# ZhuoyangLiu2005/MLA

Measured on AMD Instinct MI355X. Metric: training samples/sec + step-time, MLA-Llama2-7B bf16, higher is better.
Workload: dtype bf16; 1 GPU; BASELINE.json configs[1]: MLA-Llama2-7B SFT, use_pointcloud+use_contrastive, 672x672(+mask) image + 1024 points + 32 text tokens, per-GPU batch 8 x 4 diffusion repeats = 32 x 548 tokens; model=mla-llama2-7b, global_batch=8, seq_len=548, parallelism=single-gpu, activation_save_level=1, optimizer=fused AdamW + grad clip inside the timed region

## Files before the change

### include/mla_hip.h

```cpp
#ifndef MLA_HIP_H
#define MLA_HIP_H

#include <stddef.h>
#include <stdint.h>

#ifdef __cplusplus
extern "C" {
#endif

typedef struct ihipStream_t* mla_stream_t;

const char* mla_last_error(void);
int mla_query(int what);
const char* mla_gemm_source_id(void);
int mla_selftest(const void* src_1k, int* out_tr_256, void* out_glds_1k, mla_stream_t stream);
int mla_calib_mfma(const void* operands, float* out, int blocks, int iters, double* flops_per_launch, mla_stream_t stream);
int mla_dispatch_probe(int* out, int blocks, int hold_us, mla_stream_t stream);

int mla_gemm_bf16(const void* A, const void* B, void* C, const void* R, const void* bias, int M, int N, int K, int lda, int ldb,
                  int ldc, int ldr, int a_mode, int b_mode, int out_fp32, int accumulate, float alpha, int force_generic,
                  mla_stream_t stream);
int mla_gemm_bf16_ws(const void* A, const void* B, void* C, const void* R, const void* bias, int M, int N, int K, int lda, int ldb,
                     int ldc, int ldr, int a_mode, int b_mode, int out_fp32, int accumulate, float alpha, int force_generic,
                     float* workspace, size_t workspace_bytes, mla_stream_t stream);
int mla_gemm_sq_slots(int M, int N, int K, size_t workspace_bytes);
int mla_gemm_kloop(int mode);
int mla_gemm_cus(int n);
int mla_gemm_bf16_ws_sq(const void* A, const void* B, void* C, int M, int N, int K, int lda, int ldb, int ldc, int accumulate,
                        float alpha, float* workspace, size_t workspace_bytes, float* sq_out, int sq_capacity, int* sq_slots,
                        mla_stream_t stream);
int mla_gemm_bf16_ws_sq_rm(const void* A, const void* B, void* C, int M, int N, int K, int lda, int ldb, int ldc, int a_mode, int b_mode,
                           int accumulate, float alpha, float* workspace, size_t workspace_bytes, float* sq_out, int sq_capacity,
                           int* sq_slots, mla_stream_t stream);

int mla_gemm_qkv_rope(const void* A, const void* B, void* C, int M, int N, int K, int lda, int ldb, int ldc, const float* rope_cos,
                      const float* rope_sin, int S, int rope_cols, mla_stream_t stream);

int mla_gemm_gateup_swiglu(const void* x, const void* wgu, void* gu, void* act, void* actT, int M, int I, int K, int lda, int ldb,
                           long long ldt, mla_stream_t stream);
int mla_gemm_dact_swiglu_bwd(const void* dy, const void* wT, const void* gu, void* dgu, void* dguT, int M, int I, int K, int lda,
                             int ldb, long long ldt, mla_stream_t stream);
int mla_gemm_dact_swiglu_bwd_rm(const void* dy, const void* w, const void* gu, void* dgu, void* dguT, int M, int I, int K, int lda,
                                int ldb, long long ldt, mla_stream_t stream);

int mla_gemm_res_norm(const void* A, const void* B, void* C, const void* R, const void* g, void* xg, float* ss, int M, int N, int K,
                      int lda, int ldb, int ldc, int ldr, float* workspace, size_t workspace_bytes, mla_stream_t stream);
int mla_gemm_qkv_rope_rs(const void* A, const void* B, void* C, int M, int N, int K, int lda, int ldb, int ldc, const float* rope_cos,
                         const float* rope_sin, int S, int rope_cols, const float* ss, int parts, float eps, float* rstd,
                         mla_stream_t stream);
int mla_gemm_gateup_swiglu_rs(const void* x, const void* wgu, void* gu, void* act, void* actT, int M, int I, int K, int lda, int ldb,
                              long long ldt, const float* ss, int parts, float eps, float* rstd, mla_stream_t stream);
int mla_rmsnorm_prep(const void* x, const void* w, void* xg, float* rstd, int rows, int H, float eps, mla_stream_t stream);

int mla_rmsnorm_fwd(const void* x, const void* w, void* y, float* rstd, int rows, int H, float eps, mla_stream_t stream);
int mla_rmsnorm_apply(const void* x, const void* w, const float* rstd, void* y, long long rows, int H, mla_stream_t stream);
int mla_rmsnorm_bwd_blocks(int rows);
int mla_rmsnorm_bwd(const void* dy, const void* x, const void* w, const float* rstd, const void* dres, void* dx, float* dw,
                    int dw_accumulate, int rows, int H, float* workspace, size_t workspace_bytes, mla_stream_t stream);
int mla_timm_rmsnorm_fwd(const void* x, const void* w, void* y, float* mean, float* rstd, int rows, int H, float eps,
                         mla_stream_t stream);
int mla_timm_rmsnorm_bwd(const void* dy, const void* x, const void* w, const float* mean, const float* rstd, void* dx, float* dw,
                         int dw_accumulate, int rows, int H, float* workspace, size_t workspace_bytes, mla_stream_t stream);
int mla_colsum_blocks(int rows);
int mla_colsum_bf16(const void* dy, float* out, int accumulate, int rows, int N, int ld, float* workspace, size_t workspace_bytes,
                    mla_stream_t stream);
int mla_layernorm_fwd(const void* x, const void* w, const void* b, void* y, int rows, int H, float eps, mla_stream_t stream);

int mla_rope_inplace(void* buf, const float* cos_t, const float* sin_t, long long tokens, int S, int nheads, int D, int ld,
                     int q_off, int k_off, int backward, mla_stream_t stream);

int mla_swiglu_fwd(const void* gu, void* act, long long rows, int I, mla_stream_t stream);
int mla_swiglu_bwd(const void* dact, const void* gu, void* dgu, void* act_out, long long rows, int I, mla_stream_t stream);
int mla_act_fwd(const void* x, void* y, long long n, int kind, mla_stream_t stream);
int mla_act_bwd(const void* dy, const void* x, void* dx, long long n, int kind, mla_stream_t stream);

int mla_cast_f32_to_bf16(const float* x, void* y, long long n, mla_stream_t stream);
int mla_cast_bf16_to_f32(const void* x, float* y, long long n, mla_stream_t stream);
int mla_add_bf16(const void* a, const void* b, void* y, long long n, mla_stream_t stream);
int mla_gather_rows_bf16(const void* src, const long long* idx, void* out, long long rows, int H, int scatter, mla_stream_t stream);

int mla_transpose_bf16(const void* src, void* dst, long long R, int C, long long ld, long long ldt, mla_stream_t stream);
int mla_rmsnorm_apply_t(const void* x, const void* w, const float* rstd, void* dst, long long rows, int H, long long ldt,
                        mla_stream_t stream);
int mla_swiglu_fwd_t(const void* gu, void* dst, long long rows, int I, long long ldt, mla_stream_t stream);
int mla_swiglu_fwd_dual(const void* gu, void* act, void* actT, long long rows, int I, long long ldt, mla_stream_t stream);
int mla_swiglu_bwd_t(const void* dact, const void* gu, void* dgu, void* dguT, long long rows, int I, long long ldt, mla_stream_t stream);

int mla_embedding_fwd(const long long* ids, const void* table, void* out, long long tokens, int H, int vocab, mla_stream_t stream);
int mla_embedding_bwd(const long long* ids, const void* dy, float* grad, float* workspace, long long tokens, int H, int vocab,
                      mla_stream_t stream);

int mla_adamw_step(float* p, const float* g, float* m, float* v, void* p16, long long n, float lr, float beta1, float beta2,
                   float eps, float weight_decay, int step, const float* grad_scale, mla_stream_t stream);
int mla_adamw_step_groups(float* p, const float* g, float* m, float* v, void* p16, long long n, long long n_decay, float lr, float beta1,
                          float beta2, float eps, float weight_decay, int step, const float* grad_scale, mla_stream_t stream);
int mla_sumsq_f32(const float* x, long long n, float* out, int accumulate, float* workspace, size_t workspace_bytes,
                  mla_stream_t stream);
int mla_sum_partials(const float* partial, int n, float* out, int accumulate, mla_stream_t stream);
int mla_clip_coef(const float* sumsq, float max_norm, float* coef, float* norm_out, mla_stream_t stream);

int mla_q_sample(const float* x0, const float* noise, const long long* t, const float* sqrt_ac, const float* sqrt_1mac, float* out,
                 int batch, int per, int nsteps, mla_stream_t stream);

int mla_attn_fwd(const void* q, const void* k, const void* v, void* o, float* lse, const int* seqlens, int B, int S, int H,
                 int head_dim, long long ld_qkv, long long ld_o, float scale, mla_stream_t stream);
int mla_attn_fwd_g(const void* q, const void* k, const void* v, void* o, float* lse, const int* seqlens, int B, int S, int H,
                   int head_dim, long long ld_qkv, long long ld_o, float scale, int grp_start, int grp_len, const int* grp_starts,
                   mla_stream_t stream);
int mla_attn_bwd_g(const void* q, const void* k, const void* v, const void* o, const void* dout, const float* lse, const int* seqlens,
                   void* dq, void* dk, void* dv, float* delta, int B, int S, int H, int head_dim, long long ld_qkv, long long ld_o,
                   float scale, const float* rope_cos, const float* rope_sin, void* dqT, void* dkT, void* dvT, void* oT,
                   long long ldt, int* head_sync, long long head_sync_ints, int grp_start, int grp_len, const int* grp_starts,
                   int rope_per_sample, mla_stream_t stream);
long long mla_attn_bwd_sync_ints(int B, int H);
int mla_attn_bwd(const void* q, const void* k, const void* v, const void* o, const void* dout, const float* lse, const int* seqlens,
                 void* dq, void* dk, void* dv, float* delta, int B, int S, int H, int head_dim, long long ld_qkv, long long ld_o,
                 float scale, const float* rope_cos, const float* rope_sin, int* head_sync, long long head_sync_ints,
                 mla_stream_t stream);
int mla_attn_bwd_t(const void* q, const void* k, const void* v, const void* o, const void* dout, const float* lse, const int* seqlens,
                   void* dq, void* dk, void* dv, float* delta, int B, int S, int H, int head_dim, long long ld_qkv, long long ld_o,
                   float scale, const float* rope_cos, const float* rope_sin, void* dqT, void* dkT, void* dvT, void* oT,
                   long long ldt, int* head_sync, long long head_sync_ints, mla_stream_t stream);
long long mla_attn_bwd_ws_bytes(int B, int S, int H);
int mla_attn_bwd_ws(const void* q, const void* k, const void* v, const void* o, const void* dout, const float* lse, const int* seqlens,
                    void* dq, void* dk, void* dv, float* delta, int B, int S, int H, int head_dim, long long ld_qkv, long long ld_o,
                    float scale, const float* rope_cos, const float* rope_sin, void* dqT, void* dkT, void* dvT, void* oT, long long ldt,
                    void* ws, long long ws_bytes, mla_stream_t stream);

int mla_gemv_bf16(const void* x, long long ldx, const void* W, long long ldw, void* out, long long ldo, long long out_batch_stride,
                  int rows_per_batch, const void* residual, long long ld_res, int M, int N, int K, int pre, const void* pre_w, float eps,
                  const float* rope_cos, const float* rope_sin, int rope_cols, mla_stream_t stream);
int mla_attn_decode(const void* q, const void* k, const void* v, void* o, int B, int H, int head_dim, int S_kv, int R, long long ld,
                    long long batch_stride, long long ld_o, float scale, mla_stream_t stream);
int mla_gemm_skinny_bf16(const void* x, long long ldx, const void* W, long long ldw, void* out, long long ldo, long long out_batch_stride,
                         int rows_per_batch, const void* residual, long long ld_res, int M, int N, int K, int pre, const void* pre_w, float eps,
                         const float* rope_cos, const float* rope_sin, int rope_cols, mla_stream_t stream);
int mla_quant_fp8_rows(const void* W, long long ldw, void* q, long long ldq, float* scale, int N, int K, mla_stream_t stream);
int mla_gemv_w8(const void* x, long long ldx, const void* W, long long ldw, const float* w_scale, void* out, long long ldo,
                long long out_batch_stride, int rows_per_batch, const void* residual, long long ld_res, int M, int N, int K, int pre,
                const void* pre_w, float eps, const float* rope_cos, const float* rope_sin, int rope_cols, mla_stream_t stream);
int mla_gemm_skinny_w8(const void* x, long long ldx, const void* W, long long ldw, const float* w_scale, void* out, long long ldo,
                       long long out_batch_stride, int rows_per_batch, const void* residual, long long ld_res, int M, int N, int K, int pre,
                       const void* pre_w, float eps, const float* rope_cos, const float* rope_sin, int rope_cols, mla_stream_t stream);
int mla_attn_chunk(const void* q, const void* k, const void* v, void* o, int B, int H, int head_dim, int S_kv, int R, long long ld,
                   long long batch_stride, long long ld_o, float scale, mla_stream_t stream);
int mla_attn_chunk_ragged(const void* q, const void* k, const void* v, void* o, int B, int H, int head_dim, const int* kv_len, int S_cap,
                          int R, long long ld, long long batch_stride, long long ld_o, float scale, mla_stream_t stream);
int mla_gemm_suffix_bf16(const void* x, long long ldx, const void* W, long long ldw, void* out, long long ldo, long long out_batch_stride,
                         int rows_per_batch, const int* slot, int cap_rows, const void* residual, long long ld_res, int M, int N, int K,
                         const float* rope_cos, const float* rope_sin, int rope_cols, mla_stream_t stream);
int mla_gemm_suffix_w8(const void* x, long long ldx, const void* W, long long ldw, const float* w_scale, void* out, long long ldo,
                       long long out_batch_stride, int rows_per_batch, const int* slot, int cap_rows, const void* residual, long long ld_res,
                       int M, int N, int K, const float* rope_cos, const float* rope_sin, int rope_cols, mla_stream_t stream);
int mla_attn_chunk_groups(const void* q, const void* k, const void* v, void* o, int G, int H, int head_dim, int S_p, int R, long long ld,
                          long long ld_o, float scale, mla_stream_t stream);
int mla_attn_chunk_groups_gw(const void* q, const void* k, const void* v, void* o, int G, int H, int head_dim, int S_p, int R, long long ld,
                             long long ld_o, float scale, int gw, int order, mla_stream_t stream);
int mla_attn_chunk_ragged_groups(const void* q, const void* k, const void* v, void* o, int B, int G, int H, int head_dim,
                                 const int* prefix_len, int S_cap, int R, long long ld, long long batch_stride, long long ld_o, float scale,
                                 mla_stream_t stream);
int mla_attn_chunk_ragged_groups_gw(const void* q, const void* k, const void* v, void* o, int B, int G, int H, int head_dim,
                                    const int* prefix_len, int S_cap, int R, long long ld, long long batch_stride, long long ld_o, float scale,
                                    int gw, int order, mla_stream_t stream);
int mla_gemm_suffix_bf16_pos(const void* x, long long ldx, const void* W, long long ldw, void* out, long long ldo, long long out_batch_stride,
                             int rows_per_batch, const int* slot, int cap_rows, const void* residual, long long ld_res, int M, int N, int K,
                             const float* rope_cos, const float* rope_sin, int rope_cols, const int* rope_pos, int rope_rows,
                             mla_stream_t stream);
int mla_gemm_suffix_w8_pos(const void* x, long long ldx, const void* W, long long ldw, const float* w_scale, void* out, long long ldo,
                           long long out_batch_stride, int rows_per_batch, const int* slot, int cap_rows, const void* residual,
                           long long ld_res, int M, int N, int K, const float* rope_cos, const float* rope_sin, int rope_cols,
                           const int* rope_pos, int rope_rows, mla_stream_t stream);
int mla_gemm_prefill_plan(int M, int N, int K, int cus, int* out4);
long long mla_gemm_prefill_ws_bytes(int M, int N, int K);
int mla_gemm_prefill_bf16(const void* x, long long ldx, const void* W, long long ldw, void* out, long long ldo, long long out_batch_stride,
                          int rows_per_batch, const void* residual, long long ld_res, int M, int N, int K, void* workspace,
                          size_t workspace_bytes, mla_stream_t stream);
int mla_gemm_prefill_qkv_rope(const void* x, long long ldx, const void* W, long long ldw, void* out, long long ldo,
                              long long out_batch_stride, int rows_per_batch, int M, int N, int K, const float* rope_cos,
                              const float* rope_sin, int rope_cols, int head_dim, void* workspace, size_t workspace_bytes,
                              mla_stream_t stream);
int mla_gemm_prefill_gateup_swiglu(const void* x, long long ldx, const void* wgu, long long ldw, void* act, long long ldo,
                                   long long out_batch_stride, int rows_per_batch, int M, int I, int K, void* workspace,
                                   size_t workspace_bytes, mla_stream_t stream);
int mla_gemm_prefill_f8_plan(int M, int N, int K, int cus, int* out4);
long long mla_gemm_prefill_f8_ws_bytes(int M, int N, int K);
int mla_gemm_prefill_f8(const void* xq, long long ldx, const float* x_scale, const void* Wq, long long ldw, const float* w_scale, void* out,
                        long long ldo, long long out_batch_stride, int rows_per_batch, const void* residual, long long ld_res, int M, int N,
                        int K, void* workspace, size_t workspace_bytes, mla_stream_t stream);
int mla_gemm_prefill_f8_qkv_rope(const void* xq, long long ldx, const float* x_scale, const void* Wq, long long ldw, const float* w_scale,
                                 void* out, long long ldo, long long out_batch_stride, int rows_per_batch, int M, int N, int K,
                                 const float* rope_cos, const float* rope_sin, int rope_cols, int head_dim, void* workspace,
                                 size_t workspace_bytes, mla_stream_t stream);
int mla_gemm_prefill_f8_gateup_swiglu(const void* xq, long long ldx, const float* x_scale, const void* wgu_q, long long ldw,
                                      const float* w_scale, void* act, long long ldo, long long out_batch_stride, int rows_per_batch, int M,
                                      int I, int K, void* workspace, size_t workspace_bytes, mla_stream_t stream);
int mla_gemm_prefill_f8_wide_plan(int M, int N, int K, int cus, int* out4);
long long mla_gemm_prefill_f8_wide_ws_bytes(int M, int N, int K);
int mla_gemm_prefill_f8_wide(const void* xq, long long ldx, const float* x_scale, const void* Wq, long long ldw, const float* w_scale,
                             void* out, long long ldo, long long out_batch_stride, int rows_per_batch, const void* residual,
                             long long ld_res, int M, int N, int K, void* workspace, size_t workspace_bytes, mla_stream_t stream);
int mla_gemm_prefill_f8_wide_qkv_rope(const void* xq, long long ldx, const float* x_scale, const void* Wq, long long ldw,
                                      const float* w_scale, void* out, long long ldo, long long out_batch_stride, int rows_per_batch, int M,
                                      int N, int K, const float* rope_cos, const float* rope_sin, int rope_cols, int head_dim,
                                      void* workspace, size_t workspace_bytes, mla_stream_t stream);
int mla_gemm_prefill_f8_wide_gateup_swiglu(const void* xq, long long ldx, const float* x_scale, const void* wgu_q, long long ldw,
                                           const float* w_scale, void* act, long long ldo, long long out_batch_stride, int rows_per_batch,
                                           int M, int I, int K, void* workspace, size_t workspace_bytes, mla_stream_t stream);

int mla_ddim_step(float* x, const void* eps, void* x_bf16, const float* coef, int* step, int n, int steps, int advance,
                  mla_stream_t stream);
int mla_ddpm_step(float* x, const void* eps, void* x_bf16, const float* coef, const float* noise, int* step, int n, int steps,
                  int advance, mla_stream_t stream);
int mla_sampler_rows(void* h_in, const void* t_table, const void* x_e, const int* step, int G, int T, int H, int steps,
                     mla_stream_t stream);

int mla_attn_chunk_split_plan(int B, int H, int R, int S_kv, int cus, int* out4);
long long mla_attn_chunk_split_ws_bytes(int B, int H, int R, int S_kv, int splits);
int mla_attn_chunk_split(const void* q, const void* k, const void* v, void* o, int B, int H, int head_dim, int S_kv, int R, long long ld,
                         long long batch_stride, long long ld_o, float scale, int splits, void* ws, size_t ws_bytes, mla_stream_t stream);
int mla_attn_groups_split(const void* q, const void* k, const void* v, void* o, int B, int G, int H, int head_dim, const int* prefix_len,
                          int S_p_or_cap, int R, long long ld, long long batch_stride, long long ld_o, float scale, int splits, void* ws,
                          size_t ws_bytes, mla_stream_t stream);

int mla_ce_fwd(const void* logits, int logits_fp32, long long ld, const long long* labels, float* loss, float* lse, int rows,
               int ncols, long long ignore_index, mla_stream_t stream);
int mla_ce_bwd(const void* logits, int logits_fp32, long long ld, const long long* labels, const float* lse, const float* gscale,
               float inv_count, void* dlogits, long long ldd, int rows, int ncols, long long ignore_index, mla_stream_t stream);
int mla_infonce_bwd(const float* L, const float* rlse, const float* clse, const float* gscale, void* dL, int M, int Mp,
                    mla_stream_t stream);
int mla_l2norm_fwd(const void* x, void* y, float* norms, int rows, int ncols, float eps, mla_stream_t stream);
int mla_l2norm_bwd(const void* dy, const void* y, const float* norms, void* dx, int rows, int ncols, mla_stream_t stream);

int mla_project_points(const float* xyz, const float* consts21, long long* idx, unsigned char* valid, int n, float W, float Hh,
                       float stride, int ph, int pw, mla_stream_t stream);
int mla_fps(const float* xyz, const long long* start, long long* out, int B, int N, int npoint, mla_stream_t stream);
int mla_knn(const float* xyz, const float* centers, int* out, int B, int N, int G, int k, mla_stream_t stream);
int mla_gather_rows_f32(const float* src, const long long* idx, float* out, int B, int N, int G, int W, mla_stream_t stream);
int mla_lga_prep(const float* xyz, const void* feats, const long long* fps_idx, const int* knn, void* rows, float* lc_xyz, int B,
                 int N, int G, int K, int C, float alpha, float beta, mla_stream_t stream);
int mla_colstats_blocks(long long rows);
int mla_colstats_bf16(const void* x, float* mean, float* var, long long rows, int C, int ld, float* workspace, size_t workspace_bytes,
                      mla_stream_t stream);
int mla_bn_apply(const void* x, const float* mean, const float* var, const void* w, const void* b, const void* res, void* y,
                 long long rows, int C, float eps, int relu, mla_stream_t stream);
int mla_maxpool_k(const void* x, void* out, long long groups, int K, int C, mla_stream_t stream);
int mla_lga_prep_bwd(const void* drows, const long long* fps_idx, const int* knn, float* dfeats, int B, int N, int G, int K, int C,
                     mla_stream_t stream);
int mla_maxpool_k_bwd(const void* x, const void* dy, void* dx, long long groups, int K, int C, mla_stream_t stream);

int mla_im2col_patch(const void* pix, int pix_fp32, void* rows, int B, int CT, int Himg, int Wimg, int P, int Kpad,
                     mla_stream_t stream);
int mla_avgpool_tokens(const void* x, void* y, int B, int gh, int gw, int C, int cs, mla_stream_t stream);
int mla_local_attn(const void* q, const void* kv, void* out, int B, int gh, int gw, int C, int cs, int heads, float scale,
                   mla_stream_t stream);
int mla_local_attn_bwd(const void* q, const void* kv, const void* dout, void* dq, void* dkv, int B, int gh, int gw, int C, int cs,
                       int heads, float scale, mla_stream_t stream);
int mla_clip_preprocess(const unsigned char* img, int B, int Hin, int Win, const int* bounds_h, const int* coef_h, int ks_h,
                        const int* bounds_v, const int* coef_v, int ks_v, void* out, int out_fp32, int OH, int OW, const float* mean3,
                        const float* std3, int mask_channel, mla_stream_t stream);
int mla_avgpool_tokens_bwd(const void* dy, const void* other, void* dx, int B, int gh, int gw, int C, int cs, mla_stream_t stream);

int mla_gemm_batched_bf16(const void* A, const void* B, void* C, int M, int N, int K, int lda, int ldb, int ldc, int a_mode, int b_mode,
                          int out_fp32, float alpha, int n_outer, int n_inner, long long sAo, long long sAi, long long sBo,
                          long long sBi, long long sCo, long long sCi, mla_stream_t stream);

int mla_softmax_rows_fwd(const float* scores, void* P, void* Pd, long long rows, int ncols, int nvalid, float p,
                         unsigned long long seed, mla_stream_t stream);
int mla_softmax_rows_bwd(const void* dPd, int dpd_fp32, const void* P, void* dS, long long rows, int ncols, int nvalid, float p,
                         unsigned long long seed, mla_stream_t stream);
int mla_dropout_fwd(const void* x, const void* residual, void* y, long long n, float p, unsigned long long seed, mla_stream_t stream);
int mla_dropout_bwd(const void* dy, void* dx, long long n, float p, unsigned long long seed, mla_stream_t stream);
int mla_scale_batch(const void* x, const float* scale, void* y, long long batch, long long per, mla_stream_t stream);
int mla_layernorm_stats_fwd(const void* x, const void* w, const void* b, void* y, float* mean, float* rstd, long long rows, int H,
                            float eps, mla_stream_t stream);
int mla_layernorm_bwd_blocks(long long rows);
int mla_layernorm_bwd(const void* dy, const void* x, const void* w, const float* mean, const float* rstd, void* dx, float* dw,
                      float* db, int accumulate, long long rows, int H, float* workspace, size_t workspace_bytes,
                      mla_stream_t stream);
int mla_seqmean_fwd(const void* x, void* y, int B, int S, int C, mla_stream_t stream);
int mla_seqmean_bwd(const void* dy, void* dx, int B, int S, int C, mla_stream_t stream);
int mla_bn_bwd_blocks(long long rows);
int mla_bn_bwd(const void* dy, const void* x, const float* mean, const float* var, const void* w, void* dx, float* dw, float* db,
               int accumulate, long long rows, int C, float eps, float* workspace, size_t workspace_bytes, mla_stream_t stream);
int mla_chamfer_fwd(const float* pred, const float* gt, float* d1, int* i1, float* d2, int* i2, float* loss, int B, int N, int M,
                    float* workspace, size_t workspace_bytes, mla_stream_t stream);
int mla_chamfer_bwd(const float* pred, const float* gt, const float* d1, const int* i1, const float* d2, const int* i2,
                    const float* gscale, float* dpred, int B, int N, int M, mla_stream_t stream);
int mla_imgloss_fwd(const void* delta_raw, int ld, const void* curr, const void* next, int img_fp32, float* sums, int B, int CT_curr,
                    int CT_next, int HW, int ps, float clip, float* workspace, size_t workspace_bytes, mla_stream_t stream);
int mla_imgroi_fwd(const void* delta_raw, int ld, const void* a_raw, int lda, const void* o_raw, int ldo, const unsigned char* roi,
                   const void* curr, const void* next, int img_fp32, float* sums, int B, int CT_curr, int CT_next, int HW, int ps,
                   float clip, float shift, float* workspace, size_t workspace_bytes, mla_stream_t stream);
int mla_imgroi_bwd(const void* delta_raw, int ld, const void* a_raw, int lda, const void* o_raw, int ldo, const unsigned char* roi,
                   const void* curr, const void* next, int img_fp32, const float* coef, void* ddelta_raw, float* dalpha_raw,
                   float* doff_raw, int B, int CT_curr, int CT_next, int HW, int ps, float clip, float shift, mla_stream_t stream);
int mla_imgloss_bwd(const void* delta_raw, int ld, const void* curr, const void* next, int img_fp32, const float* gscale,
                    void* ddelta_raw, int B, int CT_curr, int CT_next, int HW, int ps, float clip, mla_stream_t stream);

int mla_side_traffic(const float* a, const float* b, float* out, long long n, int blocks, int lds_bytes, int sleep_ticks, mla_stream_t stream);

#ifdef __cplusplus
}
#endif
#endif
```

### mla_amd/csrc/gemm256.hip

```cpp
#include "common.h"

#include "gemm_args.h"

#include "gemm256_kloop_clobbers.inc"
#include "gemm256_kloop_rm_clobbers.inc"
#ifndef MLA_GEMM_PLAIN_STORES
#define MLA_ST16(ADDR, VAL) __builtin_nontemporal_store((u32x4_t)(VAL), (u32x4_t*)(ADDR))
#define MLA_LD16(ADDR) __builtin_nontemporal_load((const u32x4_t*)(ADDR))
#else
#define MLA_ST16(ADDR, VAL) (*(u32x4_t*)(ADDR) = (VAL))
#define MLA_LD16(ADDR) (*(const u32x4_t*)(ADDR))
#endif

namespace {

constexpr int SLOT = 16384;
constexpr int SA0 = 0, SB0 = SLOT, SB1 = 2 * SLOT, SA1 = 3 * SLOT, BUF = 4 * SLOT;

__device__ __forceinline__ int hsw(int kr) { return (kr & 3) | (((kr >> 3) & 1) << 2); }
__device__ __forceinline__ int xcd_remap(int bid, int nwg) {
  const int q = nwg >> 3, r = nwg & 7;
  const int xcd = bid & 7, idx = bid >> 3;
  return (xcd < r ? xcd * (q + 1) : r * (q + 1) + (xcd - r) * q) + idx;
}

template <int MODE, bool IS_A>
__device__ __forceinline__ const bf16_t* stage_src(const bf16_t* g, int ld, int base, int lim, int h, int instr, int lane) {
  const int p = instr * 64 + lane;
  if (MODE == 0) {
    const int rp = p >> 3, cp = p & 7;
    const int c = cp ^ (rp & 7);
    int gi = base + h * 128 + rp;
    gi = gi < lim ? gi : lim - 1;
    return g + (size_t)gi * ld + c * 8;
  } else {
    const int kr = p >> 4, cp = p & 15;
    const int c = cp ^ (hsw(kr) << 1);
    const int ip = c * 8;
    int gi = base + h * 128 + ip;
    gi = (gi + 8 <= lim) ? gi : 0;
    return g + (size_t)kr * ld + gi;
  }
}

#ifndef MLA_GROUP_M
#define MLA_GROUP_M 4
#endif
#ifndef MLA_GEMM256_UNTRACKED
#define MLA_GEMM256_UNTRACKED 0
#endif
template <int AMODE, int BMODE, int EPI = 0, bool ASM = false>
__global__ __launch_bounds__(512, 2) void gemm256_kernel(GemmArgs p) {
  const bool LGKM_BEFORE = false;
  const int GROUP_M = MLA_GROUP_M;
#ifdef MLA_GEMM256_ABLATION
  const bool NO_READ = (p.debug & 4) != 0, NO_STAGE = (p.debug & 8) != 0, NO_BAR2 = (p.debug & 16) != 0, NO_BAR1 = (p.debug & 32) != 0;
  const int dbg = p.debug;
#else
  constexpr bool NO_READ = false, NO_STAGE = false, NO_BAR2 = false, NO_BAR1 = false;
  constexpr int dbg = 0;
#endif
  extern __shared__ __attribute__((aligned(16))) char smem[];
  const int tid = threadIdx.x, lane = tid & 63;
  const int wave = __builtin_amdgcn_readfirstlane(tid >> 6);
  const int wr = wave >> 2, wc = wave & 3;
  const int li = lane & 15, lg = lane >> 4;

  const int num_m = (p.M + 255) / 256, num_n = (p.N + 255) / 256;
  int pid, kt0 = 0, nt = p.K / 64;
  float* part = nullptr;
  if (p.sk_split <= 1) {
    pid = xcd_remap(blockIdx.x, gridDim.x);
  } else if ((int)blockIdx.x < p.sk_full) {
    pid = xcd_remap(blockIdx.x, p.sk_full);
  } else {
    const int u = blockIdx.x - p.sk_full;
    const int slice = u % p.sk_split;
    pid = p.sk_full + u / p.sk_split;
    if ((nt & 1) == 0) {
      const int np = nt >> 1;
      kt0 = 2 * (int)((long long)slice * np / p.sk_split);
      nt = 2 * (int)((long long)(slice + 1) * np / p.sk_split) - kt0;
    } else {
    kt0 = (int)((long long)slice * nt / p.sk_split);
    nt = (int)((long long)(slice + 1) * nt / p.sk_split) - kt0;
    }
    part = p.sk_ws + (size_t)u * 65536;
  }
#ifdef MLA_EXPERIMENTAL_KERNELS
  if (EPI != 0 && p.stagger_mode && (int)blockIdx.x < 256) {
    const bool late = p.stagger_mode == 1 ? (blockIdx.x & 1) : ((blockIdx.x >> 3) & 1);
    if (late) {
      const unsigned long long t0 = wall_clock64();
      while ((long long)(wall_clock64() - t0) < (long long)p.stagger_ticks) __builtin_amdgcn_s_sleep(64);
    }
  }
#endif
  const int in_group = GROUP_M * num_n;
  const int group_id = pid / in_group;
  const int first_m = group_id * GROUP_M;
  const int gsz = (num_m - first_m) < GROUP_M ? (num_m - first_m) : GROUP_M;
  const int pid_m = first_m + (pid % in_group) % gsz;
  const int pid_n = (pid % in_group) / gsz;
  const int m0 = pid_m * 256, n0 = pid_n * 256;

  f32x4_t acc[8][4];
  if constexpr (ASM) {
    static_assert(EPI == 0 || (AMODE == 0 && BMODE == 0) || (EPI == 2 && AMODE == 0 && BMODE == 1),
                  "the fused epilogues take k-contiguous operands (SwiGLU backward: or the weight as stored, B reduction-major)");
    const unsigned c0 = ((unsigned)lg ^ ((unsigned)li & 7u)) << 4;
    const unsigned vA0 = (unsigned)((wr * 64 + li) * 128) + c0, vB0 = 32768u + (unsigned)((wc * 32 + li) * 128) + c0;
    const unsigned lchunk = ((unsigned)lane & 7u) ^ (((unsigned)lane >> 3) & 7u);
    const int rt0 = wave * 32 + (lane >> 3);
    const int lastA = (p.M - 1 - m0) < 255 ? (p.M - 1 - m0) : 255;
    int lastB = (p.N - 1 - n0) < 255 ? (p.N - 1 - n0) : 255, bshift = 0;
    const bf16_t* pB = p.B + (size_t)n0 * p.ldb + (size_t)kt0 * 64;
    if (EPI == 1) {
      pB = p.B + (size_t)pid_n * 128 * p.ldb;
      bshift = wave >= 4 ? p.sf_I - 128 : 0;
      lastB = 255;
    }
    const unsigned oA0 = (unsigned)rt0 * (unsigned)p.lda * 2u + lchunk * 16u;
    const unsigned oB0 = (unsigned)(rt0 + bshift) * (unsigned)p.ldb * 2u + lchunk * 16u;
    const unsigned oAmax = (unsigned)lastA * (unsigned)p.lda * 2u + lchunk * 16u;
    const unsigned oBmax = (unsigned)(lastB + bshift) * (unsigned)p.ldb * 2u + lchunk * 16u;
    const int sA8 = p.lda * 16, sB8 = p.ldb * 16;
    const bf16_t* pA = p.A + (size_t)m0 * p.lda + (size_t)kt0 * 64;
    const int kmax = nt * 128 - 128, nit = nt >> 1, ldsw = wave * 4096;
    const bool img_bf16 = !part && !p.out_fp32 && p.R == nullptr && p.bias == nullptr;
    const bool rowscale = img_bf16 && p.rs_rstd != nullptr;
    if (rowscale && tid < 256) {
      const int mr = (m0 + tid) < p.M ? (m0 + tid) : (p.M - 1);
      float r;
      if (p.rs_ss) {
        const float* sp = p.rs_ss + (size_t)mr * p.rs_parts;
        float t = 0.f;
        for (int j = 0; j < p.rs_parts; ++j) t += sp[j];
        r = 1.0f / sqrtf(t / (float)p.K + p.rs_eps);
        if (pid_n == 0 && m0 + tid < p.M) p.rs_rstd[mr] = r;
      } else {
        r = p.rs_rstd[mr];
      }
      *(float*)(smem + 2 * BUF + tid * 4) = r;
    }
    const int emode = img_bf16 ? (rowscale ? 2 : 0) : 1;
    const float alpha = part ? 1.f : p.alpha;
    const unsigned vImg = img_bf16 ? (unsigned)((wr * 64 + li) * 512) + ((((unsigned)(wc * 4 + (lg >> 1))) ^ (unsigned)li) << 4) + (unsigned)(lg & 1) * 8u
                                   : (unsigned)((wr * 64 + li) * 1024) + ((((unsigned)(wc * 8 + lg)) ^ (unsigned)li) << 4);
    if constexpr (AMODE != 0 || BMODE != 0) {
      const int hs = ((li >> 2) & 3) | ((lg & 1) << 2);
      const unsigned rmrow = (unsigned)((lg * 8 + (li >> 2)) * 16), rmsub = (unsigned)((li & 3) >> 1), rmlo = (unsigned)(li & 1) * 8u;
      const unsigned vA = AMODE ? (rmrow + (((unsigned)(wr * 8) + rmsub) ^ ((unsigned)hs << 1))) * 16u + rmlo : vA0;
      const unsigned vB = BMODE ? 32768u + (rmrow + (((unsigned)(wc * 4) + rmsub) ^ ((unsigned)hs << 1))) * 16u + rmlo : vB0;
      const unsigned oAh0 = AMODE ? (unsigned)((const char*)stage_src<1, true>(p.A, p.lda, m0, p.M, 0, wave * 2, lane) - (const char*)p.A) : oA0;
      const unsigned oAh1 = AMODE ? (unsigned)((const char*)stage_src<1, true>(p.A, p.lda, m0, p.M, 1, wave * 2, lane) - (const char*)p.A) : oAmax;
      const unsigned oBh0 = BMODE ? (unsigned)((const char*)stage_src<1, false>(p.B, p.ldb, n0, p.N, 0, wave * 2, lane) - (const char*)p.B) : oB0;
      const unsigned oBh1 = BMODE ? (unsigned)((const char*)stage_src<1, false>(p.B, p.ldb, n0, p.N, 1, wave * 2, lane) - (const char*)p.B) : oBmax;
      const bf16_t* pAr = AMODE ? p.A + (size_t)kt0 * 64 * p.lda : pA;
      const bf16_t* pBr = BMODE ? p.B + (size_t)kt0 * 64 * p.ldb : pB;
      const int ldswA = AMODE ? wave * 2048 : ldsw, ldswB = BMODE ? wave * 2048 : ldsw;
      const int sA4 = p.lda * 8, sB4 = p.ldb * 8;
      const int nit_s = __builtin_amdgcn_readfirstlane(nit), emode_s = __builtin_amdgcn_readfirstlane(emode);
      const int alpha_s = __builtin_amdgcn_readfirstlane(__float_as_int(alpha));
#if defined(__HIP_DEVICE_COMPILE__)
#define MLA_KLOOP_RM_OPERANDS                                                                                                              \
        : : [pA] "s"(pAr), [pB] "s"(pBr), [nit] "s"(nit_s), [ldsw] "s"(ldswA), [ldswB] "s"(ldswB), [kA] "s"(p.lda), [kB] "s"(p.ldb),          \
            [sA8] "s"(sA8), [sB8] "s"(sB8), [sA4] "s"(sA4), [sB4] "s"(sB4), [emode] "s"(emode_s), [alpha] "s"(alpha_s), [vA0] "v"(vA),         \
            [vB0] "v"(vB), [oA0] "v"(oAh0), [oA2] "v"(oAh1), [oAmax] "v"(oAh1), [oB0] "v"(oBh0), [oB2] "v"(oBh1), [oBmax] "v"(oBh1),        \
            [vImg] "v"(vImg)                                                                                                                \
        : "memory", "scc", "vcc", "s40", "s41", "s42", "s43", "s44", "s45", "s46", "s47", "s48", "s49", "s50", "s51", "s52", "s53", "s54",  \
          "s55", "s56", "s57", "s58"
      if constexpr (AMODE != 0 && BMODE != 0) {
        asm volatile(
#include "gemm256_kloop_rm11.inc"
            MLA_KLOOP_RM_OPERANDS, G256K_RM11_CLOBBERS);
      } else if constexpr (AMODE != 0) {
        asm volatile(
#include "gemm256_kloop_rm10.inc"
            MLA_KLOOP_RM_OPERANDS, G256K_RM10_CLOBBERS);
      } else {
        asm volatile(
#include "gemm256_kloop_rm01.inc"
            MLA_KLOOP_RM_OPERANDS, G256K_RM01_CLOBBERS);
      }
#undef MLA_KLOOP_RM_OPERANDS
#endif
    } else {
#if defined(__HIP_DEVICE_COMPILE__)
    asm volatile(
#include "gemm256_kloop.inc"
        : : [pA] "s"(pA), [pB] "s"(pB), [kmax] "v"(kmax), [nit] "v"(nit), [ldsw] "s"(ldsw), [sA8] "s"(sA8), [sB8] "s"(sB8),
            [emode] "v"(emode), [alpha] "v"(alpha), [vA0] "v"(vA0), [vB0] "v"(vB0), [oA0] "v"(oA0), [oB0] "v"(oB0), [oAmax] "v"(oAmax),
            [oBmax] "v"(oBmax), [vImg] "v"(vImg)
        : "memory", "scc", "vcc", "s40", "s41", "s42", "s43", "s44", "s45", "s46", "s47", "s48", "s49", "s50", "s51", "s52", "s53", G256K_CLOBBERS);
#endif
    }
    if constexpr (EPI == 0) if (part) {
#pragma unroll
      for (int hf = 0; hf < 2; ++hf) {
        if (hf) {
          __syncthreads();
#if defined(__HIP_DEVICE_COMPILE__)
          asm volatile(
#include "gemm256_kloop_half1.inc"
              : : [alpha] "v"(alpha), [vImg] "v"(vImg) : "memory", "v0", "v1", "v2", "v3", "v4", "v5", "v6", "v7", "v8", "v9", "v10", "v11",
                "v12", "v13", "v14", "v15", "v16", "v17", "v18", "v19");
#endif
        }
        __syncthreads();
#pragma unroll
        for (int it = 0; it < 16; ++it) {
          const int row = wave * 16 + it;
          *(f32x4_t*)(part + (hf * 128 + row) * 256 + lane * 4) = *(const f32x4_t*)(smem + row * 1024 + ((lane ^ (row & 63)) << 4));
        }
      }
      return;
    }
  } else {
  const size_t stepA = (dbg & 64) ? 0 : (dbg & 2) ? 64 : (AMODE == 0 ? 64 : (size_t)64 * p.lda);
  const size_t stepB = (dbg & 64) ? 0 : (dbg & 2) ? 64 : (BMODE == 0 ? 64 : (size_t)64 * p.ldb);
  const bf16_t* pA0[2]; const bf16_t* pA1[2]; const bf16_t* pB0[2]; const bf16_t* pB1[2];
#pragma unroll
  for (int it = 0; it < 2; ++it) {
    if (dbg & 2) {
      pA0[it] = stage_src<0, true>(p.A, 4096, 0, 4096, 0, wave * 2 + it, lane);
      pA1[it] = stage_src<0, true>(p.A, 4096, 0, 4096, 1, wave * 2 + it, lane);
      pB0[it] = stage_src<0, false>(p.B, 4096, 0, 4096, 0, wave * 2 + it, lane);
      pB1[it] = stage_src<0, false>(p.B, 4096, 0, 4096, 1, wave * 2 + it, lane);
      continue;
    }
    pA0[it] = stage_src<AMODE, true>(p.A, p.lda, m0, p.M, 0, wave * 2 + it, lane);
    pA1[it] = stage_src<AMODE, true>(p.A, p.lda, m0, p.M, 1, wave * 2 + it, lane);
    if (EPI == 1) {
      pB0[it] = stage_src<BMODE, false>(p.B, p.ldb, pid_n * 128, p.sf_I, 0, wave * 2 + it, lane);
      pB1[it] = stage_src<BMODE, false>(p.B, p.ldb, p.sf_I + pid_n * 128 - 128, 2 * p.sf_I, 1, wave * 2 + it, lane);
      continue;
    }
    pB0[it] = stage_src<BMODE, false>(p.B, p.ldb, n0, p.N, 0, wave * 2 + it, lane);
    pB1[it] = stage_src<BMODE, false>(p.B, p.ldb, n0, p.N, 1, wave * 2 + it, lane);
  }
  if (kt0) {
#pragma unroll
    for (int it = 0; it < 2; ++it) {
      pA0[it] += (size_t)kt0 * stepA; pA1[it] += (size_t)kt0 * stepA;
      pB0[it] += (size_t)kt0 * stepB; pB1[it] += (size_t)kt0 * stepB;
    }
  }
  int tA0 = 0, tA1 = 0, tB0 = 0, tB1 = 0;
  constexpr bool UNTRACKED = (AMODE != 0 || BMODE != 0) || MLA_GEMM256_UNTRACKED;

#define STAGE(PTR, TCNT, STEP, SLOTOFF)                                                           \
  do {                                                                                            \
    const size_t back__ = (TCNT < nt) ? 0 : (size_t)TCNT * (STEP);  \
    char* dst__ = smem + (TCNT & 1) * BUF + (SLOTOFF) + wave * 2048;                              \
    if (!NO_STAGE || TCNT < 2) {  \
      if (UNTRACKED) {                                                                            \
        glds16_untracked(PTR[0] - back__, dst__);                                                 \
        glds16_untracked(PTR[1] - back__, dst__ + 1024);                                          \
      } else {                                                                                    \
        glds16(PTR[0] - back__, dst__);                                                           \
        glds16(PTR[1] - back__, dst__ + 1024);                                                    \
      }                                                                                           \
    }                                                                                             \
    PTR[0] += (STEP); PTR[1] += (STEP); ++TCNT;                                                   \
  } while (0)

  int offA[4], offB[2];
  if (AMODE == 0) {
    offA[0] = (wr * 64 + li) * 128 + ((lg ^ (li & 7)) * 16);
    offA[1] = offA[2] = offA[3] = 0;
  } else {
    const int h = ((li >> 2) & 3) | ((lg & 1) << 2);
#pragma unroll
    for (int rb = 0; rb < 4; ++rb)
      offA[rb] = ((lg * 8 + (li >> 2)) * 16 + ((wr * 8 + rb * 2 + ((li & 3) >> 1)) ^ (h << 1))) * 16 + (li & 1) * 8;
  }
  if (BMODE == 0) {
    offB[0] = (wc * 32 + li) * 128 + ((lg ^ (li & 7)) * 16);
    offB[1] = 0;
  } else {
    const int h = ((li >> 2) & 3) | ((lg & 1) << 2);
#pragma unroll
    for (int cb = 0; cb < 2; ++cb)
      offB[cb] = ((lg * 8 + (li >> 2)) * 16 + ((wc * 4 + cb * 2 + ((li & 3) >> 1)) ^ (h << 1))) * 16 + (li & 1) * 8;
  }

  auto ldA = [&](const char* slot, int rb, int ks) -> bf16x8_t {
    if (AMODE == 0) {
      return *(const bf16x8_t*)(slot + ((offA[0] + rb * 2048) ^ (ks * 64)));
    } else {
      if (dbg & 1) return *(const bf16x8_t*)(slot + (((wr * 64 + li) * 128 + ((lg ^ (li & 7)) * 16) + rb * 2048) ^ (ks * 64)));
      union { bf16x8_t v; short4_t h2[2]; } u;
      u.h2[0] = lds_tr16_b64(slot + offA[rb] + ks * 8192);
      u.h2[1] = lds_tr16_b64(slot + offA[rb] + ks * 8192 + 1024);
      return u.v;
    }
  };
  auto ldB = [&](const char* slot, int cb, int ks) -> bf16x8_t {
    if (BMODE == 0) {
      return *(const bf16x8_t*)(slot + ((offB[0] + cb * 2048) ^ (ks * 64)));
    } else {
      if (dbg & 1) return *(const bf16x8_t*)(slot + (((wc * 32 + li) * 128 + ((lg ^ (li & 7)) * 16) + cb * 2048) ^ (ks * 64)));
      union { bf16x8_t v; short4_t h2[2]; } u;
      u.h2[0] = lds_tr16_b64(slot + offB[cb] + ks * 8192);
      u.h2[1] = lds_tr16_b64(slot + offB[cb] + ks * 8192 + 1024);
      return u.v;
    }
  };

#pragma unroll
  for (int a = 0; a < 8; ++a)
#pragma unroll
    for (int b = 0; b < 4; ++b) acc[a][b] = f32x4_t{0.f, 0.f, 0.f, 0.f};

  bf16x8_t fa[4][2], fb0[2][2], fb1[2][2];
  bool rd_on = true;

#define READ_A(SLOTP)                                              \
  if (rd_on) _Pragma("unroll") for (int rb = 0; rb < 4; ++rb) {    \
    fa[rb][0] = ldA(SLOTP, rb, 0); fa[rb][1] = ldA(SLOTP, rb, 1);  \
  }
#define READ_B(DST, SLOTP)                                          \
  if (rd_on) _Pragma("unroll") for (int cb = 0; cb < 2; ++cb) {     \
    DST[cb][0] = ldB(SLOTP, cb, 0); DST[cb][1] = ldB(SLOTP, cb, 1); \
  }
#define SEG_END()                                                  \
  __builtin_amdgcn_sched_barrier(0);                               \
  if (LGKM_BEFORE) asm volatile("s_waitcnt vmcnt(8) lgkmcnt(0)" ::: "memory"); \
  else asm volatile("s_waitcnt vmcnt(10)" ::: "memory");           \
  if (!NO_BAR1) __builtin_amdgcn_s_barrier();                      \
  asm volatile("s_waitcnt lgkmcnt(0)" ::: "memory");               \
  __builtin_amdgcn_sched_barrier(0);
#define MMA(QI, QJ, FB)                                                                                          \
  __builtin_amdgcn_s_setprio(1);                                                                                 \
  _Pragma("unroll") for (int ks = 0; ks < 2; ++ks)                                                               \
  _Pragma("unroll") for (int rb = 0; rb < 4; ++rb)                                                               \
  _Pragma("unroll") for (int cb = 0; cb < 2; ++cb)                                                               \
    acc[QI * 4 + rb][QJ * 2 + cb] =                                                                              \
        __builtin_amdgcn_mfma_f32_16x16x32_bf16(FB[cb][ks], fa[rb][ks], acc[QI * 4 + rb][QJ * 2 + cb], 0, 0, 0); \
  __builtin_amdgcn_s_setprio(0);                                                                                 \
  __builtin_amdgcn_sched_barrier(0);                                                                             \
  asm volatile("" ::: "memory");                                                                                 \
  if (!NO_BAR2) __builtin_amdgcn_s_barrier();                                                                    \
  asm volatile("" ::: "memory");

  STAGE(pB0, tB0, stepB, SB0);
  STAGE(pA0, tA0, stepA, SA0);
  STAGE(pB1, tB1, stepB, SB1);
  STAGE(pA1, tA1, stepA, SA1);
  STAGE(pB0, tB0, stepB, SB0);
  STAGE(pA0, tA0, stepA, SA0);
  STAGE(pB1, tB1, stepB, SB1);
  asm volatile("s_waitcnt vmcnt(10)" ::: "memory");
  __builtin_amdgcn_s_barrier();
  READ_B(fb0, smem + SB0)
  if (wr == 1) __builtin_amdgcn_s_barrier();

#define TILE_BODY(X, Y, T_)                                          \
  {                                                                  \
    const char* buf = smem + ((T_) & 1) * BUF;                       \
    const char* nbuf = smem + (((T_) + 1) & 1) * BUF;                \
    if (NO_READ) rd_on = (T_) < 2;                                   \
    STAGE(pA1, tA1, stepA, SA1);                       \
    READ_A(buf + SA0)                                                \
    SEG_END()                                                        \
    MMA(0, 0, X)                                                     \
    STAGE(pB0, tB0, stepB, SB0);                       \
    READ_B(Y, buf + SB1)                                             \
    SEG_END()                                                        \
    MMA(0, 1, Y)                                                     \
    STAGE(pA0, tA0, stepA, SA0);                       \
    READ_A(buf + SA1)                                                \
    SEG_END()                                                        \
    MMA(1, 1, Y)                                                     \
    STAGE(pB1, tB1, stepB, SB1);                       \
    READ_B(Y, nbuf + SB0)                                            \
    SEG_END()                                                        \
    MMA(1, 0, X)                                                     \
  }
  int t = 0;
  for (; t + 1 < nt; t += 2) {
    TILE_BODY(fb0, fb1, t)
    TILE_BODY(fb1, fb0, t + 1)
  }
  if (t < nt) TILE_BODY(fb0, fb1, t)
#undef TILE_BODY
  if (wr == 0) __builtin_amdgcn_s_barrier();
  asm volatile("s_waitcnt vmcnt(0)" ::: "memory");
  }

  if constexpr (!ASM) if (part) {
#pragma unroll
    for (int ri = 0; ri < 8; ++ri) {
      const int ml = (ri >> 2) * 128 + wr * 64 + (ri & 3) * 16 + li;
#pragma unroll
      for (int ci = 0; ci < 4; ++ci) {
        const int nl = (ci >> 1) * 128 + wc * 32 + (ci & 1) * 16 + lg * 4;
        *(f32x4_t*)(part + ml * 256 + nl) = acc[ri][ci];
      }
    }
    return;
  }
  const bool vec_ok = ((p.ldc & 3) == 0) && (p.R == nullptr || (p.ldr & 3) == 0);
  const bool fast = (p.N & 7) == 0 && (p.ldc & 7) == 0 && (((uintptr_t)p.C) & 15) == 0 &&
                    (p.R == nullptr || ((p.ldr & 7) == 0 && (((uintptr_t)p.R) & 15) == 0)) &&
                    (p.bias == nullptr || (((uintptr_t)p.bias) & 15) == 0);
  if (fast) {
    __syncthreads();
    if (!p.out_fp32 && p.R == nullptr && p.bias == nullptr) {
      if constexpr (!ASM) {
      if (p.rs_rstd) {
        if (tid < 256) {
          const int mr = (m0 + tid) < p.M ? (m0 + tid) : (p.M - 1);
          float r;
          if (p.rs_ss) {
            const float* sp = p.rs_ss + (size_t)mr * p.rs_parts;
            float t = 0.f;
            for (int j = 0; j < p.rs_parts; ++j) t += sp[j];
            r = 1.0f / sqrtf(t / (float)p.K + p.rs_eps);
            if (pid_n == 0 && m0 + tid < p.M) p.rs_rstd[mr] = r;
          } else {
            r = p.rs_rstd[mr];
          }
          *(float*)(smem + 2 * BUF + tid * 4) = r;
        }
        __syncthreads();
      }
#pragma unroll
      for (int ri = 0; ri < 8; ++ri) {
        const int ml = (ri >> 2) * 128 + wr * 64 + (ri & 3) * 16 + li;
        const float rsc = p.rs_rstd ? *(const float*)(smem + 2 * BUF + ml * 4) : p.alpha;
#pragma unroll
        for (int ci = 0; ci < 4; ++ci) {
          const int nl = (ci >> 1) * 128 + wc * 32 + (ci & 1) * 16 + lg * 4;
          u32x2_t o;
          o[0] = pack2bf(acc[ri][ci][0] * rsc, acc[ri][ci][1] * rsc);
          o[1] = pack2bf(acc[ri][ci][2] * rsc, acc[ri][ci][3] * rsc);
          *(u32x2_t*)(smem + ml * 512 + ((((nl >> 3) ^ (ml & 31))) << 4) + ((nl >> 2) & 1) * 8) = o;
        }
      }
      }
      __syncthreads();
      if (EPI == 1) {
        const int I = p.sf_I, cbase = pid_n * 128;
        const size_t ld2 = (size_t)2 * I;
        for (int s4 = 0; s4 < 4; ++s4) {
          char* scrA = smem + s4 * 64 * 512;
          u32x4_t pa[2];
#pragma unroll
          for (int k4 = 0; k4 < 4; ++k4) {
            const int idx = tid + 512 * k4;
            const int rl = idx >> 5, ch = idx & 31;
            const int row = s4 * 64 + rl, m = m0 + row;
            if (p.C && m < p.M)
              MLA_ST16((bf16_t*)p.C + (size_t)m * ld2 + (ch < 16 ? cbase + ch * 8 : I + cbase + (ch - 16) * 8), *(const u32x4_t*)(smem + row * 512 + ((ch ^ (row & 31)) << 4)));
          }
#pragma unroll
          for (int k2 = 0; k2 < 2; ++k2) {
            const int idx = tid + 512 * k2;
            const int rl = idx >> 4, c = idx & 15;
            const int row = s4 * 64 + rl, m = m0 + row;
            float gv[8], uv[8], o[8];
            unpack8(*(const u32x4_t*)(smem + row * 512 + ((c ^ (row & 31)) << 4)), gv);
            unpack8(*(const u32x4_t*)(smem + row * 512 + (((16 + c) ^ (row & 31)) << 4)), uv);
#pragma unroll
            for (int j = 0; j < 8; ++j) o[j] = swiglu_fwd_elem(gv[j], uv[j]);
            pa[k2] = pack8(o);
            if (p.sf_act && m < p.M) MLA_ST16(p.sf_act + (size_t)m * I + cbase + c * 8, pa[k2]);
          }
          if (p.sf_actT == nullptr) continue;
          __syncthreads();
#pragma unroll
          for (int k2 = 0; k2 < 2; ++k2) {
            const int idx = tid + 512 * k2;
            const int rl = idx >> 4, c = idx & 15;
            const int slot2 = (rl ^ (2 * c)) * 2;
#pragma unroll
            for (int j = 0; j < 4; ++j) {
              const int c0 = (c * 8 + 2 * j) * 128 + slot2;
              *(unsigned short*)(scrA + c0) = (unsigned short)(pa[k2][j] & 0xffffu);
              *(unsigned short*)(scrA + c0 + 128) = (unsigned short)(pa[k2][j] >> 16);
            }
          }
          __syncthreads();
#pragma unroll
          for (int k2 = 0; k2 < 2; ++k2) {
            const int idx = tid + 512 * k2;
            const int col = idx >> 3, rc = idx & 7;
            const int chc = col >> 3, b = chc & 3;
            const int m = m0 + s4 * 64 + rc * 8;
            if (m < p.M) {
              u32x4_t w = *(const u32x4_t*)(scrA + col * 128 + ((rc ^ (chc >> 2)) << 4));
              if (b & 1) w = u32x4_t{w[1], w[0], w[3], w[2]};
              if (b & 2) w = u32x4_t{w[2], w[3], w[0], w[1]};
              MLA_ST16(p.sf_actT + (size_t)(cbase + col) * p.sf_ldt + m, w);
            }
          }
        }
        return;
      }
      if (EPI == 2) {
        const int I = p.sw_I;
        char* scrB = smem + 2 * BUF;
        const size_t ld2 = (size_t)2 * I;
        u32x4_t gq[4], uq[4];
        auto fetch_gu = [&](int strip, u32x4_t* g4, u32x4_t* u4) {
#pragma unroll
          for (int k4 = 0; k4 < 4; ++k4) {
            const int idx = tid + 512 * k4;
            const int m = m0 + strip * 64 + (idx >> 5), n = n0 + (idx & 31) * 8;
            g4[k4] = u32x4_t{0u, 0u, 0u, 0u};
            u4[k4] = g4[k4];
            if (m < p.M && n < p.N) {
              g4[k4] = MLA_LD16(p.sw_gu + (size_t)m * ld2 + n);
              u4[k4] = MLA_LD16(p.sw_gu + (size_t)m * ld2 + I + n);
            }
          }
        };
        if constexpr (ASM) fetch_gu(0, gq, uq);
        for (int s4 = 0; s4 < 4; ++s4) {
          char* scrA = smem + s4 * 64 * 512;
          u32x4_t pg[4], pu[4];
          u32x4_t gn[4], un[4];
          if constexpr (ASM) if (s4 < 3) fetch_gu(s4 + 1, gn, un);
#pragma unroll
          for (int k4 = 0; k4 < 4; ++k4) {
            const int idx = tid + 512 * k4;
            const int rl = idx >> 5, ch = idx & 31;
            const int row = s4 * 64 + rl;
            const int m = m0 + row, n = n0 + ch * 8;
            pg[k4] = u32x4_t{0u, 0u, 0u, 0u};
            pu[k4] = pg[k4];
            if (m < p.M && n < p.N) {
              float dv[8], gv[8], uv[8], dg[8], du[8];
              unpack8(*(const u32x4_t*)(smem + row * 512 + ((ch ^ (row & 31)) << 4)), dv);
              if constexpr (ASM) {
                unpack8(gq[k4], gv);
                unpack8(uq[k4], uv);
              } else {
              unpack8(*(const u32x4_t*)(p.sw_gu + (size_t)m * ld2 + n), gv);
              unpack8(*(const u32x4_t*)(p.sw_gu + (size_t)m * ld2 + I + n), uv);
              }
#pragma unroll
              for (int j = 0; j < 8; ++j) swiglu_bwd_elem(dv[j], gv[j], uv[j], dg[j], du[j]);
              pg[k4] = pack8(dg);
              pu[k4] = pack8(du);
              MLA_ST16(p.sw_dgu + (size_t)m * ld2 + n, pg[k4]);
              MLA_ST16(p.sw_dgu + (size_t)m * ld2 + I + n, pu[k4]);
            }
          }
          if (p.sw_dguT == nullptr) {
            if constexpr (ASM) {
#pragma unroll
              for (int k4 = 0; k4 < 4; ++k4) { gq[k4] = gn[k4]; uq[k4] = un[k4]; }
            }
            continue;
          }
          __syncthreads();
#pragma unroll
          for (int k4 = 0; k4 < 4; ++k4) {
            const int idx = tid + 512 * k4;
            const int rl = idx >> 5, ch = idx & 31;
            const int slot2 = (rl ^ (2 * ch)) * 2;
#pragma unroll
            for (int j = 0; j < 4; ++j) {
              const int c0 = (ch * 8 + 2 * j) * 128 + slot2;
              *(unsigned short*)(scrA + c0) = (unsigned short)(pg[k4][j] & 0xffffu);
              *(unsigned short*)(scrA + c0 + 128) = (unsigned short)(pg[k4][j] >> 16);
              *(unsigned short*)(scrB + c0) = (unsigned short)(pu[k4][j] & 0xffffu);
              *(unsigned short*)(scrB + c0 + 128) = (unsigned short)(pu[k4][j] >> 16);
            }
          }
          __syncthreads();
#pragma unroll
          for (int k4 = 0; k4 < 4; ++k4) {
            const int idx = tid + 512 * k4;
            const int col = idx >> 3, rc = idx & 7;
            const int chc = col >> 3;
            const int off = col * 128 + ((rc ^ (chc >> 2)) << 4);
            const int b = chc & 3;
            const int m = m0 + s4 * 64 + rc * 8, n = n0 + col;
            if (m < p.M && n < p.N) {
#pragma unroll
              for (int which = 0; which < 2; ++which) {
                u32x4_t w = *(const u32x4_t*)((which ? scrB : scrA) + off);
                if (b & 1) w = u32x4_t{w[1], w[0], w[3], w[2]};
                if (b & 2) w = u32x4_t{w[2], w[3], w[0], w[1]};
                MLA_ST16(p.sw_dguT + (size_t)(which * I + n) * p.sw_ldt + m, w);
              }
            }
          }
          if constexpr (ASM) {
#pragma unroll
            for (int k4 = 0; k4 < 4; ++k4) { gq[k4] = gn[k4]; uq[k4] = un[k4]; }
          }
        }
        return;
      }
      const int ch = lane & 31;
      const int n = n0 + ch * 8;
      if (p.rope_cos && n0 < p.rope_cols) {
        if (n < p.N) {
          const bool lo = (ch & 8) == 0;
#pragma unroll 4
          for (int it = 0; it < 16; ++it) {
            const int row = wave * 32 + it * 2 + (lane >> 5);
            const int m = m0 + row;
            if (m < p.M) {
              float own[8], par[8], c[8], sn[8], o[8];
              unpack8(*(const u32x4_t*)(smem + row * 512 + ((ch ^ (row & 31)) << 4)), own);
              unpack8(*(const u32x4_t*)(smem + row * 512 + (((ch ^ 8) ^ (row & 31)) << 4)), par);
              const float* ct = p.rope_cos + (size_t)(m % p.rope_S) * 64 + (ch & 7) * 8;
              const float* st = p.rope_sin + (size_t)(m % p.rope_S) * 64 + (ch & 7) * 8;
              const f32x4_t c0 = *(const f32x4_t*)ct, c1 = *(const f32x4_t*)(ct + 4), s0 = *(const f32x4_t*)st, s1 = *(const f32x4_t*)(st + 4);
#pragma unroll
              for (int j = 0; j < 4; ++j) { c[j] = c0[j]; c[j + 4] = c1[j]; sn[j] = s0[j]; sn[j + 4] = s1[j]; }
#pragma unroll
              for (int j = 0; j < 8; ++j)
                o[j] = lo ? fmaf(own[j], c[j], -(par[j] * sn[j])) : fmaf(own[j], c[j], par[j] * sn[j]);
              MLA_ST16((bf16_t*)p.C + (size_t)m * p.ldc + n, pack8(o));
            }
          }
        }
        return;
      }
      if (n < p.N) {
#pragma unroll
        for (int it = 0; it < 16; ++it) {
          const int row = wave * 32 + it * 2 + (lane >> 5);
          const int m = m0 + row;
          if (m < p.M)
            MLA_ST16((bf16_t*)p.C + (size_t)m * p.ldc + n, *(const u32x4_t*)(smem + row * 512 + ((ch ^ (row & 31)) << 4)));
        }
      }
      return;
    }
    if constexpr (EPI == 0 || !ASM) {
    float sq = 0.f;
    u32x4_t rpre[2][8];
    const bool r_pre = ASM && p.R != nullptr && !p.out_fp32;
    if (r_pre) {
      const int nn = n0 + (lane & 31) * 8;
#pragma unroll
      for (int h2 = 0; h2 < 2; ++h2)
#pragma unroll
        for (int it = 0; it < 8; ++it) {
          const int m = m0 + h2 * 128 + wave * 16 + it * 2 + (lane >> 5);
          rpre[h2][it] = u32x4_t{0u, 0u, 0u, 0u};
          if (m < p.M && nn < p.N) rpre[h2][it] = MLA_LD16(p.R + (size_t)m * p.ldr + nn);
        }
    }
#pragma unroll
    for (int hf = 0; hf < 2; ++hf) {
      if (hf) __syncthreads();
      if constexpr (ASM) {
#if defined(__HIP_DEVICE_COMPILE__)
        if (hf) {
          const unsigned vImg2 = (unsigned)((wr * 64 + li) * 1024) + ((((unsigned)(wc * 8 + lg)) ^ (unsigned)li) << 4);
          asm volatile(
#include "gemm256_kloop_half1.inc"
              : : [alpha] "v"(p.alpha), [vImg] "v"(vImg2) : "memory", "v0", "v1", "v2", "v3", "v4", "v5", "v6", "v7", "v8", "v9", "v10",
                "v11", "v12", "v13", "v14", "v15", "v16", "v17", "v18", "v19");
        }
#endif
      } else {
#pragma unroll
      for (int r4 = 0; r4 < 4; ++r4) {
        const int ri = hf * 4 + r4;
        const int ml = wr * 64 + r4 * 16 + li;
#pragma unroll
        for (int ci = 0; ci < 4; ++ci) {
          const int nl = (ci >> 1) * 128 + wc * 32 + (ci & 1) * 16 + lg * 4;
          *(f32x4_t*)(smem + ml * 1024 + (((nl >> 2) ^ (ml & 63)) << 4)) = acc[ri][ci] * p.alpha;
        }
      }
      }
      __syncthreads();
      if (p.out_fp32) {
        const int n = n0 + lane * 4;
        if (n < p.N) {
#pragma unroll
          for (int it = 0; it < 16; ++it) {
            const int row = wave * 16 + it;
            const int m = m0 + hf * 128 + row;
            if (m < p.M) {
              f32x4_t o = *(const f32x4_t*)(smem + row * 1024 + ((lane ^ (row & 63)) << 4));
              if (p.bias) {
                const u32x2_t bb = *(const u32x2_t*)(p.bias + n);
                o[0] += bflo(bb[0]); o[1] += bfhi(bb[0]); o[2] += bflo(bb[1]); o[3] += bfhi(bb[1]);
              }
              if (p.R) {
                const u32x2_t rr = *(const u32x2_t*)(p.R + (size_t)m * p.ldr + n);
                o[0] += bflo(rr[0]); o[1] += bfhi(rr[0]); o[2] += bflo(rr[1]); o[3] += bfhi(rr[1]);
              }
              float* c = (float*)p.C + (size_t)m * p.ldc + n;
              if (p.accumulate) o += *(const f32x4_t*)c;
              *(f32x4_t*)c = o;
              sq += (o[0] * o[0] + o[1] * o[1]) + (o[2] * o[2] + o[3] * o[3]);
            }
          }
        }
      } else {
        const int ch = lane & 31;
        const int n = n0 + ch * 8;
        if (n < p.N) {
          float bv[8];
#pragma unroll
          for (int j = 0; j < 8; ++j) bv[j] = 0.f;
          if (p.bias) unpack8(*(const u32x4_t*)(p.bias + n), bv);
          float ngv[8];
#pragma unroll
          for (int j = 0; j < 8; ++j) ngv[j] = 0.f;
          if (p.nrm_xg) unpack8(*(const u32x4_t*)(p.nrm_g + n), ngv);
#pragma unroll
          for (int it = 0; it < 8; ++it) {
            const int row = wave * 16 + it * 2 + (lane >> 5);
            const int m = m0 + hf * 128 + row;
            if (m < p.M) {
              const f32x4_t a = *(const f32x4_t*)(smem + row * 1024 + (((2 * ch) ^ (row & 63)) << 4));
              const f32x4_t b = *(const f32x4_t*)(smem + row * 1024 + (((2 * ch + 1) ^ (row & 63)) << 4));
              float v[8] = {a[0] + bv[0], a[1] + bv[1], a[2] + bv[2], a[3] + bv[3], b[0] + bv[4], b[1] + bv[5], b[2] + bv[6], b[3] + bv[7]};
              if (p.R) {
                float rv[8];
                unpack8(r_pre ? rpre[hf][it] : *(const u32x4_t*)(p.R + (size_t)m * p.ldr + n), rv);
#pragma unroll
                for (int j = 0; j < 8; ++j) v[j] += rv[j];
              }
              const u32x4_t hq = pack8(v);
              MLA_ST16((bf16_t*)p.C + (size_t)m * p.ldc + n, hq);
              if (p.nrm_xg) {
                float hv[8], xg[8];
                unpack8(hq, hv);
                float q = 0.f;
#pragma unroll
                for (int j = 0; j < 8; ++j) { q += hv[j] * hv[j]; xg[j] = hv[j] * ngv[j]; }
                MLA_ST16(p.nrm_xg + (size_t)m * p.ldc + n, pack8(xg));
                q = half_wave_sum_last(q);
                if (ch == 31) p.nrm_ss[(size_t)m * num_n + pid_n] = q;
              }
            }
          }
        }
      }
    }
    if (p.sq_out) {
      sq = wave_sum(sq);
      __syncthreads();
      if (lane == 0) ((float*)smem)[wave] = sq;
      __syncthreads();
      if (tid == 0) {
        float t = 0.f;
#pragma unroll
        for (int w = 0; w < 8; ++w) t += ((float*)smem)[w];
        p.sq_out[pid] = t;
      }
    }
    }
    return;
  }
  if constexpr (!ASM) {
#pragma unroll
  for (int ri = 0; ri < 8; ++ri) {
    const int m = m0 + (ri >> 2) * 128 + wr * 64 + (ri & 3) * 16 + li;
    if (m >= p.M) continue;

#pragma unroll
    for (int ci = 0; ci < 4; ++ci) {
      const int n = n0 + (ci >> 1) * 128 + wc * 32 + (ci & 1) * 16 + lg * 4;
      if (n >= p.N) continue;
      float v[4];
#pragma unroll
      for (int r = 0; r < 4; ++r) v[r] = acc[ri][ci][r] * p.alpha;
      if (n + 3 < p.N && vec_ok) {
        if (p.bias) {
          const u32x2_t bb = *(const u32x2_t*)(p.bias + n);
          v[0] += bflo(bb[0]); v[1] += bfhi(bb[0]); v[2] += bflo(bb[1]); v[3] += bfhi(bb[1]);
        }
        if (p.R) {
          const u32x2_t rr = *(const u32x2_t*)(p.R + (size_t)m * p.ldr + n);
          v[0] += bflo(rr[0]); v[1] += bfhi(rr[0]); v[2] += bflo(rr[1]); v[3] += bfhi(rr[1]);
        }
        if (p.out_fp32) {
          float* c = (float*)p.C + (size_t)m * p.ldc + n;
          f32x4_t o = {v[0], v[1], v[2], v[3]};
          if (p.accumulate) o += *(const f32x4_t*)c;
          *(f32x4_t*)c = o;
        } else {
          u32x2_t o;
          o[0] = pack2bf(v[0], v[1]);
          o[1] = pack2bf(v[2], v[3]);
          *(u32x2_t*)((bf16_t*)p.C + (size_t)m * p.ldc + n) = o;
        }
      } else {
        for (int r = 0; r < 4 && n + r < p.N; ++r) {
          float x = v[r];
          if (p.bias) x += bf2f(p.bias[n + r]);
          if (p.R) x += bf2f(p.R[(size_t)m * p.ldr + n + r]);
          if (p.out_fp32) {
            float* c = (float*)p.C + (size_t)m * p.ldc + n + r;
            *c = p.accumulate ? (*c + x) : x;
          } else {
            ((bf16_t*)p.C)[(size_t)m * p.ldc + n + r] = f2bf(x);
          }
        }
      }
    }
  }
  }
#undef STAGE
#undef READ_A
#undef READ_B
#undef SEG_END
#undef MMA
}

#ifdef MLA_EXPERIMENTAL_KERNELS
struct Unit {
  int m0, n0, kt0, nt;
  float* part;
};

__global__ __launch_bounds__(512, 2) void gemm256p_kernel(GemmArgs p) {
  const int GROUP_M = MLA_GROUP_M;
  extern __shared__ __attribute__((aligned(16))) char smem[];
  const int tid = threadIdx.x, lane = tid & 63;
  const int wave = __builtin_amdgcn_readfirstlane(tid >> 6);
  const int wr = wave >> 2, wc = wave & 3;
  const int li = lane & 15, lg = lane >> 4;
  const int num_m = (p.M + 255) / 256, num_n = (p.N + 255) / 256;
  const int ntK = p.K / 64;

  const int G = gridDim.x, W = G >> 3, b = blockIdx.x, x = b & 7, j = b >> 3;
  const int F = p.sk_split > 1 ? p.sk_full : num_m * num_n;
  const int q8 = F >> 3, r8 = F & 7;
  const int cnt_x = q8 + (x < r8 ? 1 : 0);
  const int start_x = x < r8 ? x * (q8 + 1) : r8 * (q8 + 1) + (x - r8) * q8;
  const int nfull = j < cnt_x ? (cnt_x - j + W - 1) / W : 0;
  const int tail_units = p.sk_split > 1 ? (num_m * num_n - p.sk_full) * p.sk_split : 0;
  const int ntail = b < tail_units ? (tail_units - b + G - 1) / G : 0;
  const int n_units = nfull + ntail;
  if (n_units == 0) return;
  auto get_unit = [&](int i) -> Unit {
    Unit u;
    int pid;
    if (i < nfull) {
      pid = start_x + j + W * i;
      u.kt0 = 0; u.nt = ntK; u.part = nullptr;
    } else {
      const int t = b + (i - nfull) * G;
// ... 6 lines not shown
    const int in_group = GROUP_M * num_n;
    const int first_m = (pid / in_group) * GROUP_M;
    const int gsz = (num_m - first_m) < GROUP_M ? (num_m - first_m) : GROUP_M;
    u.m0 = __builtin_amdgcn_readfirstlane((first_m + (pid % in_group) % gsz) * 256);
    u.n0 = __builtin_amdgcn_readfirstlane(((pid % in_group) / gsz) * 256);
    u.kt0 = __builtin_amdgcn_readfirstlane(u.kt0);
    u.nt = __builtin_amdgcn_readfirstlane(u.nt);
    return u;
  };

  const int rowA = p.lda * 2, rowB = p.ldb * 2;
  const char* gbA0; const char* gbA1; const char* gbB0; const char* gbB1;
  unsigned voA0[2], voA1[2], voB0[2], voB1[2];
  int stA0 = 128, stA1 = 128, stB0 = 128, stB1 = 128;
  int leftA0, leftB0, leftB1, leftA1, suA0 = 0, suB0 = 0, suB1 = 0, suA1 = 0, tA0 = 0, tB0 = 0, tB1 = 0, tA1 = 0;
#define PSLOT_SET(X, U, ISA, HALF)                                                                                  \
  do {                                                                                                              \
    const int lim_rows__ = (ISA) ? p.M : p.N;                                                                       \
    int hb__ = ((ISA) ? (U).m0 : (U).n0) + (HALF) * 128;                                                            \
    int lim__ = lim_rows__ - 1 - hb__;                                                                              \
    if (lim__ < 0) { hb__ = lim_rows__ - 128; lim__ = 127; }       \
    lim__ = lim__ < 127 ? lim__ : 127;                                                                              \
    gb##X = (const char*)((ISA) ? p.A : p.B) + (size_t)hb__ * ((ISA) ? rowA : rowB) + (size_t)(U).kt0 * 128;        \
    _Pragma("unroll") for (int it__ = 0; it__ < 2; ++it__) {                                                        \
      const int q__ = (wave * 2 + it__) * 64 + lane;                                                                \
      const int rp__ = q__ >> 3, cp__ = q__ & 7;                                                                    \
      const int c__ = cp__ ^ (rp__ & 7);                                                                            \
      const int re__ = rp__ < lim__ ? rp__ : lim__;                                                                 \
      vo##X[it__] = (unsigned)((re__ * ((ISA) ? p.lda : p.ldb) + c__ * 8) * 2);                                     \
    }                                                                                                               \
    left##X = (U).nt;                                                                                               \
  } while (0)
  Unit cu = get_unit(0);
  PSLOT_SET(A0, cu, true, 0);
  PSLOT_SET(A1, cu, true, 1);
  PSLOT_SET(B0, cu, false, 0);
  PSLOT_SET(B1, cu, false, 1);

#define PSTAGE(X, ISA, HALF, SLOTOFF)                                                                                      \
  do {                                                                                                                     \
    char* dst__ = smem + (t##X & 1) * BUF + (SLOTOFF) + wave * 2048;                                                       \
    glds16(gb##X + vo##X[0], dst__);                                                                                       \
    glds16(gb##X + vo##X[1], dst__ + 1024);                                                                                \
    gb##X += st##X; ++t##X;                                                                                                \
    if (--left##X == 0) {                                                                                                  \
      if (++su##X < n_units) {                                                                                             \
        const Unit nu__ = get_unit(su##X);                                                                                 \
        PSLOT_SET(X, nu__, ISA, HALF);                                                                                     \
      } else {                                                                                                             \
                                \
        gb##X -= 128; st##X = 0; left##X = 0x7fffffff;                                                                     \
      }                                                                                                                    \
    }                                                                                                                      \
  } while (0)
#define ST_A0() PSTAGE(A0, true, 0, SA0)
#define ST_A1() PSTAGE(A1, true, 1, SA1)
#define ST_B0() PSTAGE(B0, false, 0, SB0)
#define ST_B1() PSTAGE(B1, false, 1, SB1)

  const int offA = (wr * 64 + li) * 128 + ((lg ^ (li & 7)) * 16);
  const int offB = (wc * 32 + li) * 128 + ((lg ^ (li & 7)) * 16);
  auto ldA = [&](const char* slot, int rb, int ks) -> bf16x8_t { return *(const bf16x8_t*)(slot + ((offA + rb * 2048) ^ (ks * 64))); };
  auto ldB = [&](const char* slot, int cb, int ks) -> bf16x8_t { return *(const bf16x8_t*)(slot + ((offB + cb * 2048) ^ (ks * 64))); };

  f32x4_t acc[8][4];
#pragma unroll
  for (int a = 0; a < 8; ++a)
#pragma unroll
    for (int c = 0; c < 4; ++c) acc[a][c] = f32x4_t{0.f, 0.f, 0.f, 0.f};
  bf16x8_t fa[4][2], fb0[2][2], fb1[2][2];

#define PREAD_A(SLOTP)                                             \
  _Pragma("unroll") for (int rb = 0; rb < 4; ++rb) {               \
    fa[rb][0] = ldA(SLOTP, rb, 0); fa[rb][1] = ldA(SLOTP, rb, 1);  \
  }
#define PREAD_B(DST, SLOTP)                                         \
  _Pragma("unroll") for (int cb = 0; cb < 2; ++cb) {                \
    DST[cb][0] = ldB(SLOTP, cb, 0); DST[cb][1] = ldB(SLOTP, cb, 1); \
  }
#define PSEG_END()                                   \
  __builtin_amdgcn_sched_barrier(0);                 \
  asm volatile("s_waitcnt vmcnt(6)" ::: "memory");   \
  __builtin_amdgcn_s_barrier();                      \
  asm volatile("s_waitcnt lgkmcnt(0)" ::: "memory"); \
  __builtin_amdgcn_sched_barrier(0);
#define PMMA(QI, QJ, FB)                                                                                         \
  __builtin_amdgcn_s_setprio(1);                                                                                 \
  _Pragma("unroll") for (int ks = 0; ks < 2; ++ks)                                                               \
  _Pragma("unroll") for (int rb = 0; rb < 4; ++rb)                                                               \
  _Pragma("unroll") for (int cb = 0; cb < 2; ++cb)                                                               \
    acc[QI * 4 + rb][QJ * 2 + cb] =                                                                              \
        __builtin_amdgcn_mfma_f32_16x16x32_bf16(FB[cb][ks], fa[rb][ks], acc[QI * 4 + rb][QJ * 2 + cb], 0, 0, 0); \
  __builtin_amdgcn_s_setprio(0);                                                                                 \
  __builtin_amdgcn_sched_barrier(0);                                                                             \
  asm volatile("" ::: "memory");                                                                                 \
  __builtin_amdgcn_s_barrier();                                                                                  \
  asm volatile("" ::: "memory");
#define PTILE(X, Y, PAR)                                             \
  {                                                                  \
    const char* buf = smem + (PAR) * BUF;                            \
    const char* nbuf = smem + (1 - (PAR)) * BUF;                     \
    ST_B1();                                                         \
    PREAD_A(buf + SA0)                                               \
    PSEG_END()                                                       \
    PMMA(0, 0, X)                                                    \
    ST_A1();                                                         \
    PREAD_B(Y, buf + SB1)                                            \
    PSEG_END()                                                       \
    PMMA(0, 1, Y)                                                    \
    ST_A0();                                                         \
    PREAD_A(buf + SA1)                                               \
    PSEG_END()                                                       \
    PMMA(1, 1, Y)                                                    \
    ST_B0();                                                         \
    PREAD_B(Y, nbuf + SB0)                                           \
    PSEG_END()                                                       \
    PMMA(1, 0, X)                                                    \
  }

  auto epilogue = [&]() __attribute__((always_inline)) {
    const int m0 = cu.m0, n0 = cu.n0;
    if (cu.part) {
      float* part = cu.part;
#pragma unroll
      for (int ri = 0; ri < 8; ++ri) {
        const int ml = (ri >> 2) * 128 + wr * 64 + (ri & 3) * 16 + li;
#pragma unroll
        for (int ci = 0; ci < 4; ++ci) {
          const int nl = (ci >> 1) * 128 + wc * 32 + (ci & 1) * 16 + lg * 4;
          *(f32x4_t*)(part + ml * 256 + nl) = acc[ri][ci];
        }
      }
    } else {
      const bool vec_ok = ((p.ldc & 3) == 0) && (p.R == nullptr || (p.ldr & 3) == 0);
#pragma unroll
      for (int ri = 0; ri < 8; ++ri) {
        const int m = m0 + (ri >> 2) * 128 + wr * 64 + (ri & 3) * 16 + li;
        if (m >= p.M) continue;
#pragma unroll
        for (int ci = 0; ci < 4; ++ci) {
          const int n = n0 + (ci >> 1) * 128 + wc * 32 + (ci & 1) * 16 + lg * 4;
          if (n >= p.N) continue;
          float v[4];
#pragma unroll
          for (int r = 0; r < 4; ++r) v[r] = acc[ri][ci][r] * p.alpha;
          if (n + 3 < p.N && vec_ok) {
            if (p.bias) {
              const u32x2_t bb = *(const u32x2_t*)(p.bias + n);
              v[0] += bflo(bb[0]); v[1] += bfhi(bb[0]); v[2] += bflo(bb[1]); v[3] += bfhi(bb[1]);
            }
            if (p.R) {
              const u32x2_t rr = *(const u32x2_t*)(p.R + (size_t)m * p.ldr + n);
              v[0] += bflo(rr[0]); v[1] += bfhi(rr[0]); v[2] += bflo(rr[1]); v[3] += bfhi(rr[1]);
            }
            if (p.out_fp32) {
              float* c = (float*)p.C + (size_t)m * p.ldc + n;
              f32x4_t o = {v[0], v[1], v[2], v[3]};
              if (p.accumulate) o += *(const f32x4_t*)c;
              *(f32x4_t*)c = o;
            } else {
              u32x2_t o;
              o[0] = pack2bf(v[0], v[1]);
              o[1] = pack2bf(v[2], v[3]);
              *(u32x2_t*)((bf16_t*)p.C + (size_t)m * p.ldc + n) = o;
            }
          } else {
            for (int r = 0; r < 4 && n + r < p.N; ++r) {
              float xv = v[r];
              if (p.bias) xv += bf2f(p.bias[n + r]);
              if (p.R) xv += bf2f(p.R[(size_t)m * p.ldr + n + r]);
              if (p.out_fp32) {
                float* c = (float*)p.C + (size_t)m * p.ldc + n + r;
                *c = p.accumulate ? (*c + xv) : xv;
              } else {
                ((bf16_t*)p.C)[(size_t)m * p.ldc + n + r] = f2bf(xv);
              }
            }
          }
        }
      }
    }
#pragma unroll
    for (int a = 0; a < 8; ++a)
#pragma unroll
      for (int c = 0; c < 4; ++c) acc[a][c] = f32x4_t{0.f, 0.f, 0.f, 0.f};
  };

  ST_A0(); ST_B0(); ST_B1(); ST_A1(); ST_A0(); ST_B0();
  asm volatile("s_waitcnt vmcnt(8)" ::: "memory");
  __builtin_amdgcn_s_barrier();
  PREAD_B(fb0, smem + SB0)
  if (wr == 1) __builtin_amdgcn_s_barrier();

  int ci_unit = 0, c_left = cu.nt;
  for (;;) {
    PTILE(fb0, fb1, 0)
    if (--c_left == 0) {
      epilogue();
      if (++ci_unit == n_units) break;
      cu = get_unit(ci_unit);
      c_left = cu.nt;
    }
    PTILE(fb1, fb0, 1)
    if (--c_left == 0) {
      epilogue();
      if (++ci_unit == n_units) break;
      cu = get_unit(ci_unit);
      c_left = cu.nt;
    }
  }
  if (wr == 0) __builtin_amdgcn_s_barrier();
  asm volatile("s_waitcnt vmcnt(0)" ::: "memory");
#undef PTILE
#undef PMMA
#undef PSEG_END
#undef PREAD_A
#undef PREAD_B
#undef PSTAGE
#undef PSLOT_SET
#undef ST_A0
#undef ST_A1
#undef ST_B0
#undef ST_B1
}

#endif

__global__ __launch_bounds__(256) void gemm256_fixup_kernel(GemmArgs p) {
  const int GROUP_M = MLA_GROUP_M;
  const int num_m = (p.M + 255) / 256, num_n = (p.N + 255) / 256;
  const int tile = blockIdx.x >> 6;
  const int pid = p.sk_full + tile;
  const int in_group = GROUP_M * num_n;
  const int group_id = pid / in_group;
  const int first_m = group_id * GROUP_M;
  const int gsz = (num_m - first_m) < GROUP_M ? (num_m - first_m) : GROUP_M;
  const int pid_m = first_m + (pid % in_group) % gsz, pid_n = (pid % in_group) / gsz;
  const int e = ((blockIdx.x & 63) * 256 + threadIdx.x) * 4;
  const int ml = e >> 8, nl = e & 255;
  const int m = pid_m * 256 + ml, n = pid_n * 256 + nl;
  if (p.sq_out) {
    __shared__ float sq_s[16];
    float sq = 0.f;
    if (m < p.M && n < p.N) {
      const float* src = p.sk_ws + (size_t)tile * p.sk_split * 65536 + ml * 256 + nl;
      f32x4_t a = *(const f32x4_t*)src;
      for (int sl = 1; sl < p.sk_split; ++sl) a += *(const f32x4_t*)(src + (size_t)sl * 65536);
      f32x4_t o = a * p.alpha;
      if (p.bias) { const u32x2_t bb = *(const u32x2_t*)(p.bias + n); o[0] += bflo(bb[0]); o[1] += bfhi(bb[0]); o[2] += bflo(bb[1]); o[3] += bfhi(bb[1]); }
      if (p.R) { const u32x2_t rr = *(const u32x2_t*)(p.R + (size_t)m * p.ldr + n); o[0] += bflo(rr[0]); o[1] += bfhi(rr[0]); o[2] += bflo(rr[1]); o[3] += bfhi(rr[1]); }
      float* c = (float*)p.C + (size_t)m * p.ldc + n;
      if (p.accumulate) o += *(const f32x4_t*)c;
      *(f32x4_t*)c = o;
      sq = (o[0] * o[0] + o[1] * o[1]) + (o[2] * o[2] + o[3] * o[3]);
    }
    sq = block_sum(sq, sq_s);
    if (threadIdx.x == 0) p.sq_out[p.sk_full + blockIdx.x] = sq;
    return;
  }
  if (m >= p.M || n >= p.N) return;
  const float* src = p.sk_ws + (size_t)tile * p.sk_split * 65536 + ml * 256 + nl;
  f32x4_t a = *(const f32x4_t*)src;
  for (int sl = 1; sl < p.sk_split; ++sl) a += *(const f32x4_t*)(src + (size_t)sl * 65536);
  float v[4] = {a[0] * p.alpha, a[1] * p.alpha, a[2] * p.alpha, a[3] * p.alpha};
  const bool vec_ok = ((p.ldc & 3) == 0) && (p.R == nullptr || (p.ldr & 3) == 0) && (n + 3 < p.N);
  for (int r = 0; r < 4 && n + r < p.N; ++r) {
    if (p.bias) v[r] += bf2f(p.bias[n + r]);
    if (p.R) v[r] += bf2f(p.R[(size_t)m * p.ldr + n + r]);
  }
  if (vec_ok) {
    if (p.out_fp32) {
      float* c = (float*)p.C + (size_t)m * p.ldc + n;
      f32x4_t o = {v[0], v[1], v[2], v[3]};
      if (p.accumulate) o += *(const f32x4_t*)c;
      *(f32x4_t*)c = o;
    } else {
      u32x2_t o;
      o[0] = pack2bf(v[0], v[1]);
      o[1] = pack2bf(v[2], v[3]);
      *(u32x2_t*)((bf16_t*)p.C + (size_t)m * p.ldc + n) = o;
      if (p.nrm_xg) {
        const u32x2_t gg = *(const u32x2_t*)(p.nrm_g + n);
        const float h0 = bflo(o[0]), h1 = bfhi(o[0]), h2 = bflo(o[1]), h3 = bfhi(o[1]);
        u32x2_t x;
        x[0] = pack2bf(h0 * bflo(gg[0]), h1 * bfhi(gg[0]));
        x[1] = pack2bf(h2 * bflo(gg[1]), h3 * bfhi(gg[1]));
        *(u32x2_t*)(p.nrm_xg + (size_t)m * p.ldc + n) = x;
        const float q = wave_sum((h0 * h0 + h1 * h1) + (h2 * h2 + h3 * h3));
        if ((threadIdx.x & 63) == 0) p.nrm_ss[(size_t)m * num_n + pid_n] = q;
      }
    }
  } else {
    for (int r = 0; r < 4 && n + r < p.N; ++r) {
      if (p.out_fp32) {
        float* c = (float*)p.C + (size_t)m * p.ldc + n + r;
        *c = p.accumulate ? (*c + v[r]) : v[r];
      } else {
        ((bf16_t*)p.C)[(size_t)m * p.ldc + n + r] = f2bf(v[r]);
      }
    }
  }
}

inline int choose_split(int tiles, int ncu, int nt, size_t ws_bytes, int* full_out) {
  const int r = tiles % ncu;
  *full_out = tiles - r;
  if (r == 0) return 1;
  int best = 1;
  double best_cost = 1.0;
  for (int s = 2; s <= 8; ++s) {
    if (nt / s < 8) break;
    if ((size_t)r * s * 65536 * sizeof(float) > ws_bytes) break;
    const double cost = (double)((r * s + ncu - 1) / ncu) / s + 0.04 + 0.01 * s;
    if (cost < best_cost - 1e-9) { best_cost = cost; best = s; }
  }
  return best;
}

int g_ncu_plan = -1;
int planned_cus(int device_cus) {
  if (g_ncu_plan < 0) {
    const char* e = getenv("MLA_GEMM_CUS");
    const int v = e ? atoi(e) : 0;
    g_ncu_plan = (v >= 8 && v % 8 == 0) ? v : 0;
  }
  return (g_ncu_plan > 0 && g_ncu_plan < device_cus) ? g_ncu_plan : device_cus;
}

int g_kloop = -1;
int kloop_mode() {
  if (g_kloop < 0) {
    const char* e = getenv("MLA_GEMM_KLOOP");
    g_kloop = (e && e[0] == '0') ? 0 : 1;
  }
  return g_kloop;
}

template <int EPI, int AM = 0, int BM_ = 0>
void launch_asm(const GemmArgs& p, dim3 grid, size_t lds, hipStream_t stream) {
  static bool attr = false;
  if (!attr) {
    hipFuncSetAttribute((const void*)gemm256_kernel<AM, BM_, EPI, true>, hipFuncAttributeMaxDynamicSharedMemorySize, (int)lds);
    attr = true;
  }
  hipLaunchKernelGGL((gemm256_kernel<AM, BM_, EPI, true>), grid, dim3(512), lds, stream, p);
}

template <int AM, int BM_>
int launch256(const GemmArgs& p, hipStream_t stream, int persistent_grid) {
  if constexpr (AM != 0 || BM_ != 0) {
    static bool attr_rm = false;
    if (!attr_rm) {
      hipFuncSetAttribute((const void*)gemm256_kernel<AM, BM_>, hipFuncAttributeMaxDynamicSharedMemorySize, 2 * BUF);
      attr_rm = true;
    }
    const int tiles = ((p.M + 255) / 256) * ((p.N + 255) / 256);
    const bool fast = (p.N & 7) == 0 && (p.ldc & 7) == 0 && (((uintptr_t)p.C) & 15) == 0 &&
                      (p.R == nullptr || ((p.ldr & 7) == 0 && (((uintptr_t)p.R) & 15) == 0)) && (p.bias == nullptr || (((uintptr_t)p.bias) & 15) == 0);
    if (p.sw_gu) {
      if constexpr (AM == 0 && BM_ == 1) {
        if (kloop_mode() && (p.K % 128) == 0) {
          launch_asm<2, 0, 1>(p, dim3(tiles), 2 * BUF + 32768, stream);
        } else {
          static bool attr_sw = false;
          if (!attr_sw) {
            hipFuncSetAttribute((const void*)gemm256_kernel<0, 1, 2>, hipFuncAttributeMaxDynamicSharedMemorySize, 2 * BUF + 32768);
            attr_sw = true;
          }
          hipLaunchKernelGGL((gemm256_kernel<0, 1, 2>), dim3(tiles), dim3(512), 2 * BUF + 32768, stream, p);
        }
      } else {
        mla_set_error("gemm256: the fused SwiGLU backward reads only its B operand reduction-major");
        return -1;
      }
    } else if (kloop_mode() && (p.K % 128) == 0 && fast) {
      if (p.sk_split > 1) {
        const int tail = tiles - p.sk_full;
        launch_asm<0, AM, BM_>(p, dim3(p.sk_full + tail * p.sk_split), 2 * BUF, stream);
        hipLaunchKernelGGL(gemm256_fixup_kernel, dim3(tail * 64), dim3(256), 0, stream, p);
      } else {
        launch_asm<0, AM, BM_>(p, dim3(tiles), 2 * BUF, stream);
      }
    } else if (p.sk_split > 1) {
      const int tail = tiles - p.sk_full;
      hipLaunchKernelGGL((gemm256_kernel<AM, BM_>), dim3(p.sk_full + tail * p.sk_split), dim3(512), 2 * BUF, stream, p);
      hipLaunchKernelGGL(gemm256_fixup_kernel, dim3(tail * 64), dim3(256), 0, stream, p);
    } else {
      hipLaunchKernelGGL((gemm256_kernel<AM, BM_>), dim3(tiles), dim3(512), 2 * BUF, stream, p);
    }
    hipError_t e = hipGetLastError();
    if (e != hipSuccess) {
      mla_set_error("gemm256 launch failed: %s", hipGetErrorString(e));
      return (int)e;
    }
    return 0;
  } else {
  static bool attr_set = false;
  if (!attr_set) {
    hipFuncSetAttribute((const void*)gemm256_kernel<AM, BM_>, hipFuncAttributeMaxDynamicSharedMemorySize, 2 * BUF + 1024);
    attr_set = true;
  }
  const int num_m = (p.M + 255) / 256, num_n = (p.N + 255) / 256;
  const bool fast = (p.N & 7) == 0 && (p.ldc & 7) == 0 && (((uintptr_t)p.C) & 15) == 0 &&
                    (p.R == nullptr || ((p.ldr & 7) == 0 && (((uintptr_t)p.R) & 15) == 0)) && (p.bias == nullptr || (((uintptr_t)p.bias) & 15) == 0);
  if (kloop_mode() && (p.K % 128) == 0 && fast && persistent_grid <= 0) {
    if (p.sk_split > 1) {
      const int tail = num_m * num_n - p.sk_full;
      launch_asm<0>(p, dim3(p.sk_full + tail * p.sk_split), 2 * BUF + 1024, stream);
      hipLaunchKernelGGL(gemm256_fixup_kernel, dim3(tail * 64), dim3(256), 0, stream, p);
    } else if (p.sw_gu) {
      launch_asm<2>(p, dim3(num_m * num_n), 2 * BUF + 32768, stream);
    } else if (p.sf_I) {
      launch_asm<1>(p, dim3(num_m * num_n), 2 * BUF + 1024, stream);
    } else {
      launch_asm<0>(p, dim3(num_m * num_n), 2 * BUF + 1024, stream);
    }
    hipError_t e = hipGetLastError();
    if (e != hipSuccess) {
      mla_set_error("gemm256 launch failed: %s", hipGetErrorString(e));
      return (int)e;
    }
    return 0;
  }
#ifdef MLA_EXPERIMENTAL_KERNELS
  if (AM == 0 && BM_ == 0 && persistent_grid > 0) {
    static bool attr_p = false;
    if (!attr_p) {
      hipFuncSetAttribute((const void*)gemm256p_kernel, hipFuncAttributeMaxDynamicSharedMemorySize, 2 * BUF);
      attr_p = true;
    }
    hipLaunchKernelGGL(gemm256p_kernel, dim3(persistent_grid), dim3(512), 2 * BUF, stream, p);
    if (p.sk_split > 1) hipLaunchKernelGGL(gemm256_fixup_kernel, dim3((num_m * num_n - p.sk_full) * 64), dim3(256), 0, stream, p);
  } else
#endif
  if (p.sk_split > 1) {
    const int tail = num_m * num_n - p.sk_full;
    hipLaunchKernelGGL((gemm256_kernel<AM, BM_>), dim3(p.sk_full + tail * p.sk_split), dim3(512), 2 * BUF + 1024, stream, p);
    hipLaunchKernelGGL(gemm256_fixup_kernel, dim3(tail * 64), dim3(256), 0, stream, p);
  } else if (p.sw_gu) {
    static bool attr_sw = false;
    if (!attr_sw) {
      hipFuncSetAttribute((const void*)gemm256_kernel<AM, BM_, 2>, hipFuncAttributeMaxDynamicSharedMemorySize, 2 * BUF + 32768);
      attr_sw = true;
    }
    hipLaunchKernelGGL((gemm256_kernel<AM, BM_, 2>), dim3(num_m * num_n), dim3(512), 2 * BUF + 32768, stream, p);
  } else if (p.sf_I) {
    static bool attr_sf = false;
    if (!attr_sf) {
      hipFuncSetAttribute((const void*)gemm256_kernel<AM, BM_, 1>, hipFuncAttributeMaxDynamicSharedMemorySize, 2 * BUF + 1024);
      attr_sf = true;
    }
    hipLaunchKernelGGL((gemm256_kernel<AM, BM_, 1>), dim3(num_m * num_n), dim3(512), 2 * BUF + 1024, stream, p);
  } else {
    hipLaunchKernelGGL((gemm256_kernel<AM, BM_>), dim3(num_m * num_n), dim3(512), 2 * BUF + 1024, stream, p);
  }
  hipError_t e = hipGetLastError();
  if (e != hipSuccess) {
    mla_set_error("gemm256 launch failed: %s", hipGetErrorString(e));
    return (int)e;
  }
  return 0;
  }
}

}

int mla_gemm256_dispatch(const void* args, int a_mode, int b_mode, size_t ws_bytes, hipStream_t stream, int* sq_slots = nullptr);

extern "C" int mla_gemm_kloop(int mode) {
  if (mode == 0 || mode == 1) g_kloop = mode;
  return kloop_mode();
}

extern "C" int mla_gemm_qkv_rope(const void* A, const void* B, void* C, int M, int N, int K, int lda, int ldb, int ldc,
                                 const float* rope_cos, const float* rope_sin, int S, int rope_cols, hipStream_t stream) {
  MLA_CHECK_ARG(A && B && C && rope_cos && rope_sin, "mla_gemm_qkv_rope: null pointer");
  MLA_CHECK_ARG(M >= 256 && N >= 256 && K > 0 && K % 64 == 0 && N % 8 == 0, "mla_gemm_qkv_rope: needs M, N >= 256, K %% 64 == 0, N %% 8 == 0");
  MLA_CHECK_ARG(S > 0 && rope_cols > 0 && rope_cols % 256 == 0 && rope_cols <= N, "mla_gemm_qkv_rope: rope_cols must be a multiple of 256 (two heads of 128) and <= N");
  MLA_CHECK_ARG(lda >= K && ldb >= K && ldc >= N && lda % 8 == 0 && ldb % 8 == 0 && ldc % 8 == 0, "mla_gemm_qkv_rope: leading dimensions must be multiples of 8");
  MLA_CHECK_ARG(((((uintptr_t)A) | ((uintptr_t)B) | ((uintptr_t)C) | ((uintptr_t)rope_cos) | ((uintptr_t)rope_sin)) & 15) == 0,
                "mla_gemm_qkv_rope: 16-B alignment required");
  GemmArgs p{};
  p.A = (const bf16_t*)A; p.B = (const bf16_t*)B; p.C = C; p.M = M; p.N = N; p.K = K; p.lda = lda; p.ldb = ldb; p.ldc = ldc;
  p.alpha = 1.f;
  p.rope_cos = rope_cos; p.rope_sin = rope_sin; p.rope_S = S; p.rope_cols = rope_cols;
  return mla_gemm256_dispatch(&p, 0, 0, 0, stream);
}

extern "C" int mla_gemm_gateup_swiglu(const void* x, const void* wgu, void* gu, void* act, void* actT, int M, int I, int K, int lda,
                                      int ldb, long long ldt, hipStream_t stream) {
  MLA_CHECK_ARG(x && wgu && (act || actT) && (gu || act), "mla_gemm_gateup_swiglu: null pointer (act may be NULL only when actT is given, gu only when act is)");
  MLA_CHECK_ARG(M >= 256 && I >= 128 && I % 128 == 0 && K > 0 && K % 64 == 0, "mla_gemm_gateup_swiglu: needs M >= 256, I %% 128 == 0, K %% 64 == 0");
  MLA_CHECK_ARG(lda >= K && ldb >= K && lda % 8 == 0 && ldb % 8 == 0, "mla_gemm_gateup_swiglu: leading dimensions must be multiples of 8");
  MLA_CHECK_ARG(actT == nullptr || (M % 8 == 0 && ldt >= M && ldt % 8 == 0), "mla_gemm_gateup_swiglu: transposed output needs M %% 8 == 0, ldt >= M, ldt %% 8 == 0");
  MLA_CHECK_ARG(((((uintptr_t)x) | ((uintptr_t)wgu) | ((uintptr_t)gu) | ((uintptr_t)act) | ((uintptr_t)actT)) & 15) == 0,
                "mla_gemm_gateup_swiglu: 16-B alignment required");
  GemmArgs p{};
  p.A = (const bf16_t*)x; p.B = (const bf16_t*)wgu; p.C = gu; p.M = M; p.N = 2 * I; p.K = K; p.lda = lda; p.ldb = ldb; p.ldc = 2 * I;
  p.alpha = 1.f;
  p.sf_I = I; p.sf_act = (bf16_t*)act; p.sf_actT = (bf16_t*)actT; p.sf_ldt = ldt;
  return mla_gemm256_dispatch(&p, 0, 0, 0, stream);
}

extern "C" int mla_gemm_dact_swiglu_bwd(const void* dy, const void* wT, const void* gu, void* dgu, void* dguT, int M, int I, int K,
                                        int lda, int ldb, long long ldt, hipStream_t stream) {
  MLA_CHECK_ARG(dy && wT && gu && dgu, "mla_gemm_dact_swiglu_bwd: null pointer");
  MLA_CHECK_ARG(M >= 256 && I >= 256 && K > 0 && K % 64 == 0 && I % 8 == 0 && M % 8 == 0,
                "mla_gemm_dact_swiglu_bwd: needs M, I >= 256, K %% 64 == 0, I %% 8 == 0, M %% 8 == 0");
  MLA_CHECK_ARG(lda >= K && ldb >= K && lda % 8 == 0 && ldb % 8 == 0 && ldt >= M && ldt % 8 == 0,
                "mla_gemm_dact_swiglu_bwd: leading dimensions must be multiples of 8 (ldt >= M)");
  MLA_CHECK_ARG(((((uintptr_t)dy) | ((uintptr_t)wT) | ((uintptr_t)gu) | ((uintptr_t)dgu) | ((uintptr_t)dguT)) & 15) == 0,
                "mla_gemm_dact_swiglu_bwd: 16-B alignment required");
  GemmArgs p{};
  p.A = (const bf16_t*)dy; p.B = (const bf16_t*)wT; p.C = dgu ;
  p.M = M; p.N = I; p.K = K; p.lda = lda; p.ldb = ldb; p.ldc = 2 * I; p.alpha = 1.f;
  p.sw_gu = (const bf16_t*)gu; p.sw_dgu = (bf16_t*)dgu; p.sw_dguT = (bf16_t*)dguT; p.sw_I = I; p.sw_ldt = ldt;
  return mla_gemm256_dispatch(&p, 0, 0, 0, stream);
}

extern "C" int mla_gemm_dact_swiglu_bwd_rm(const void* dy, const void* w, const void* gu, void* dgu, void* dguT, int M, int I, int K,
                                           int lda, int ldb, long long ldt, hipStream_t stream) {
  MLA_CHECK_ARG(dy && w && gu && dgu, "mla_gemm_dact_swiglu_bwd_rm: null pointer");
  MLA_CHECK_ARG(M >= 256 && I >= 256 && K > 0 && K % 64 == 0 && I % 8 == 0 && M % 8 == 0,
                "mla_gemm_dact_swiglu_bwd_rm: needs M, I >= 256, K %% 64 == 0, I %% 8 == 0, M %% 8 == 0");
  MLA_CHECK_ARG(lda >= K && ldb >= I && lda % 8 == 0 && ldb % 8 == 0 && ldt >= M && ldt % 8 == 0,
                "mla_gemm_dact_swiglu_bwd_rm: leading dimensions must be multiples of 8 (lda >= K, ldb >= I, ldt >= M)");
  MLA_CHECK_ARG((size_t)64 * (size_t)ldb * 2 < 0x80000000ULL, "mla_gemm_dact_swiglu_bwd_rm: ldb too large (64 weight rows must span < 2 GiB)");
  MLA_CHECK_ARG(((((uintptr_t)dy) | ((uintptr_t)w) | ((uintptr_t)gu) | ((uintptr_t)dgu) | ((uintptr_t)dguT)) & 15) == 0,
                "mla_gemm_dact_swiglu_bwd_rm: 16-B alignment required");
  GemmArgs p{};
  p.A = (const bf16_t*)dy; p.B = (const bf16_t*)w; p.C = dgu ;
  p.M = M; p.N = I; p.K = K; p.lda = lda; p.ldb = ldb; p.ldc = 2 * I; p.alpha = 1.f;
  p.sw_gu = (const bf16_t*)gu; p.sw_dgu = (bf16_t*)dgu; p.sw_dguT = (bf16_t*)dguT; p.sw_I = I; p.sw_ldt = ldt;
  return mla_gemm256_dispatch(&p, 0, 1, 0, stream);
}

extern "C" int mla_gemm_res_norm(const void* A, const void* B, void* C, const void* R, const void* g, void* xg, float* ss, int M, int N,
                                 int K, int lda, int ldb, int ldc, int ldr, float* workspace, size_t workspace_bytes, hipStream_t stream) {
  MLA_CHECK_ARG(A && B && C && R && g && xg && ss, "mla_gemm_res_norm: null pointer");
  MLA_CHECK_ARG(M >= 256 && N >= 256 && N % 256 == 0 && K > 0 && K % 64 == 0, "mla_gemm_res_norm: needs M >= 256, N %% 256 == 0, K %% 64 == 0");
  MLA_CHECK_ARG(lda >= K && ldb >= K && ldc >= N && ldr >= N && lda % 8 == 0 && ldb % 8 == 0 && ldc % 8 == 0 && ldr % 8 == 0,
                "mla_gemm_res_norm: leading dimensions must be multiples of 8");
  MLA_CHECK_ARG(((((uintptr_t)A) | ((uintptr_t)B) | ((uintptr_t)C) | ((uintptr_t)R) | ((uintptr_t)g) | ((uintptr_t)xg) | ((uintptr_t)ss) |
                  ((uintptr_t)workspace)) & 15) == 0, "mla_gemm_res_norm: 16-B alignment required");
  GemmArgs p{};
  p.A = (const bf16_t*)A; p.B = (const bf16_t*)B; p.C = C; p.R = (const bf16_t*)R; p.M = M; p.N = N; p.K = K;
  p.lda = lda; p.ldb = ldb; p.ldc = ldc; p.ldr = ldr; p.alpha = 1.f;
  p.sk_ws = workspace;
  p.nrm_g = (const bf16_t*)g; p.nrm_xg = (bf16_t*)xg; p.nrm_ss = ss;
  return mla_gemm256_dispatch(&p, 0, 0, workspace ? workspace_bytes : 0, stream);
}

static int rs_args(GemmArgs& p, const float* ss, int parts, float eps, float* rstd, const char* who) {
  MLA_CHECK_ARG(rstd != nullptr && (ss == nullptr || parts > 0), "%s: null rstd / bad partial count", who);
  p.rs_ss = ss; p.rs_parts = parts; p.rs_eps = eps; p.rs_rstd = rstd;
  return 0;
}

extern "C" int mla_gemm_qkv_rope_rs(const void* A, const void* B, void* C, int M, int N, int K, int lda, int ldb, int ldc,
                                    const float* rope_cos, const float* rope_sin, int S, int rope_cols, const float* ss, int parts,
                                    float eps, float* rstd, hipStream_t stream) {
  MLA_CHECK_ARG(A && B && C && rope_cos && rope_sin, "mla_gemm_qkv_rope_rs: null pointer");
  MLA_CHECK_ARG(M >= 256 && N >= 256 && K > 0 && K % 64 == 0 && N % 8 == 0, "mla_gemm_qkv_rope_rs: needs M, N >= 256, K %% 64 == 0, N %% 8 == 0");
  MLA_CHECK_ARG(S > 0 && rope_cols > 0 && rope_cols % 256 == 0 && rope_cols <= N, "mla_gemm_qkv_rope_rs: rope_cols must be a multiple of 256 (two heads of 128) and <= N");
  MLA_CHECK_ARG(lda >= K && ldb >= K && ldc >= N && lda % 8 == 0 && ldb % 8 == 0 && ldc % 8 == 0, "mla_gemm_qkv_rope_rs: leading dimensions must be multiples of 8");
  MLA_CHECK_ARG(((((uintptr_t)A) | ((uintptr_t)B) | ((uintptr_t)C) | ((uintptr_t)rope_cos) | ((uintptr_t)rope_sin)) & 15) == 0,
                "mla_gemm_qkv_rope_rs: 16-B alignment required");
  GemmArgs p{};
  p.A = (const bf16_t*)A; p.B = (const bf16_t*)B; p.C = C; p.M = M; p.N = N; p.K = K; p.lda = lda; p.ldb = ldb; p.ldc = ldc;
  p.alpha = 1.f;
  p.rope_cos = rope_cos; p.rope_sin = rope_sin; p.rope_S = S; p.rope_cols = rope_cols;
  if (int rc = rs_args(p, ss, parts, eps, rstd, "mla_gemm_qkv_rope_rs")) return rc;
  return mla_gemm256_dispatch(&p, 0, 0, 0, stream);
}

extern "C" int mla_gemm_gateup_swiglu_rs(const void* x, const void* wgu, void* gu, void* act, void* actT, int M, int I, int K, int lda,
                                         int ldb, long long ldt, const float* ss, int parts, float eps, float* rstd, hipStream_t stream) {
  MLA_CHECK_ARG(x && wgu && (act || actT) && (gu || act), "mla_gemm_gateup_swiglu_rs: null pointer (act may be NULL only when actT is given, gu only when act is)");
  MLA_CHECK_ARG(M >= 256 && I >= 128 && I % 128 == 0 && K > 0 && K % 64 == 0, "mla_gemm_gateup_swiglu_rs: needs M >= 256, I %% 128 == 0, K %% 64 == 0");
  MLA_CHECK_ARG(lda >= K && ldb >= K && lda % 8 == 0 && ldb % 8 == 0, "mla_gemm_gateup_swiglu_rs: leading dimensions must be multiples of 8");
  MLA_CHECK_ARG(actT == nullptr || (M % 8 == 0 && ldt >= M && ldt % 8 == 0), "mla_gemm_gateup_swiglu_rs: transposed output needs M %% 8 == 0, ldt >= M, ldt %% 8 == 0");
  MLA_CHECK_ARG(((((uintptr_t)x) | ((uintptr_t)wgu) | ((uintptr_t)gu) | ((uintptr_t)act) | ((uintptr_t)actT)) & 15) == 0,
                "mla_gemm_gateup_swiglu_rs: 16-B alignment required");
  GemmArgs p{};
  p.A = (const bf16_t*)x; p.B = (const bf16_t*)wgu; p.C = gu; p.M = M; p.N = 2 * I; p.K = K; p.lda = lda; p.ldb = ldb; p.ldc = 2 * I;
  p.alpha = 1.f;
  p.sf_I = I; p.sf_act = (bf16_t*)act; p.sf_actT = (bf16_t*)actT; p.sf_ldt = ldt;
  if (int rc = rs_args(p, ss, parts, eps, rstd, "mla_gemm_gateup_swiglu_rs")) return rc;
  return mla_gemm256_dispatch(&p, 0, 0, 0, stream);
}

extern "C" int mla_gemm_cus(int n) {
  if (n >= 0) {
    if (n != 0 && (n < 8 || n % 8 != 0 || n > 1024)) return -1;
    g_ncu_plan = n;
  } else if (g_ncu_plan < 0) {
    (void)planned_cus(1 << 20);
  }
  return g_ncu_plan;
}
extern "C" int mla_gemm_sq_slots(int M, int N, int K, size_t workspace_bytes) {
  if (M < 256 || N < 256 || K <= 0 || (K % 64) != 0 || (N % 8) != 0) return -1;
  int ncu = 0, dev = 0;
  (void)hipGetDevice(&dev);
  (void)hipDeviceGetAttribute(&ncu, hipDeviceAttributeMultiprocessorCount, dev);
  if (ncu <= 0) ncu = 256;
  const int tiles = ((M + 255) / 256) * ((N + 255) / 256);
  if (workspace_bytes) {
    int full = 0;
    const int s = choose_split(tiles, planned_cus(ncu), K / 64, workspace_bytes, &full);
    if (s > 1 && full % 8 == 0) return full + (tiles - full) * 64;
  }
  return tiles;
}

int mla_gemm256_dispatch(const void* args, int a_mode, int b_mode, size_t ws_bytes, hipStream_t stream, int* sq_slots) {
  GemmArgs p = *(const GemmArgs*)args;
  if ((a_mode != 0 || b_mode != 0) && (p.sf_I || p.rope_cos || (p.sw_gu && !(a_mode == 0 && b_mode == 1)))) {
    mla_set_error("gemm256: the fused epilogues take k-contiguous operands only (SwiGLU backward: or B reduction-major)");
    return -1;
  }
  p.sk_split = 1;
  p.sk_full = 0;
  if (p.nrm_xg || p.rs_rstd) {
    const bool fast = (p.N & 7) == 0 && (p.ldc & 7) == 0 && (((uintptr_t)p.C) & 15) == 0 &&
                      (p.R == nullptr || ((p.ldr & 7) == 0 && (((uintptr_t)p.R) & 15) == 0)) && p.bias == nullptr && !p.out_fp32;
    const bool ok = fast && a_mode == 0 && b_mode == 0 && p.alpha == 1.f &&
                    (p.nrm_xg ? (p.R != nullptr && p.N % 256 == 0 && !p.rs_rstd && !p.sf_I && !p.sw_gu && !p.rope_cos) : (p.R == nullptr && !p.sw_gu));
    if (!ok) {
      mla_set_error("gemm256: the folded-RMSNorm forms need bf16 k-contiguous operands, alpha 1 and the whole-row epilogue");
      return -1;
    }
  }
  static int ncu = 0, persist = -1;
  if (!ncu) {
    int dev = 0;
    (void)hipGetDevice(&dev);
    (void)hipDeviceGetAttribute(&ncu, hipDeviceAttributeMultiprocessorCount, dev);
    if (ncu <= 0) ncu = 256;
    const char* e = getenv("MLA_GEMM_PERSIST");
    persist = (e && e[0] == '1') ? 1 : 0;
  }
#ifdef MLA_EXPERIMENTAL_KERNELS
  if (p.sf_I || p.sw_gu) {
    static int st_mode = -1, st_ticks = 0;
    if (st_mode < 0) {
      const char* e = getenv("MLA_GEMM_STAGGER");
      st_mode = 0;
      if (e && sscanf(e, "%d:%d", &st_mode, &st_ticks) != 2) st_mode = 0;
    }
    p.stagger_mode = st_mode;
    p.stagger_ticks = st_ticks;
  }
#endif
  const int tiles = ((p.M + 255) / 256) * ((p.N + 255) / 256);
  if (p.sq_out) {
    const bool ok = p.out_fp32 && !p.sf_I && !p.sw_gu && !p.rope_cos && (p.N & 7) == 0 && (p.ldc & 7) == 0 &&
                    (((uintptr_t)p.C) & 15) == 0 && (p.R == nullptr || ((p.ldr & 7) == 0 && (((uintptr_t)p.R) & 15) == 0)) &&
                    (p.bias == nullptr || (((uintptr_t)p.bias) & 15) == 0);
    if (!ok) {
      mla_set_error("gemm256: sum-of-squares partials need an fp32, 8-column-aligned output of the plain kernel");
      return -1;
    }
  }
  if (p.sk_ws && ws_bytes) {
    int full = 0;
    const int s = choose_split(tiles, planned_cus(ncu), p.K / 64, ws_bytes, &full);
    if (s > 1 && full % 8 == 0) { p.sk_split = s; p.sk_full = full; }
  }
  const size_t bytesA = ((size_t)(p.M - 1) * p.lda + p.K) * 2, bytesB = ((size_t)(p.N - 1) * p.ldb + p.K) * 2;
  const int grid = ncu & ~7;
#ifndef MLA_EXPERIMENTAL_KERNELS
  if (p.debug & 0x100) { mla_set_error("gemm256: the persistent experiment kernel is not in this build (MLA_EXPERIMENTAL=1)"); return -1; }
  persist = 0;
#endif
  const bool use_p = (persist || (p.debug & 0x100)) && (p.debug & 0x80) == 0 && tiles > grid && bytesA < 0x7fffffffULL && bytesB < 0x7fffffffULL &&
                     p.sf_I == 0 && p.sw_gu == nullptr && p.rope_cos == nullptr && p.sq_out == nullptr && p.nrm_xg == nullptr && p.rs_rstd == nullptr;
  if (sq_slots) *sq_slots = p.sk_split > 1 ? p.sk_full + (tiles - p.sk_full) * 64 : tiles;
  if (a_mode == 0 && b_mode == 1) return launch256<0, 1>(p, stream, 0);
  if (a_mode == 1 && b_mode == 0) return launch256<1, 0>(p, stream, 0);
  if (a_mode == 1 && b_mode == 1) return launch256<1, 1>(p, stream, 0);
  return launch256<0, 0>(p, stream, use_p ? grid : 0);
}
```

### mla_amd/hip.py

```python
from __future__ import annotations

import ctypes
import os
from ctypes import c_float, c_int, c_longlong, c_size_t, c_void_p
from typing import NamedTuple, Optional

import torch

_LIB_PATH = os.environ.get("MLA_HIP_LIB") or os.path.join(os.path.dirname(os.path.abspath(__file__)), "libmla_hip.so")
_lib = None

ACT_GELU_ERF, ACT_GELU_TANH, ACT_RELU, ACT_SILU = 0, 1, 2, 3

SPLITK = os.environ.get("MLA_GEMM_SPLITK", "1") != "0"
SPLITK_WS_BYTES = int(os.environ.get("MLA_GEMM_SPLITK_WS_MB", "64")) << 20

GEMM_PROFILE = None

_SIGNATURES = {
    "mla_query": [c_int],
    "mla_selftest": [c_void_p, c_void_p, c_void_p, c_void_p],
    "mla_dispatch_probe": [c_void_p, c_int, c_int, c_void_p],
    "mla_calib_mfma": [c_void_p, c_void_p, c_int, c_int, c_void_p, c_void_p],
    "mla_gemv_bf16": [c_void_p, c_longlong, c_void_p, c_longlong, c_void_p, c_longlong, c_longlong, c_int, c_void_p, c_longlong, c_int, c_int,
                      c_int, c_int, c_void_p, c_float, c_void_p, c_void_p, c_int, c_void_p],
    "mla_attn_decode": [c_void_p, c_void_p, c_void_p, c_void_p, c_int, c_int, c_int, c_int, c_int, c_longlong, c_longlong, c_longlong, c_float,
                        c_void_p],
    "mla_gemm_skinny_bf16": [c_void_p, c_longlong, c_void_p, c_longlong, c_void_p, c_longlong, c_longlong, c_int, c_void_p, c_longlong, c_int,
                             c_int, c_int, c_int, c_void_p, c_float, c_void_p, c_void_p, c_int, c_void_p],
    "mla_quant_fp8_rows": [c_void_p, c_longlong, c_void_p, c_longlong, c_void_p, c_int, c_int, c_void_p],
    "mla_gemv_w8": [c_void_p, c_longlong, c_void_p, c_longlong, c_void_p, c_void_p, c_longlong, c_longlong, c_int, c_void_p, c_longlong, c_int,
                    c_int, c_int, c_int, c_void_p, c_float, c_void_p, c_void_p, c_int, c_void_p],
    "mla_gemm_skinny_w8": [c_void_p, c_longlong, c_void_p, c_longlong, c_void_p, c_void_p, c_longlong, c_longlong, c_int, c_void_p, c_longlong,
                           c_int, c_int, c_int, c_int, c_void_p, c_float, c_void_p, c_void_p, c_int, c_void_p],
    "mla_attn_chunk": [c_void_p, c_void_p, c_void_p, c_void_p, c_int, c_int, c_int, c_int, c_int, c_longlong, c_longlong, c_longlong, c_float,
                       c_void_p],
    "mla_attn_chunk_ragged": [c_void_p, c_void_p, c_void_p, c_void_p, c_int, c_int, c_int, c_void_p, c_int, c_int, c_longlong, c_longlong,
                              c_longlong, c_float, c_void_p],
    "mla_attn_chunk_groups": [c_void_p, c_void_p, c_void_p, c_void_p, c_int, c_int, c_int, c_int, c_int, c_longlong, c_longlong, c_float,
                              c_void_p],
    "mla_attn_chunk_groups_gw": [c_void_p, c_void_p, c_void_p, c_void_p, c_int, c_int, c_int, c_int, c_int, c_longlong, c_longlong, c_float,
                                 c_int, c_int, c_void_p],
    "mla_gemm_suffix_bf16": [c_void_p, c_longlong, c_void_p, c_longlong, c_void_p, c_longlong, c_longlong, c_int, c_void_p, c_int, c_void_p,
                             c_longlong, c_int, c_int, c_int, c_void_p, c_void_p, c_int, c_void_p],
    "mla_gemm_suffix_w8": [c_void_p, c_longlong, c_void_p, c_longlong, c_void_p, c_void_p, c_longlong, c_longlong, c_int, c_void_p, c_int,
                           c_void_p, c_longlong, c_int, c_int, c_int, c_void_p, c_void_p, c_int, c_void_p],
    "mla_attn_chunk_ragged_groups": [c_void_p, c_void_p, c_void_p, c_void_p, c_int, c_int, c_int, c_int, c_void_p, c_int, c_int, c_longlong,
                                     c_longlong, c_longlong, c_float, c_void_p],
    "mla_attn_chunk_ragged_groups_gw": [c_void_p, c_void_p, c_void_p, c_void_p, c_int, c_int, c_int, c_int, c_void_p, c_int, c_int, c_longlong,
                                        c_longlong, c_longlong, c_float, c_int, c_int, c_void_p],
    "mla_gemm_suffix_bf16_pos": [c_void_p, c_longlong, c_void_p, c_longlong, c_void_p, c_longlong, c_longlong, c_int, c_void_p, c_int, c_void_p,
                                 c_longlong, c_int, c_int, c_int, c_void_p, c_void_p, c_int, c_void_p, c_int, c_void_p],
    "mla_gemm_suffix_w8_pos": [c_void_p, c_longlong, c_void_p, c_longlong, c_void_p, c_void_p, c_longlong, c_longlong, c_int, c_void_p, c_int,
                               c_void_p, c_longlong, c_int, c_int, c_int, c_void_p, c_void_p, c_int, c_void_p, c_int, c_void_p],
    "mla_gemm_prefill_plan": [c_int, c_int, c_int, c_int, c_void_p],
    "mla_gemm_prefill_ws_bytes": [c_int, c_int, c_int],
    "mla_gemm_prefill_bf16": [c_void_p, c_longlong, c_void_p, c_longlong, c_void_p, c_longlong, c_longlong, c_int, c_void_p, c_longlong, c_int,
                              c_int, c_int, c_void_p, c_size_t, c_void_p],
    "mla_gemm_prefill_qkv_rope": [c_void_p, c_longlong, c_void_p, c_longlong, c_void_p, c_longlong, c_longlong, c_int, c_int, c_int, c_int,
                                  c_void_p, c_void_p, c_int, c_int, c_void_p, c_size_t, c_void_p],
    "mla_gemm_prefill_gateup_swiglu": [c_void_p, c_longlong, c_void_p, c_longlong, c_void_p, c_longlong, c_longlong, c_int, c_int, c_int,
                                       c_int, c_void_p, c_size_t, c_void_p],
    "mla_gemm_prefill_f8_plan": [c_int, c_int, c_int, c_int, c_void_p],
    "mla_gemm_prefill_f8_ws_bytes": [c_int, c_int, c_int],
    "mla_gemm_prefill_f8": [c_void_p, c_longlong, c_void_p, c_void_p, c_longlong, c_void_p, c_void_p, c_longlong, c_longlong, c_int, c_void_p,
                            c_longlong, c_int, c_int, c_int, c_void_p, c_size_t, c_void_p],
    "mla_gemm_prefill_f8_qkv_rope": [c_void_p, c_longlong, c_void_p, c_void_p, c_longlong, c_void_p, c_void_p, c_longlong, c_longlong, c_int,
                                     c_int, c_int, c_int, c_void_p, c_void_p, c_int, c_int, c_void_p, c_size_t, c_void_p],
    "mla_gemm_prefill_f8_gateup_swiglu": [c_void_p, c_longlong, c_void_p, c_void_p, c_longlong, c_void_p, c_void_p, c_longlong, c_longlong,
                                          c_int, c_int, c_int, c_int, c_void_p, c_size_t, c_void_p],
    "mla_gemm_prefill_f8_wide_plan": [c_int, c_int, c_int, c_int, c_void_p],
    "mla_gemm_prefill_f8_wide_ws_bytes": [c_int, c_int, c_int],
    "mla_gemm_prefill_f8_wide": [c_void_p, c_longlong, c_void_p, c_void_p, c_longlong, c_void_p, c_void_p, c_longlong, c_longlong, c_int,
                                 c_void_p, c_longlong, c_int, c_int, c_int, c_void_p, c_size_t, c_void_p],
    "mla_gemm_prefill_f8_wide_qkv_rope": [c_void_p, c_longlong, c_void_p, c_void_p, c_longlong, c_void_p, c_void_p, c_longlong, c_longlong,
                                          c_int, c_int, c_int, c_int, c_void_p, c_void_p, c_int, c_int, c_void_p, c_size_t, c_void_p],
    "mla_gemm_prefill_f8_wide_gateup_swiglu": [c_void_p, c_longlong, c_void_p, c_void_p, c_longlong, c_void_p, c_void_p, c_longlong,
                                               c_longlong, c_int, c_int, c_int, c_int, c_void_p, c_size_t, c_void_p],
    "mla_ddim_step": [c_void_p, c_void_p, c_void_p, c_void_p, c_void_p, c_int, c_int, c_int, c_void_p],
    "mla_ddpm_step": [c_void_p, c_void_p, c_void_p, c_void_p, c_void_p, c_void_p, c_int, c_int, c_int, c_void_p],
    "mla_sampler_rows": [c_void_p, c_void_p, c_void_p, c_void_p, c_int, c_int, c_int, c_int, c_void_p],
    "mla_attn_chunk_split_plan": [c_int, c_int, c_int, c_int, c_int, c_void_p],
    "mla_attn_chunk_split_ws_bytes": [c_int, c_int, c_int, c_int, c_int],
    "mla_attn_chunk_split": [c_void_p, c_void_p, c_void_p, c_void_p, c_int, c_int, c_int, c_int, c_int, c_longlong, c_longlong, c_longlong,
                             c_float, c_int, c_void_p, c_size_t, c_void_p],
    "mla_attn_groups_split": [c_void_p, c_void_p, c_void_p, c_void_p, c_int, c_int, c_int, c_int, c_void_p, c_int, c_int, c_longlong, c_longlong,
                              c_longlong, c_float, c_int, c_void_p, c_size_t, c_void_p],
    "mla_gemm_bf16": [c_void_p, c_void_p, c_void_p, c_void_p, c_void_p, c_int, c_int, c_int, c_int, c_int, c_int, c_int,
                      c_int, c_int, c_int, c_int, c_float, c_int, c_void_p],
    "mla_gemm_bf16_ws": [c_void_p, c_void_p, c_void_p, c_void_p, c_void_p, c_int, c_int, c_int, c_int, c_int, c_int, c_int,
                         c_int, c_int, c_int, c_int, c_float, c_int, c_void_p, c_size_t, c_void_p],
    "mla_gemm_qkv_rope": [c_void_p, c_void_p, c_void_p, c_int, c_int, c_int, c_int, c_int, c_int, c_void_p, c_void_p, c_int, c_int,
                          c_void_p],
    "mla_gemm_bf16_ws_sq": [c_void_p, c_void_p, c_void_p, c_int, c_int, c_int, c_int, c_int, c_int, c_int, c_float, c_void_p, c_size_t,
                            c_void_p, c_int, c_void_p, c_void_p],
    "mla_gemm_bf16_ws_sq_rm": [c_void_p, c_void_p, c_void_p, c_int, c_int, c_int, c_int, c_int, c_int, c_int, c_int, c_int, c_float, c_void_p,
                               c_size_t, c_void_p, c_int, c_void_p, c_void_p],
    "mla_sum_partials": [c_void_p, c_int, c_void_p, c_int, c_void_p],
    "mla_gemm_sq_slots": [c_int, c_int, c_int, c_size_t],
    "mla_gemm_kloop": [c_int],
    "mla_gemm_cus": [c_int],
    "mla_side_traffic": [c_void_p, c_void_p, c_void_p, c_longlong, c_int, c_int, c_int, c_void_p],
    "mla_gemm_gateup_swiglu": [c_void_p, c_void_p, c_void_p, c_void_p, c_void_p, c_int, c_int, c_int, c_int, c_int, c_longlong,
                               c_void_p],
    "mla_gemm_dact_swiglu_bwd": [c_void_p, c_void_p, c_void_p, c_void_p, c_void_p, c_int, c_int, c_int, c_int, c_int, c_longlong,
                                 c_void_p],
    "mla_gemm_dact_swiglu_bwd_rm": [c_void_p, c_void_p, c_void_p, c_void_p, c_void_p, c_int, c_int, c_int, c_int, c_int, c_longlong,
                                    c_void_p],
    "mla_rmsnorm_fwd": [c_void_p, c_void_p, c_void_p, c_void_p, c_int, c_int, c_float, c_void_p],
    "mla_rmsnorm_apply": [c_void_p, c_void_p, c_void_p, c_void_p, c_longlong, c_int, c_void_p],
    "mla_rmsnorm_prep": [c_void_p, c_void_p, c_void_p, c_void_p, c_int, c_int, c_float, c_void_p],
    "mla_gemm_res_norm": [c_void_p, c_void_p, c_void_p, c_void_p, c_void_p, c_void_p, c_void_p, c_int, c_int, c_int, c_int, c_int, c_int,
                          c_int, c_void_p, c_size_t, c_void_p],
    "mla_gemm_qkv_rope_rs": [c_void_p, c_void_p, c_void_p, c_int, c_int, c_int, c_int, c_int, c_int, c_void_p, c_void_p, c_int, c_int,
                             c_void_p, c_int, c_float, c_void_p, c_void_p],
    "mla_gemm_gateup_swiglu_rs": [c_void_p, c_void_p, c_void_p, c_void_p, c_void_p, c_int, c_int, c_int, c_int, c_int, c_longlong,
                                  c_void_p, c_int, c_float, c_void_p, c_void_p],
    "mla_rmsnorm_bwd_blocks": [c_int],
    "mla_timm_rmsnorm_fwd": [c_void_p, c_void_p, c_void_p, c_void_p, c_void_p, c_int, c_int, c_float, c_void_p],
    "mla_timm_rmsnorm_bwd": [c_void_p, c_void_p, c_void_p, c_void_p, c_void_p, c_void_p, c_void_p, c_int, c_int, c_int, c_void_p,
                             c_size_t, c_void_p],
    "mla_rmsnorm_bwd": [c_void_p, c_void_p, c_void_p, c_void_p, c_void_p, c_void_p, c_void_p, c_int, c_int, c_int, c_void_p,
                        c_size_t, c_void_p],
    "mla_colsum_blocks": [c_int],
    "mla_colsum_bf16": [c_void_p, c_void_p, c_int, c_int, c_int, c_int, c_void_p, c_size_t, c_void_p],
    "mla_layernorm_fwd": [c_void_p, c_void_p, c_void_p, c_void_p, c_int, c_int, c_float, c_void_p],
    "mla_rope_inplace": [c_void_p, c_void_p, c_void_p, c_longlong, c_int, c_int, c_int, c_int, c_int, c_int, c_int, c_void_p],
    "mla_swiglu_fwd": [c_void_p, c_void_p, c_longlong, c_int, c_void_p],
    "mla_swiglu_bwd": [c_void_p, c_void_p, c_void_p, c_void_p, c_longlong, c_int, c_void_p],
    "mla_act_fwd": [c_void_p, c_void_p, c_longlong, c_int, c_void_p],
    "mla_act_bwd": [c_void_p, c_void_p, c_void_p, c_longlong, c_int, c_void_p],
    "mla_cast_f32_to_bf16": [c_void_p, c_void_p, c_longlong, c_void_p],
    "mla_cast_bf16_to_f32": [c_void_p, c_void_p, c_longlong, c_void_p],
    "mla_add_bf16": [c_void_p, c_void_p, c_void_p, c_longlong, c_void_p],
    "mla_embedding_fwd": [c_void_p, c_void_p, c_void_p, c_longlong, c_int, c_int, c_void_p],
    "mla_embedding_bwd": [c_void_p, c_void_p, c_void_p, c_void_p, c_longlong, c_int, c_int, c_void_p],
    "mla_adamw_step_groups": [c_void_p, c_void_p, c_void_p, c_void_p, c_void_p, c_longlong, c_longlong, c_float, c_float, c_float, c_float,
                              c_float, c_int, c_void_p, c_void_p],
    "mla_adamw_step": [c_void_p, c_void_p, c_void_p, c_void_p, c_void_p, c_longlong, c_float, c_float, c_float, c_float,
                       c_float, c_int, c_void_p, c_void_p],
    "mla_sumsq_f32": [c_void_p, c_longlong, c_void_p, c_int, c_void_p, c_size_t, c_void_p],
    "mla_clip_coef": [c_void_p, c_float, c_void_p, c_void_p, c_void_p],
    "mla_q_sample": [c_void_p, c_void_p, c_void_p, c_void_p, c_void_p, c_void_p, c_int, c_int, c_int, c_void_p],
    "mla_attn_fwd": [c_void_p, c_void_p, c_void_p, c_void_p, c_void_p, c_void_p, c_int, c_int, c_int, c_int, c_longlong,
                     c_longlong, c_float, c_void_p],
    "mla_attn_bwd": [c_void_p, c_void_p, c_void_p, c_void_p, c_void_p, c_void_p, c_void_p, c_void_p, c_void_p, c_void_p,
                     c_void_p, c_int, c_int, c_int, c_int, c_longlong, c_longlong, c_float, c_void_p, c_void_p, c_void_p, c_longlong,
                     c_void_p],
    "mla_attn_bwd_t": [c_void_p, c_void_p, c_void_p, c_void_p, c_void_p, c_void_p, c_void_p, c_void_p, c_void_p, c_void_p,
                       c_void_p, c_int, c_int, c_int, c_int, c_longlong, c_longlong, c_float, c_void_p, c_void_p,
                       c_void_p, c_void_p, c_void_p, c_void_p, c_longlong, c_void_p, c_longlong, c_void_p],
    "mla_attn_bwd_sync_ints": [c_int, c_int],
    "mla_attn_fwd_g": [c_void_p, c_void_p, c_void_p, c_void_p, c_void_p, c_void_p, c_int, c_int, c_int, c_int, c_longlong,
                       c_longlong, c_float, c_int, c_int, c_void_p, c_void_p],
    "mla_attn_bwd_g": [c_void_p, c_void_p, c_void_p, c_void_p, c_void_p, c_void_p, c_void_p, c_void_p, c_void_p, c_void_p,
                       c_void_p, c_int, c_int, c_int, c_int, c_longlong, c_longlong, c_float, c_void_p, c_void_p,
                       c_void_p, c_void_p, c_void_p, c_void_p, c_longlong, c_void_p, c_longlong, c_int, c_int, c_void_p, c_int, c_void_p],
    "mla_attn_bwd_ws_bytes": [c_int, c_int, c_int],
    "mla_attn_bwd_ws": [c_void_p, c_void_p, c_void_p, c_void_p, c_void_p, c_void_p, c_void_p, c_void_p, c_void_p, c_void_p,
                        c_void_p, c_int, c_int, c_int, c_int, c_longlong, c_longlong, c_float, c_void_p, c_void_p,
                        c_void_p, c_void_p, c_void_p, c_void_p, c_longlong, c_void_p, c_longlong, c_void_p],
    "mla_ce_fwd": [c_void_p, c_int, c_longlong, c_void_p, c_void_p, c_void_p, c_int, c_int, c_longlong, c_void_p],
    "mla_ce_bwd": [c_void_p, c_int, c_longlong, c_void_p, c_void_p, c_void_p, c_float, c_void_p, c_longlong, c_int, c_int,
                   c_longlong, c_void_p],
    "mla_infonce_bwd": [c_void_p, c_void_p, c_void_p, c_void_p, c_void_p, c_int, c_int, c_void_p],
    "mla_l2norm_fwd": [c_void_p, c_void_p, c_void_p, c_int, c_int, c_float, c_void_p],
    "mla_l2norm_bwd": [c_void_p, c_void_p, c_void_p, c_void_p, c_int, c_int, c_void_p],
}


def exported_symbols():
    return sorted(list(_SIGNATURES.keys()) + ["mla_last_error", "mla_gemm_source_id"] + list(_EXTRA_SIGNATURES.keys()))


_EXTRA_SIGNATURES = {}


def register_signatures(sigs):
    _EXTRA_SIGNATURES.update(sigs)
    global _lib
    if _lib is not None:
        for name, argt in sigs.items():
            fn = getattr(_lib, name)
            fn.argtypes = argt
            fn.restype = c_int


def lib():
    global _lib
    if _lib is None:
        if not os.path.exists(_LIB_PATH):
            raise RuntimeError(
                f"{_LIB_PATH} not found: build it with `python -c 'import __graft_entry__ as g; g.build()'` "
                "(mla_amd has no CPU fallback)")
        L = ctypes.CDLL(_LIB_PATH)
        L.mla_last_error.restype = ctypes.c_char_p
        L.mla_last_error.argtypes = []
        L.mla_gemm_source_id.restype = ctypes.c_char_p
        L.mla_gemm_source_id.argtypes = []
        for name, argt in {**_SIGNATURES, **_EXTRA_SIGNATURES}.items():
            fn = getattr(L, name)
            fn.argtypes = argt
            fn.restype = c_int
        L.mla_attn_bwd_ws_bytes.restype = c_longlong
        L.mla_attn_bwd_sync_ints.restype = c_longlong
        L.mla_gemm_prefill_ws_bytes.restype = c_longlong
        L.mla_gemm_prefill_f8_ws_bytes.restype = c_longlong
        L.mla_gemm_prefill_f8_wide_ws_bytes.restype = c_longlong
        L.mla_attn_chunk_split_ws_bytes.restype = c_longlong
        _lib = L
    return _lib


def gemm_cus(n: int = -1) -> int:
    return lib().mla_gemm_cus(n)


def side_traffic(a32, b32, out32, blocks: int, lds_bytes: int = 0, sleep_ticks: int = 0):
    call("mla_side_traffic", _p(a32), _p(b32), _p(out32), a32.numel(), blocks, lds_bytes, sleep_ticks)


def gemm_source_id() -> str:
    return lib().mla_gemm_source_id().decode()


def _stream():
    return c_void_p(torch.cuda.current_stream().cuda_stream)


def _p(t: Optional[torch.Tensor]):
    return None if t is None else c_void_p(t.data_ptr())


def _check(rc: int, name: str):
    if rc != 0:
        raise RuntimeError(f"{name} failed (rc={rc}): {lib().mla_last_error().decode()}")


def _req(t: torch.Tensor, dtype, name: str):
    if t.dtype != dtype:
        raise TypeError(f"{name}: expected {dtype}, got {t.dtype}")
    if not t.is_cuda:
        raise RuntimeError(f"{name}: tensor must live on the GPU (mla_amd has no CPU path)")


def call(name: str, *args):
    rc = getattr(lib(), name)(*args, _stream())
    _check(rc, name)


_ws_cache = {}


def workspace(nbytes: int, device) -> torch.Tensor:
    key = (str(device), torch.cuda.current_stream().cuda_stream)
    buf = _ws_cache.get(key)
    if buf is None or buf.numel() < nbytes:
        buf = torch.empty(max(nbytes, 1 << 24), dtype=torch.uint8, device=device)
        _ws_cache[key] = buf
    return buf


def gemm(a: torch.Tensor, b: torch.Tensor, out: Optional[torch.Tensor] = None, *, a_mode: int = 0, b_mode: int = 0,
         M: Optional[int] = None, N: Optional[int] = None, K: Optional[int] = None, lda: Optional[int] = None,
         ldb: Optional[int] = None, ldc: Optional[int] = None, bias: Optional[torch.Tensor] = None,
         residual: Optional[torch.Tensor] = None, ldr: Optional[int] = None, out_dtype=torch.bfloat16,
         accumulate: bool = False, alpha: float = 1.0, force_generic: int = 0) -> torch.Tensor:
    _req(a, torch.bfloat16, "gemm a")
    _req(b, torch.bfloat16, "gemm b")
    assert a.dim() == 2 and b.dim() == 2 and a.stride(1) == 1 and b.stride(1) == 1
    if M is None:
        M = a.shape[0] if a_mode == 0 else a.shape[1]
    if K is None:
        K = a.shape[1] if a_mode == 0 else a.shape[0]
    if N is None:
        N = b.shape[0] if b_mode == 0 else b.shape[1]
    kb = b.shape[1] if b_mode == 0 else b.shape[0]
    if kb != K:
        raise ValueError(f"gemm: reduction mismatch {K} vs {kb}")
    lda = a.stride(0) if lda is None else lda
    ldb = b.stride(0) if ldb is None else ldb
    if out is None:
        out = torch.empty((M, N), dtype=out_dtype, device=a.device)
    assert out.stride(-1) == 1
    out_fp32 = 1 if out.dtype == torch.float32 else 0
    if not out_fp32:
        _req(out, torch.bfloat16, "gemm out")
    ldc = out.stride(0) if ldc is None else ldc
    if residual is not None:
        _req(residual, torch.bfloat16, "gemm residual")
        ldr = residual.stride(0) if ldr is None else ldr
    if bias is not None:
        _req(bias, torch.bfloat16, "gemm bias")
    prof = GEMM_PROFILE
    if prof is not None:
        ev0, ev1 = torch.cuda.Event(enable_timing=True), torch.cuda.Event(enable_timing=True)
        ev0.record()
    if SPLITK and (force_generic & 15) == 0 and M >= 256 and N >= 256:
        ws = workspace(SPLITK_WS_BYTES, a.device)
        call("mla_gemm_bf16_ws", _p(a), _p(b), _p(out), _p(residual), _p(bias), M, N, K, lda, ldb, ldc, ldr or 0, a_mode, b_mode,
             out_fp32, 1 if accumulate else 0, float(alpha), int(force_generic), _p(ws), SPLITK_WS_BYTES)
    else:
        call("mla_gemm_bf16", _p(a), _p(b), _p(out), _p(residual), _p(bias), M, N, K, lda, ldb, ldc, ldr or 0, a_mode, b_mode,
             out_fp32, 1 if accumulate else 0, float(alpha), int(force_generic))
    if prof is not None:
        ev1.record()
        prof.append((ev0, ev1, 2.0 * M * N * K, (a_mode, b_mode, M, N, K)))
    return out


def gemm_kloop(mode: int = -1) -> int:
    return int(lib().mla_gemm_kloop(int(mode)))


def gemm_sq_slots(a: torch.Tensor, b: torch.Tensor, out: torch.Tensor, a_mode: int = 0, b_mode: int = 0) -> int:
    M, K = a.shape if a_mode == 0 else (a.shape[1], a.shape[0])
    N, kb = b.shape if b_mode == 0 else (b.shape[1], b.shape[0])
    ok = (a.dtype == torch.bfloat16 and b.dtype == torch.bfloat16 and out.dtype == torch.float32 and kb == K and
          (a_mode == 0 or M % 8 == 0) and
          a.stride(1) == 1 and b.stride(1) == 1 and out.stride(1) == 1 and M >= 256 and N >= 256 and K % 64 == 0 and N % 8 == 0 and
          a.stride(0) % 8 == 0 and b.stride(0) % 8 == 0 and out.stride(0) % 8 == 0 and
          all(t.data_ptr() % 16 == 0 for t in (a, b, out)) and tuple(out.shape) == (M, N))
    if not ok:
        return -1
    return int(lib().mla_gemm_sq_slots(M, N, K, SPLITK_WS_BYTES if SPLITK else 0))


def gemm_sq(a: torch.Tensor, b: torch.Tensor, out: torch.Tensor, accumulate: bool, part: Optional[torch.Tensor] = None,
            a_mode: int = 0, b_mode: int = 0):
    need = gemm_sq_slots(a, b, out, a_mode, b_mode)
    if need < 0:
        return None
    M, K = a.shape if a_mode == 0 else (a.shape[1], a.shape[0])
    N = b.shape[0] if b_mode == 0 else b.shape[1]
    if part is None:
        part = torch.empty(need, dtype=torch.float32, device=out.device)
    assert part.dtype == torch.float32 and part.is_contiguous() and part.numel() >= need
    slots = ctypes.c_int(0)
    ws = workspace(SPLITK_WS_BYTES, a.device) if SPLITK else None
    prof = GEMM_PROFILE
    if prof is not None:
        ev0, ev1 = torch.cuda.Event(enable_timing=True), torch.cuda.Event(enable_timing=True)
        ev0.record()
    if a_mode or b_mode:
        call("mla_gemm_bf16_ws_sq_rm", _p(a), _p(b), _p(out), M, N, K, a.stride(0), b.stride(0), out.stride(0), int(a_mode), int(b_mode),
             1 if accumulate else 0, 1.0, _p(ws), SPLITK_WS_BYTES if ws is not None else 0, _p(part), part.numel(), ctypes.byref(slots))
    else:
        call("mla_gemm_bf16_ws_sq", _p(a), _p(b), _p(out), M, N, K, a.stride(0), b.stride(0), out.stride(0), 1 if accumulate else 0, 1.0,
             _p(ws), SPLITK_WS_BYTES if ws is not None else 0, _p(part), part.numel(), ctypes.byref(slots))
    assert int(slots.value) == need
    if prof is not None:
        ev1.record()
        prof.append((ev0, ev1, 2.0 * M * N * K, (a_mode, b_mode, M, N, K)))
    return part, need


def sum_partials(partials: torch.Tensor, n: int, out1: torch.Tensor, accumulate: bool):
    call("mla_sum_partials", _p(partials), int(n), _p(out1), 1 if accumulate else 0)


def _rs_args(norm, rows, device):
    ss, rstd, eps = norm
    if ss is not None:
        assert ss.dtype == torch.float32 and ss.is_contiguous() and ss.shape[0] == rows
        rstd = torch.empty(rows, dtype=torch.float32, device=device)
        return ss, int(ss.shape[1]), float(eps), rstd
    assert rstd is not None and rstd.dtype == torch.float32 and rstd.is_contiguous() and rstd.numel() == rows
    return None, 0, float(eps), rstd


def qkv_rope_ok(x2d, wqkv, out, cos, sin, S, rope_cols) -> bool:
    T, K = x2d.shape
    N = wqkv.shape[0]
    return (T >= 256 and N >= 256 and K % 64 == 0 and N % 8 == 0 and rope_cols % 256 == 0 and x2d.stride(0) % 8 == 0 and
            wqkv.stride(0) % 8 == 0 and out.stride(0) % 8 == 0 and cos.dtype == torch.float32 and cos.is_contiguous() and
            sin.is_contiguous() and cos.shape == (S, 64) and all(t.data_ptr() % 16 == 0 for t in (x2d, wqkv, out, cos, sin)))


def gemm_qkv_rope(x2d, wqkv, out, cos, sin, S, rope_cols, norm=None):
    T, K = x2d.shape
    N = wqkv.shape[0]
    ok = qkv_rope_ok(x2d, wqkv, out, cos, sin, S, rope_cols)
    if not ok:
        return False
    if norm is not None:
        _req(x2d, torch.bfloat16, "gemm_qkv_rope x")
        _req(wqkv, torch.bfloat16, "gemm_qkv_rope w")
        ss, parts, eps, rstd = _rs_args(norm, T, x2d.device)
        prof = GEMM_PROFILE
        if prof is not None:
            ev0, ev1 = torch.cuda.Event(enable_timing=True), torch.cuda.Event(enable_timing=True)
            ev0.record()
        call("mla_gemm_qkv_rope_rs", _p(x2d), _p(wqkv), _p(out), T, N, K, x2d.stride(0), wqkv.stride(0), out.stride(0), _p(cos), _p(sin),
             int(S), int(rope_cols), _p(ss), parts, eps, _p(rstd))
        if prof is not None:
            ev1.record()
            prof.append((ev0, ev1, 2.0 * T * N * K, (0, 0, T, N, K, "rope_epilogue")))
        return rstd
    _req(x2d, torch.bfloat16, "gemm_qkv_rope x")
    _req(wqkv, torch.bfloat16, "gemm_qkv_rope w")
    prof = GEMM_PROFILE
    if prof is not None:
        ev0, ev1 = torch.cuda.Event(enable_timing=True), torch.cuda.Event(enable_timing=True)
        ev0.record()
    call("mla_gemm_qkv_rope", _p(x2d), _p(wqkv), _p(out), T, N, K, x2d.stride(0), wqkv.stride(0), out.stride(0), _p(cos), _p(sin),
         int(S), int(rope_cols))
    if prof is not None:
        ev1.record()
        prof.append((ev0, ev1, 2.0 * T * N * K, (0, 0, T, N, K, "rope_epilogue")))
    return True


def gateup_swiglu_ok(x2d, wgu, want_t) -> bool:
    T, K = x2d.shape
    I = wgu.shape[0] // 2
    return (T >= 256 and I % 128 == 0 and K % 64 == 0 and wgu.shape[0] == 2 * I and x2d.stride(0) % 8 == 0 and wgu.stride(0) % 8 == 0 and
            (not want_t or T % 8 == 0) and all(t.data_ptr() % 16 == 0 for t in (x2d, wgu)))


def gemm_gateup_swiglu(x2d, wgu, want_t, norm=None, want_act=True, want_gu=True):
    T, K = x2d.shape
    I = wgu.shape[0] // 2
    ok = gateup_swiglu_ok(x2d, wgu, want_t)
    if not ok:
        return None
    _req(x2d, torch.bfloat16, "gemm_gateup_swiglu x")
    _req(wgu, torch.bfloat16, "gemm_gateup_swiglu w")
    act = torch.empty((T, I), dtype=torch.bfloat16, device=x2d.device) if (want_act or not want_t) else None
    gu = torch.empty((T, 2 * I), dtype=torch.bfloat16, device=x2d.device) if (want_gu or act is None) else None
    actT = torch.empty((I, T), dtype=torch.bfloat16, device=x2d.device) if want_t else None
    prof = GEMM_PROFILE
    if prof is not None:
        ev0, ev1 = torch.cuda.Event(enable_timing=True), torch.cuda.Event(enable_timing=True)
        ev0.record()
    rstd = None
    if norm is not None:
        ss, parts, eps, rstd = _rs_args(norm, T, x2d.device)
        call("mla_gemm_gateup_swiglu_rs", _p(x2d), _p(wgu), _p(gu), _p(act), _p(actT), T, I, K, x2d.stride(0), wgu.stride(0), T,
             _p(ss), parts, eps, _p(rstd))
    else:
        call("mla_gemm_gateup_swiglu", _p(x2d), _p(wgu), _p(gu), _p(act), _p(actT), T, I, K, x2d.stride(0), wgu.stride(0), T)
    if prof is not None:
        ev1.record()
        prof.append((ev0, ev1, 2.0 * T * 2 * I * K, (0, 0, T, 2 * I, K, "swiglu_fwd_epilogue")))
    return (gu, act, actT) if norm is None else (gu, act, actT, rstd)


def gemm_dact_swiglu_bwd(dy2d, wT, gu2d, want_t=True):
    T, K = dy2d.shape
    I = wT.shape[0]
    ok = (T >= 256 and I >= 256 and K % 64 == 0 and I % 8 == 0 and T % 8 == 0 and gu2d.shape == (T, 2 * I) and gu2d.is_contiguous() and
          dy2d.stride(0) % 8 == 0 and wT.stride(0) % 8 == 0 and all(t.data_ptr() % 16 == 0 for t in (dy2d, wT, gu2d)))
    if not ok:
        return None
    _req(dy2d, torch.bfloat16, "gemm_dact_swiglu_bwd dy")
    _req(wT, torch.bfloat16, "gemm_dact_swiglu_bwd wT")
    dgu = torch.empty_like(gu2d)
    dguT = torch.empty((2 * I, T), dtype=torch.bfloat16, device=gu2d.device) if want_t else None
    prof = GEMM_PROFILE
    if prof is not None:
        ev0, ev1 = torch.cuda.Event(enable_timing=True), torch.cuda.Event(enable_timing=True)
        ev0.record()
    call("mla_gemm_dact_swiglu_bwd", _p(dy2d), _p(wT), _p(gu2d), _p(dgu), _p(dguT), T, I, K, dy2d.stride(0), wT.stride(0), T)
    if prof is not None:
        ev1.record()
        prof.append((ev0, ev1, 2.0 * T * I * K, (0, 0, T, I, K, "swiglu_bwd_epilogue")))
    return dgu, dguT


def dact_swiglu_bwd_rm_ok(dy2d, w, gu2d) -> bool:
    T, K = dy2d.shape
    I = w.shape[1]
    return (T >= 256 and I >= 256 and K % 64 == 0 and I % 8 == 0 and T % 8 == 0 and w.shape[0] == K and w.stride(1) == 1 and
            gu2d.shape == (T, 2 * I) and gu2d.is_contiguous() and dy2d.stride(1) == 1 and dy2d.stride(0) % 8 == 0 and
            w.stride(0) % 8 == 0 and all(t.data_ptr() % 16 == 0 for t in (dy2d, w, gu2d)))


def gemm_dact_swiglu_bwd_rm(dy2d, w, gu2d, want_t=True, dgu=None, dguT=None):
    T, K = dy2d.shape
    I = w.shape[1]
    for t, nm in ((dy2d, "dy"), (w, "w"), (gu2d, "gu")):
        _req(t, torch.bfloat16, "gemm_dact_swiglu_bwd_rm " + nm)
    if w.shape[0] != K or w.stride(1) != 1 or dy2d.stride(1) != 1 or gu2d.shape != (T, 2 * I) or not gu2d.is_contiguous():
        raise ValueError("gemm_dact_swiglu_bwd_rm: needs dy [T, K], w [K, I] (unit column stride), gu [T, 2I] contiguous")
    if dgu is None:
        dgu = torch.empty_like(gu2d)
    if dguT is None and want_t:
        dguT = torch.empty((2 * I, T), dtype=torch.bfloat16, device=gu2d.device)
    if not want_t:
        dguT = None
    for t, shp, nm in ((dgu, (T, 2 * I), "dgu"), (dguT, (2 * I, T), "dguT")):
        if t is not None and (t.shape != shp or not t.is_contiguous() or t.dtype != torch.bfloat16):
            raise ValueError(f"gemm_dact_swiglu_bwd_rm: {nm} must be a contiguous bf16 {shp}")
    prof = GEMM_PROFILE
    if prof is not None:
        ev0, ev1 = torch.cuda.Event(enable_timing=True), torch.cuda.Event(enable_timing=True)
        ev0.record()
    call("mla_gemm_dact_swiglu_bwd_rm", _p(dy2d), _p(w), _p(gu2d), _p(dgu), _p(dguT), T, I, K, dy2d.stride(0), w.stride(0), T)
    if prof is not None:
        ev1.record()
        prof.append((ev0, ev1, 2.0 * T * I * K, (0, 1, T, I, K, "swiglu_bwd_epilogue")))
    return dgu, dguT


def rmsnorm_fwd(x2d, w, eps):
    _req(x2d, torch.bfloat16, "rmsnorm x")
    _req(w, torch.bfloat16, "rmsnorm w")
    rows, H = x2d.shape
    y = torch.empty_like(x2d)
    rstd = torch.empty(rows, dtype=torch.float32, device=x2d.device)
    call("mla_rmsnorm_fwd", _p(x2d), _p(w), _p(y), _p(rstd), rows, H, float(eps))
    return y, rstd


def rmsnorm_prep(x2d, w, eps, want_rstd=True):
    _req(x2d, torch.bfloat16, "rmsnorm_prep x")
    _req(w, torch.bfloat16, "rmsnorm_prep w")
    rows, H = x2d.shape
    xg = torch.empty_like(x2d)
    rstd = torch.empty(rows, dtype=torch.float32, device=x2d.device) if want_rstd else None
    call("mla_rmsnorm_prep", _p(x2d), _p(w), _p(xg), _p(rstd), rows, H, float(eps))
    return xg, rstd


def res_norm_ok(a, b, residual) -> bool:
    M, K = a.shape
    N = b.shape[0]
    return (M >= 256 and N >= 256 and N % 256 == 0 and K % 64 == 0 and a.stride(0) % 8 == 0 and b.stride(0) % 8 == 0 and
            residual.stride(0) % 8 == 0 and a.stride(1) == 1 and b.stride(1) == 1 and residual.stride(1) == 1 and
            all(t.data_ptr() % 16 == 0 for t in (a, b, residual)))


def gemm_res_norm(a, b, residual, g):
    _req(a, torch.bfloat16, "gemm_res_norm a")
    _req(b, torch.bfloat16, "gemm_res_norm b")
    _req(residual, torch.bfloat16, "gemm_res_norm residual")
    _req(g, torch.bfloat16, "gemm_res_norm g")
    M, K = a.shape
    N = b.shape[0]
    assert b.shape[1] == K and residual.shape == (M, N) and g.numel() == N and g.data_ptr() % 16 == 0
    h = torch.empty((M, N), dtype=torch.bfloat16, device=a.device)
    xg = torch.empty((M, N), dtype=torch.bfloat16, device=a.device)
    ss = torch.empty((M, N // 256), dtype=torch.float32, device=a.device)
    ws = workspace(SPLITK_WS_BYTES, a.device) if SPLITK else None
    prof = GEMM_PROFILE
    if prof is not None:
        ev0, ev1 = torch.cuda.Event(enable_timing=True), torch.cuda.Event(enable_timing=True)
        ev0.record()
    call("mla_gemm_res_norm", _p(a), _p(b), _p(h), _p(residual), _p(g), _p(xg), _p(ss), M, N, K, a.stride(0), b.stride(0), N,
         residual.stride(0), _p(ws), SPLITK_WS_BYTES if ws is not None else 0)
    if prof is not None:
        ev1.record()
        prof.append((ev0, ev1, 2.0 * M * N * K, (0, 0, M, N, K)))
    return h, xg, ss


def rmsnorm_bwd(dy, x2d, w, rstd, dres=None, dw_out=None, dw_accumulate=False):
    rows, H = x2d.shape
    dx = torch.empty_like(x2d)
    nb = lib().mla_rmsnorm_bwd_blocks(rows)
    ws = workspace(nb * H * 4, x2d.device) if dw_out is not None else None
    call("mla_rmsnorm_bwd", _p(dy), _p(x2d), _p(w), _p(rstd), _p(dres), _p(dx), _p(dw_out), 1 if dw_accumulate else 0, rows, H,
         _p(ws), ws.numel() if ws is not None else 0)
    return dx


def timm_rmsnorm_fwd(x2d, w, eps):
    _req(x2d, torch.bfloat16, "timm_rmsnorm x")
    _req(w, torch.bfloat16, "timm_rmsnorm w")
    rows, H = x2d.shape
    y = torch.empty_like(x2d)
    stats = torch.empty(2, rows, dtype=torch.float32, device=x2d.device)
    call("mla_timm_rmsnorm_fwd", _p(x2d), _p(w), _p(y), _p(stats[0]), _p(stats[1]), rows, H, float(eps))
    return y, stats[0], stats[1]


def timm_rmsnorm_bwd(dy, x2d, w, mean, rstd, dw_out=None, dw_accumulate=False):
    rows, H = x2d.shape
    dx = torch.empty_like(x2d)
    nb = lib().mla_rmsnorm_bwd_blocks(rows)
    ws = workspace(nb * H * 4, x2d.device) if dw_out is not None else None
    call("mla_timm_rmsnorm_bwd", _p(dy), _p(x2d), _p(w), _p(mean), _p(rstd), _p(dx), _p(dw_out), 1 if dw_accumulate else 0, rows, H,
         _p(ws), ws.numel() if ws is not None else 0)
    return dx


def colsum(dy2d, out_f32, accumulate):
    rows, N = dy2d.shape
    rs = lib().mla_colsum_blocks(rows)
    ws = workspace(rs * N * 4, dy2d.device)
    call("mla_colsum_bf16", _p(dy2d), _p(out_f32), 1 if accumulate else 0, rows, N, dy2d.stride(0), _p(ws), ws.numel())


def layernorm_fwd(x2d, w, b, eps):
    rows, H = x2d.shape
    y = torch.empty_like(x2d)
    call("mla_layernorm_fwd", _p(x2d), _p(w), _p(b), _p(y), rows, H, float(eps))
    return y


def rope_inplace(buf2d, cos, sin, S, nheads, D, q_off, k_off, backward=False):
    tokens = buf2d.shape[0]
    call("mla_rope_inplace", _p(buf2d), _p(cos), _p(sin), tokens, S, nheads, D, buf2d.stride(0), q_off, k_off,
         1 if backward else 0)


def swiglu_fwd(gu2d):
    rows, two_i = gu2d.shape
    act = torch.empty((rows, two_i // 2), dtype=torch.bfloat16, device=gu2d.device)
    call("mla_swiglu_fwd", _p(gu2d), _p(act), rows, two_i // 2)
    return act


def swiglu_bwd(dact, gu2d, want_act=False):
    rows, two_i = gu2d.shape
    dgu = torch.empty_like(gu2d)
    act = torch.empty_like(dact) if want_act else None
    call("mla_swiglu_bwd", _p(dact), _p(gu2d), _p(dgu), _p(act), rows, two_i // 2)
    return dgu, act


def swiglu_bwd_t(dact, gu2d):
    rows, two_i = gu2d.shape
    dgu = torch.empty_like(gu2d)
    dguT = torch.empty((two_i, rows), dtype=gu2d.dtype, device=gu2d.device)
    call("mla_swiglu_bwd_t", _p(dact), _p(gu2d), _p(dgu), _p(dguT), rows, two_i // 2, rows)
    return dgu, dguT


def act_fwd(x, kind):
    y = torch.empty_like(x)
    call("mla_act_fwd", _p(x), _p(y), x.numel(), kind)
    return y


def act_bwd(dy, x, kind):
    dx = torch.empty_like(x)
    call("mla_act_bwd", _p(dy), _p(x), _p(dx), x.numel(), kind)
    return dx


def cast_f32_to_bf16(x, out=None):
    if out is None:
        out = torch.empty(x.shape, dtype=torch.bfloat16, device=x.device)
    call("mla_cast_f32_to_bf16", _p(x), _p(out), x.numel())
    return out


def cast_bf16_to_f32(x, out=None):
    if out is None:
        out = torch.empty(x.shape, dtype=torch.float32, device=x.device)
    call("mla_cast_bf16_to_f32", _p(x), _p(out), x.numel())
    return out


def add_bf16(a, b):
    y = torch.empty_like(a)
    call("mla_add_bf16", _p(a), _p(b), _p(y), a.numel())
    return y


def embedding_fwd(ids, table):
    tokens = ids.numel()
    vocab, H = table.shape
    out = torch.empty((tokens, H), dtype=torch.bfloat16, device=table.device)
    call("mla_embedding_fwd", _p(ids), _p(table), _p(out), tokens, H, vocab)
    return out


def embedding_bwd(ids, dy2d, grad_f32):
    vocab, H = grad_f32.shape
    tokens = ids.numel()
    ws = torch.empty((tokens // 64, H), dtype=torch.float32, device=grad_f32.device) if tokens >= 64 else None
    call("mla_embedding_bwd", _p(ids), _p(dy2d), _p(grad_f32), _p(ws), tokens, H, vocab)


def adamw_step(p32, g32, m, v, p16, lr, beta1, beta2, eps, wd, step, grad_scale=None):
    call("mla_adamw_step", _p(p32), _p(g32), _p(m), _p(v), _p(p16), p32.numel(), float(lr), float(beta1), float(beta2),
         float(eps), float(wd), int(step), _p(grad_scale))


def adamw_step_groups(p32, g32, m, v, p16, n_decay, lr, beta1, beta2, eps, wd, step, grad_scale=None):
    call("mla_adamw_step_groups", _p(p32), _p(g32), _p(m), _p(v), _p(p16), p32.numel(), int(n_decay), float(lr), float(beta1), float(beta2),
         float(eps), float(wd), int(step), _p(grad_scale))


def sumsq(x32, out1, accumulate):
    ws = workspace(8192, x32.device)
    call("mla_sumsq_f32", _p(x32), x32.numel(), _p(out1), 1 if accumulate else 0, _p(ws), ws.numel())


def clip_coef(sumsq1, max_norm, coef1, norm1=None):
    call("mla_clip_coef", _p(sumsq1), float(max_norm), _p(coef1), _p(norm1))


def q_sample(x0, noise, t, sqrt_ac, sqrt_1mac):
    out = torch.empty_like(x0)
    batch = x0.shape[0]
    call("mla_q_sample", _p(x0), _p(noise), _p(t), _p(sqrt_ac), _p(sqrt_1mac), _p(out), batch, x0.numel() // batch,
         sqrt_ac.numel())
    return out


def _group_args(groups, B):
    start = groups[0]
    if torch.is_tensor(start):
        _req(start, torch.int32, "attention group starts")
        assert start.numel() == B and start.is_contiguous()
        return 0, start
    return int(start), None


def attn_fwd(q, k, v, B, S, H, D, ld_qkv, seqlens, scale, rows=None, groups=None):
    rows = B * S if rows is None else rows
    o = torch.empty((rows, H * D), dtype=torch.bfloat16, device=q.device)
    if rows > B * S:
        o[B * S:].zero_()
    lse = torch.empty((B, H, S), dtype=torch.float32, device=q.device)
    if groups is not None:
        gs, gst = _group_args(groups, B)
        call("mla_attn_fwd_g", _p(q), _p(k), _p(v), _p(o), _p(lse), _p(seqlens), B, S, H, D, ld_qkv, H * D, float(scale), gs, int(groups[1]), _p(gst))
    else:
        call("mla_attn_fwd", _p(q), _p(k), _p(v), _p(o), _p(lse), _p(seqlens), B, S, H, D, ld_qkv, H * D, float(scale))
    return o, lse


ATTN_BWD5 = os.environ.get("MLA_ATTN_BWD5", "0") == "1"


_HEAD_SYNC = {}
_DISPATCH_OK = {}
ATTN_BWD_MERGED = os.environ.get("MLA_ATTN_BWD_MERGED", "105") != "0"


def dispatch_probe(device="cuda", blocks=4096, hold_us=20):
    dev = torch.device(device)
    out = torch.zeros(1 + 2 * blocks, dtype=torch.int32, device=dev)
    call("mla_dispatch_probe", _p(out), blocks, hold_us)
    rec = out.cpu()[1:].view(blocks, 2)
    ticket, xcc = rec[:, 0].long(), rec[:, 1].long()
    ids = torch.arange(blocks)
    n_xcd = int(xcc.unique().numel())
    xcd_ok = bool((xcc == (ids & 7)).all())
    worst = 0
    for x in range(8):
        t = ticket[ids % 8 == x]
        rank = torch.argsort(torch.argsort(t))
        worst = max(worst, int((rank - torch.arange(t.numel())).abs().max()))
    info = {"xcds": n_xcd, "xcc_is_id_mod_8": xcd_ok, "worst_start_displacement": worst, "blocks": blocks,
            "tickets_complete": bool(torch.equal(torch.sort(ticket).values, ids))}
    return (n_xcd == 8 and xcd_ok and worst <= 128 and info["tickets_complete"]), info


def _head_sync(device, B, H):
    if not ATTN_BWD_MERGED:
        return None
    idx = device.index if device.index is not None else torch.cuda.current_device()
    if idx not in _DISPATCH_OK:
        if torch.cuda.is_current_stream_capturing():
            return None
        with torch.cuda.device(idx):
            _DISPATCH_OK[idx] = dispatch_probe(torch.device("cuda", idx))
    if not _DISPATCH_OK[idx][0]:
        return None
    need = int(lib().mla_attn_bwd_sync_ints(B, H))
    key = (idx, torch.cuda.current_stream(idx).cuda_stream)
    buf = _HEAD_SYNC.get(key)
    if buf is None or buf.numel() < need:
        if torch.cuda.is_current_stream_capturing():
            return None
        buf = torch.zeros(max(need, 4096), dtype=torch.int32, device=torch.device("cuda", idx))
        _HEAD_SYNC[key] = buf
    return buf


def attn_bwd(q, k, v, o, dout, lse, seqlens, dq, dk, dv, B, S, H, D, ld_qkv, scale, rope_cos=None, rope_sin=None, transposed=None,
             five: Optional[bool] = None, merged: Optional[bool] = None, groups=None):
    delta = torch.empty((B, H, S), dtype=torch.float32, device=q.device)
    five = ATTN_BWD5 if five is None else five
    if rope_cos is not None:
        _req(rope_cos, torch.float32, "rope cos")
        _req(rope_sin, torch.float32, "rope sin")
        assert rope_cos.shape in ((S, D // 2), (B * S, D // 2)) and rope_sin.shape == rope_cos.shape and rope_cos.is_contiguous() and rope_sin.is_contiguous()
        assert rope_cos.shape[0] == S or groups is not None, "per-sample RoPE tables [B * S, 64] go with mla_attn_bwd_g (groups=...)"
    if transposed is not None:
        dqkvT, oT = transposed
        _req(dqkvT, torch.bfloat16, "dqkvT")
        _req(oT, torch.bfloat16, "oT")
        ldt = dqkvT.stride(0)
        assert dqkvT.shape[0] == 3 * H * D and oT.shape[0] == H * D and oT.stride(0) == ldt and dqkvT.stride(1) == 1 and oT.stride(1) == 1
    if five:
        nbytes = int(lib().mla_attn_bwd_ws_bytes(B, S, H))
        ws = torch.empty(nbytes, dtype=torch.uint8, device=q.device)
        if transposed is not None:
            tq, tk, tv, to_ = dqkvT[:H * D], dqkvT[H * D:2 * H * D], dqkvT[2 * H * D:], oT
        else:
            tq = tk = tv = to_ = None
            ldt = 0
        call("mla_attn_bwd_ws", _p(q), _p(k), _p(v), _p(o), _p(dout), _p(lse), _p(seqlens), _p(dq), _p(dk), _p(dv), _p(delta), B, S,
             H, D, ld_qkv, H * D, float(scale), _p(rope_cos), _p(rope_sin), _p(tq), _p(tk), _p(tv), _p(to_), ldt, _p(ws), nbytes)
        return
# ... 1004 lines not shown
```

Measured before the change: 14.55 samples/s.

## Extend split-K tail balancing to fused SwiGLU forward and backward GEMMs

Lets the fused gate-up SwiGLU GEMM and the SwiGLU-backward GEMMs use the split-K tail scheme: leftover tiles that don't fill all CUs are split along K into fp32 workspace partials. New fixup kernels sum the partials and apply the SwiGLU forward or backward epilogue, including the transposed outputs. The goal is to cut wave quantization idle time on the last wave. It adds an extra fixup launch and workspace traffic. It is on by default only for gate-up; the dact path needs MLA_FUSED_TAIL=all.

```diff
diff --git a/include/mla_hip.h b/include/mla_hip.h
--- a/include/mla_hip.h
+++ b/include/mla_hip.h
@@ -42,6 +42,13 @@
                              int ldb, long long ldt, mla_stream_t stream);
 int mla_gemm_dact_swiglu_bwd_rm(const void* dy, const void* w, const void* gu, void* dgu, void* dguT, int M, int I, int K, int lda,
                                 int ldb, long long ldt, mla_stream_t stream);
+int mla_gemm_gateup_swiglu_ws(const void* x, const void* wgu, void* gu, void* act, void* actT, int M, int I, int K, int lda, int ldb,
+                              long long ldt, float* workspace, size_t workspace_bytes, mla_stream_t stream);
+int mla_gemm_dact_swiglu_bwd_ws(const void* dy, const void* wT, const void* gu, void* dgu, void* dguT, int M, int I, int K, int lda,
+                                int ldb, long long ldt, float* workspace, size_t workspace_bytes, mla_stream_t stream);
+int mla_gemm_dact_swiglu_bwd_rm_ws(const void* dy, const void* w, const void* gu, void* dgu, void* dguT, int M, int I, int K, int lda,
+                                   int ldb, long long ldt, float* workspace, size_t workspace_bytes, mla_stream_t stream);
+int mla_gemm_tail_plan(int M, int N, int K, size_t workspace_bytes, int swiglu_bwd_rm, int* full_tiles);
 
 int mla_gemm_res_norm(const void* A, const void* B, void* C, const void* R, const void* g, void* xg, float* ss, int M, int N, int K,
                       int lda, int ldb, int ldc, int ldr, float* workspace, size_t workspace_bytes, mla_stream_t stream);
diff --git a/mla_amd/csrc/gemm256.hip b/mla_amd/csrc/gemm256.hip
--- a/mla_amd/csrc/gemm256.hip
+++ b/mla_amd/csrc/gemm256.hip
@@ -41,6 +41,25 @@
     gi = (gi + 8 <= lim) ? gi : 0;
     return g + (size_t)kr * ld + gi;
   }
+}
+
+__device__ __forceinline__ u32x4_t swiglu_fwd8(const u32x4_t& g, const u32x4_t& u) {
+  float gv[8], uv[8], o[8];
+  unpack8(g, gv);
+  unpack8(u, uv);
+#pragma unroll
+  for (int j = 0; j < 8; ++j) o[j] = swiglu_fwd_elem(gv[j], uv[j]);
+  return pack8(o);
+}
+__device__ __forceinline__ void swiglu_bwd8(const u32x4_t& d, const u32x4_t& g, const u32x4_t& u, u32x4_t& dg, u32x4_t& du) {
+  float dv[8], gv[8], uv[8], og[8], ou[8];
+  unpack8(d, dv);
+  unpack8(g, gv);
+  unpack8(u, uv);
+#pragma unroll
+  for (int j = 0; j < 8; ++j) swiglu_bwd_elem(dv[j], gv[j], uv[j], og[j], ou[j]);
+  dg = pack8(og);
+  du = pack8(ou);
 }
 
 #ifndef MLA_GROUP_M
@@ -116,7 +135,7 @@
     int lastB = (p.N - 1 - n0) < 255 ? (p.N - 1 - n0) : 255, bshift = 0;
     const bf16_t* pB = p.B + (size_t)n0 * p.ldb + (size_t)kt0 * 64;
     if (EPI == 1) {
-      pB = p.B + (size_t)pid_n * 128 * p.ldb;
+      pB = p.B + (size_t)pid_n * 128 * p.ldb + (size_t)kt0 * 64;
       bshift = wave >= 4 ? p.sf_I - 128 : 0;
       lastB = 255;
     }
@@ -195,7 +214,7 @@
         : "memory", "scc", "vcc", "s40", "s41", "s42", "s43", "s44", "s45", "s46", "s47", "s48", "s49", "s50", "s51", "s52", "s53", G256K_CLOBBERS);
 #endif
     }
-    if constexpr (EPI == 0) if (part) {
+    if (part) {
 #pragma unroll
       for (int hf = 0; hf < 2; ++hf) {
         if (hf) {
@@ -460,12 +479,8 @@
             const int idx = tid + 512 * k2;
             const int rl = idx >> 4, c = idx & 15;
             const int row = s4 * 64 + rl, m = m0 + row;
-            float gv[8], uv[8], o[8];
-            unpack8(*(const u32x4_t*)(smem + row * 512 + ((c ^ (row & 31)) << 4)), gv);
-            unpack8(*(const u32x4_t*)(smem + row * 512 + (((16 + c) ^ (row & 31)) << 4)), uv);
-#pragma unroll
-            for (int j = 0; j < 8; ++j) o[j] = swiglu_fwd_elem(gv[j], uv[j]);
-            pa[k2] = pack8(o);
+            pa[k2] = swiglu_fwd8(*(const u32x4_t*)(smem + row * 512 + ((c ^ (row & 31)) << 4)),
+                                 *(const u32x4_t*)(smem + row * 512 + (((16 + c) ^ (row & 31)) << 4)));
             if (p.sf_act && m < p.M) MLA_ST16(p.sf_act + (size_t)m * I + cbase + c * 8, pa[k2]);
           }
           if (p.sf_actT == nullptr) continue;
@@ -532,19 +547,12 @@
             pg[k4] = u32x4_t{0u, 0u, 0u, 0u};
             pu[k4] = pg[k4];
             if (m < p.M && n < p.N) {
-              float dv[8], gv[8], uv[8], dg[8], du[8];
-              unpack8(*(const u32x4_t*)(smem + row * 512 + ((ch ^ (row & 31)) << 4)), dv);
+              const u32x4_t dq = *(const u32x4_t*)(smem + row * 512 + ((ch ^ (row & 31)) << 4));
               if constexpr (ASM) {
-                unpack8(gq[k4], gv);
-                unpack8(uq[k4], uv);
+                swiglu_bwd8(dq, gq[k4], uq[k4], pg[k4], pu[k4]);
               } else {
-              unpack8(*(const u32x4_t*)(p.sw_gu + (size_t)m * ld2 + n), gv);
-              unpack8(*(const u32x4_t*)(p.sw_gu + (size_t)m * ld2 + I + n), uv);
+                swiglu_bwd8(dq, *(const u32x4_t*)(p.sw_gu + (size_t)m * ld2 + n), *(const u32x4_t*)(p.sw_gu + (size_t)m * ld2 + I + n), pg[k4], pu[k4]);
               }
-#pragma unroll
-              for (int j = 0; j < 8; ++j) swiglu_bwd_elem(dv[j], gv[j], uv[j], dg[j], du[j]);
-              pg[k4] = pack8(dg);
-              pu[k4] = pack8(du);
               MLA_ST16(p.sw_dgu + (size_t)m * ld2 + n, pg[k4]);
               MLA_ST16(p.sw_dgu + (size_t)m * ld2 + I + n, pu[k4]);
             }
@@ -1157,6 +1165,120 @@
   }
 }
 
+constexpr int FIX_ROWS = 16;
+
+__device__ __forceinline__ void tail_tile_coords(const GemmArgs& p, int tile, int& pid_m, int& pid_n) {
+  const int GROUP_M = MLA_GROUP_M;
+  const int num_m = (p.M + 255) / 256, num_n = (p.N + 255) / 256;
+  const int pid = p.sk_full + tile;
+  const int in_group = GROUP_M * num_n;
+  const int first_m = (pid / in_group) * GROUP_M;
+  const int gsz = (num_m - first_m) < GROUP_M ? (num_m - first_m) : GROUP_M;
+  pid_m = first_m + (pid % in_group) % gsz;
+  pid_n = (pid % in_group) / gsz;
+}
+
+__device__ __forceinline__ u32x4_t sum_partials8(const float* src, int split) {
+  f32x4_t a = *(const f32x4_t*)src, b = *(const f32x4_t*)(src + 4);
+  for (int sl = 1; sl < split; ++sl) {
+    a += *(const f32x4_t*)(src + (size_t)sl * 65536);
+    b += *(const f32x4_t*)(src + (size_t)sl * 65536 + 4);
+  }
+  const float v[8] = {a[0], a[1], a[2], a[3], b[0], b[1], b[2], b[3]};
+  return pack8(v);
+}
+
+__device__ __forceinline__ u32x4_t gather_piece8(const unsigned short* line) {
+  u32x4_t w;
+#pragma unroll
+  for (int j = 0; j < 4; ++j) w[j] = (uint32_t)line[2 * j] | ((uint32_t)line[2 * j + 1] << 16);
+  return w;
+}
+
+__global__ __launch_bounds__(256) void gemm256_fixup_swiglu_fwd_kernel(GemmArgs p) {
+  __shared__ unsigned short tr[128][FIX_ROWS + 2];
+  const int tile = blockIdx.x / (256 / FIX_ROWS), strip = blockIdx.x % (256 / FIX_ROWS);
+  int pid_m, pid_n;
+  tail_tile_coords(p, tile, pid_m, pid_n);
+  const int I = p.sf_I, cbase = pid_n * 128;
+  const int rl = threadIdx.x >> 4, c = threadIdx.x & 15;
+  const int ml = strip * FIX_ROWS + rl, m = pid_m * 256 + ml;
+  u32x4_t a = {0u, 0u, 0u, 0u};
+  if (m < p.M) {
+    const float* src = p.sk_ws + (size_t)tile * p.sk_split * 65536 + ml * 256 + c * 8;
+    const u32x4_t g = sum_partials8(src, p.sk_split), u = sum_partials8(src + 128, p.sk_split);
+    if (p.C) {
+      MLA_ST16((bf16_t*)p.C + (size_t)m * 2 * I + cbase + c * 8, g);
+      MLA_ST16((bf16_t*)p.C + (size_t)m * 2 * I + I + cbase + c * 8, u);
+    }
+    a = swiglu_fwd8(g, u);
+    if (p.sf_act) MLA_ST16(p.sf_act + (size_t)m * I + cbase + c * 8, a);
+  }
+  if (p.sf_actT == nullptr) return;
+#pragma unroll
+  for (int j = 0; j < 4; ++j) {
+    tr[c * 8 + 2 * j][rl] = (unsigned short)(a[j] & 0xffffu);
+    tr[c * 8 + 2 * j + 1][rl] = (unsigned short)(a[j] >> 16);
+  }
+  __syncthreads();
+  const int col = threadIdx.x >> 1, rc = threadIdx.x & 1;
+  const int mt = pid_m * 256 + strip * FIX_ROWS + rc * 8;
+  if (mt < p.M) MLA_ST16(p.sf_actT + (size_t)(cbase + col) * p.sf_ldt + mt, gather_piece8(&tr[col][rc * 8]));
+}
+
+__global__ __launch_bounds__(256) void gemm256_fixup_swiglu_bwd_kernel(GemmArgs p) {
+  __shared__ unsigned short tr[2][256][FIX_ROWS + 2];
+  const int tile = blockIdx.x / (256 / FIX_ROWS), strip = blockIdx.x % (256 / FIX_ROWS);
+  int pid_m, pid_n;
+  tail_tile_coords(p, tile, pid_m, pid_n);
+  const int I = p.sw_I, n0 = pid_n * 256;
+  const size_t ld2 = (size_t)2 * I;
+#pragma unroll
+  for (int k2 = 0; k2 < 2; ++k2) {
+    const int idx = threadIdx.x + 256 * k2;
+    const int rl = idx >> 5, ch = idx & 31;
+    const int ml = strip * FIX_ROWS + rl, m = pid_m * 256 + ml, n = n0 + ch * 8;
+    u32x4_t pg = {0u, 0u, 0u, 0u}, pu = pg;
+    if (m < p.M && n < p.N) {
+      const u32x4_t d = sum_partials8(p.sk_ws + (size_t)tile * p.sk_split * 65536 + ml * 256 + ch * 8, p.sk_split);
+      swiglu_bwd8(d, MLA_LD16(p.sw_gu + (size_t)m * ld2 + n), MLA_LD16(p.sw_gu + (size_t)m * ld2 + I + n), pg, pu);
+      MLA_ST16(p.sw_dgu + (size_t)m * ld2 + n, pg);
+      MLA_ST16(p.sw_dgu + (size_t)m * ld2 + I + n, pu);
+    }
+    if (p.sw_dguT) {
+#pragma unroll
+      for (int j = 0; j < 4; ++j) {
+        tr[0][ch * 8 + 2 * j][rl] = (unsigned short)(pg[j] & 0xffffu);
+        tr[0][ch * 8 + 2 * j + 1][rl] = (unsigned short)(pg[j] >> 16);
+        tr[1][ch * 8 + 2 * j][rl] = (unsigned short)(pu[j] & 0xffffu);
+        tr[1][ch * 8 + 2 * j + 1][rl] = (unsigned short)(pu[j] >> 16);
+      }
+    }
+  }
+  if (p.sw_dguT == nullptr) return;
+  __syncthreads();
+#pragma unroll
+  for (int k2 = 0; k2 < 2; ++k2) {
+    const int idx = threadIdx.x + 256 * k2;
+    const int col = idx >> 1, rc = idx & 1;
+    const int mt = pid_m * 256 + strip * FIX_ROWS + rc * 8, n = n0 + col;
+    if (mt < p.M && n < p.N) {
+      MLA_ST16(p.sw_dguT + (size_t)n * p.sw_ldt + mt, gather_piece8(&tr[0][col][rc * 8]));
+      MLA_ST16(p.sw_dguT + (size_t)(I + n) * p.sw_ldt + mt, gather_piece8(&tr[1][col][rc * 8]));
+    }
+  }
+}
+
+void launch_fixup(const GemmArgs& p, int tail, hipStream_t stream) {
+  if (p.sw_gu) {
+    hipLaunchKernelGGL(gemm256_fixup_swiglu_bwd_kernel, dim3(tail * (256 / FIX_ROWS)), dim3(256), 0, stream, p);
+  } else if (p.sf_I) {
+    hipLaunchKernelGGL(gemm256_fixup_swiglu_fwd_kernel, dim3(tail * (256 / FIX_ROWS)), dim3(256), 0, stream, p);
+  } else {
+    hipLaunchKernelGGL(gemm256_fixup_kernel, dim3(tail * 64), dim3(256), 0, stream, p);
+  }
+}
+
 inline int choose_split(int tiles, int ncu, int nt, size_t ws_bytes, int* full_out) {
   const int r = tiles % ncu;
   *full_out = tiles - r;
@@ -1172,6 +1294,11 @@
   return best;
 }
 
+inline int plan_split(int tiles, int ncu, int nt, size_t ws_bytes, bool swiglu_bwd_rm, int* full_out) {
+  const int s = choose_split(tiles, ncu, nt, ws_bytes, full_out);
+  return (s > 1 && *full_out % 8 == 0 && !(swiglu_bwd_rm && (nt & 1))) ? s : 1;
+}
+
 int g_ncu_plan = -1;
 int planned_cus(int device_cus) {
   if (g_ncu_plan < 0) {
@@ -1214,16 +1341,19 @@
                       (p.R == nullptr || ((p.ldr & 7) == 0 && (((uintptr_t)p.R) & 15) == 0)) && (p.bias == nullptr || (((uintptr_t)p.bias) & 15) == 0);
     if (p.sw_gu) {
       if constexpr (AM == 0 && BM_ == 1) {
+        const int tail = p.sk_split > 1 ? tiles - p.sk_full : 0;
+        const dim3 grid(p.sk_split > 1 ? p.sk_full + tail * p.sk_split : tiles);
         if (kloop_mode() && (p.K % 128) == 0) {
-          launch_asm<2, 0, 1>(p, dim3(tiles), 2 * BUF + 32768, stream);
+          launch_asm<2, 0, 1>(p, grid, 2 * BUF + 32768, stream);
         } else {
           static bool attr_sw = false;
           if (!attr_sw) {
             hipFuncSetAttribute((const void*)gemm256_kernel<0, 1, 2>, hipFuncAttributeMaxDynamicSharedMemorySize, 2 * BUF + 32768);
             attr_sw = true;
           }
-          hipLaunchKernelGGL((gemm256_kernel<0, 1, 2>), dim3(tiles), dim3(512), 2 * BUF + 32768, stream, p);
-        }
+          hipLaunchKernelGGL((gemm256_kernel<0, 1, 2>), grid, dim3(512), 2 * BUF + 32768, stream, p);
+        }
+        if (tail) launch_fixup(p, tail, stream);
       } else {
         mla_set_error("gemm256: the fused SwiGLU backward reads only its B operand reduction-major");
         return -1;
@@ -1256,20 +1386,19 @@
     attr_set = true;
   }
   const int num_m = (p.M + 255) / 256, num_n = (p.N + 255) / 256;
+  const int tail = p.sk_split > 1 ? num_m * num_n - p.sk_full : 0;
+  const dim3 grid(p.sk_split > 1 ? p.sk_full + tail * p.sk_split : num_m * num_n);
   const bool fast = (p.N & 7) == 0 && (p.ldc & 7) == 0 && (((uintptr_t)p.C) & 15) == 0 &&
                     (p.R == nullptr || ((p.ldr & 7) == 0 && (((uintptr_t)p.R) & 15) == 0)) && (p.bias == nullptr || (((uintptr_t)p.bias) & 15) == 0);
   if (kloop_mode() && (p.K % 128) == 0 && fast && persistent_grid <= 0) {
-    if (p.sk_split > 1) {
-      const int tail = num_m * num_n - p.sk_full;
-      launch_asm<0>(p, dim3(p.sk_full + tail * p.sk_split), 2 * BUF + 1024, stream);
-      hipLaunchKernelGGL(gemm256_fixup_kernel, dim3(tail * 64), dim3(256), 0, stream, p);
-    } else if (p.sw_gu) {
-      launch_asm<2>(p, dim3(num_m * num_n), 2 * BUF + 32768, stream);
+    if (p.sw_gu) {
+      launch_asm<2>(p, grid, 2 * BUF + 32768, stream);
     } else if (p.sf_I) {
-      launch_asm<1>(p, dim3(num_m * num_n), 2 * BUF + 1024, stream);
+      launch_asm<1>(p, grid, 2 * BUF + 1024, stream);
     } else {
-      launch_asm<0>(p, dim3(num_m * num_n), 2 * BUF + 1024, stream);
-    }
+      launch_asm<0>(p, grid, 2 * BUF + 1024, stream);
+    }
+    if (tail) launch_fixup(p, tail, stream);
     hipError_t e = hipGetLastError();
     if (e != hipSuccess) {
       mla_set_error("gemm256 launch failed: %s", hipGetErrorString(e));
@@ -1288,26 +1417,25 @@
     if (p.sk_split > 1) hipLaunchKernelGGL(gemm256_fixup_kernel, dim3((num_m * num_n - p.sk_full) * 64), dim3(256), 0, stream, p);
   } else
 #endif
-  if (p.sk_split > 1) {
-    const int tail = num_m * num_n - p.sk_full;
-    hipLaunchKernelGGL((gemm256_kernel<AM, BM_>), dim3(p.sk_full + tail * p.sk_split), dim3(512), 2 * BUF + 1024, stream, p);
-    hipLaunchKernelGGL(gemm256_fixup_kernel, dim3(tail * 64), dim3(256), 0, stream, p);
-  } else if (p.sw_gu) {
+  if (p.sw_gu) {
     static bool attr_sw = false;
     if (!attr_sw) {
       hipFuncSetAttribute((const void*)gemm256_kernel<AM, BM_, 2>, hipFuncAttributeMaxDynamicSharedMemorySize, 2 * BUF + 32768);
       attr_sw = true;
     }
-    hipLaunchKernelGGL((gemm256_kernel<AM, BM_, 2>), dim3(num_m * num_n), dim3(512), 2 * BUF + 32768, stream, p);
+    hipLaunchKernelGGL((gemm256_kernel<AM, BM_, 2>), grid, dim3(512), 2 * BUF + 32768, stream, p);
+    if (tail) launch_fixup(p, tail, stream);
   } else if (p.sf_I) {
     static bool attr_sf = false;
     if (!attr_sf) {
       hipFuncSetAttribute((const void*)gemm256_kernel<AM, BM_, 1>, hipFuncAttributeMaxDynamicSharedMemorySize, 2 * BUF + 1024);
       attr_sf = true;
     }
-    hipLaunchKernelGGL((gemm256_kernel<AM, BM_, 1>), dim3(num_m * num_n), dim3(512), 2 * BUF + 1024, stream, p);
+    hipLaunchKernelGGL((gemm256_kernel<AM, BM_, 1>), grid, dim3(512), 2 * BUF + 1024, stream, p);
+    if (tail) launch_fixup(p, tail, stream);
   } else {
-    hipLaunchKernelGGL((gemm256_kernel<AM, BM_>), dim3(num_m * num_n), dim3(512), 2 * BUF + 1024, stream, p);
+    hipLaunchKernelGGL((gemm256_kernel<AM, BM_>), grid, dim3(512), 2 * BUF + 1024, stream, p);
+    if (tail) launch_fixup(p, tail, stream);
   }
   hipError_t e = hipGetLastError();
   if (e != hipSuccess) {
@@ -1342,8 +1470,9 @@
   return mla_gemm256_dispatch(&p, 0, 0, 0, stream);
 }
 
-extern "C" int mla_gemm_gateup_swiglu(const void* x, const void* wgu, void* gu, void* act, void* actT, int M, int I, int K, int lda,
-                                      int ldb, long long ldt, hipStream_t stream) {
+extern "C" int mla_gemm_gateup_swiglu_ws(const void* x, const void* wgu, void* gu, void* act, void* actT, int M, int I, int K, int lda,
+                                         int ldb, long long ldt, float* workspace, size_t workspace_bytes, hipStream_t stream) {
+  MLA_CHECK_ARG((((uintptr_t)workspace) & 15) == 0, "mla_gemm_gateup_swiglu: 16-B alignment required");
   MLA_CHECK_ARG(x && wgu && (act || actT) && (gu || act), "mla_gemm_gateup_swiglu: null pointer (act may be NULL only when actT is given, gu only when act is)");
   MLA_CHECK_ARG(M >= 256 && I >= 128 && I % 128 == 0 && K > 0 && K % 64 == 0, "mla_gemm_gateup_swiglu: needs M >= 256, I %% 128 == 0, K %% 64 == 0");
   MLA_CHECK_ARG(lda >= K && ldb >= K && lda % 8 == 0 && ldb % 8 == 0, "mla_gemm_gateup_swiglu: leading dimensions must be multiples of 8");
@@ -1354,11 +1483,17 @@
   p.A = (const bf16_t*)x; p.B = (const bf16_t*)wgu; p.C = gu; p.M = M; p.N = 2 * I; p.K = K; p.lda = lda; p.ldb = ldb; p.ldc = 2 * I;
   p.alpha = 1.f;
   p.sf_I = I; p.sf_act = (bf16_t*)act; p.sf_actT = (bf16_t*)actT; p.sf_ldt = ldt;
-  return mla_gemm256_dispatch(&p, 0, 0, 0, stream);
-}
-
-extern "C" int mla_gemm_dact_swiglu_bwd(const void* dy, const void* wT, const void* gu, void* dgu, void* dguT, int M, int I, int K,
-                                        int lda, int ldb, long long ldt, hipStream_t stream) {
+  p.sk_ws = workspace;
+  return mla_gemm256_dispatch(&p, 0, 0, workspace ? workspace_bytes : 0, stream);
+}
+extern "C" int mla_gemm_gateup_swiglu(const void* x, const void* wgu, void* gu, void* act, void* actT, int M, int I, int K, int lda,
+                                      int ldb, long long ldt, hipStream_t stream) {
+  return mla_gemm_gateup_swiglu_ws(x, wgu, gu, act, actT, M, I, K, lda, ldb, ldt, nullptr, 0, stream);
+}
+
+extern "C" int mla_gemm_dact_swiglu_bwd_ws(const void* dy, const void* wT, const void* gu, void* dgu, void* dguT, int M, int I, int K,
+                                           int lda, int ldb, long long ldt, float* workspace, size_t workspace_bytes, hipStream_t stream) {
+  MLA_CHECK_ARG((((uintptr_t)workspace) & 15) == 0, "mla_gemm_dact_swiglu_bwd: 16-B alignment required");
   MLA_CHECK_ARG(dy && wT && gu && dgu, "mla_gemm_dact_swiglu_bwd: null pointer");
   MLA_CHECK_ARG(M >= 256 && I >= 256 && K > 0 && K % 64 == 0 && I % 8 == 0 && M % 8 == 0,
                 "mla_gemm_dact_swiglu_bwd: needs M, I >= 256, K %% 64 == 0, I %% 8 == 0, M %% 8 == 0");
@@ -1370,11 +1505,17 @@
   p.A = (const bf16_t*)dy; p.B = (const bf16_t*)wT; p.C = dgu ;
   p.M = M; p.N = I; p.K = K; p.lda = lda; p.ldb = ldb; p.ldc = 2 * I; p.alpha = 1.f;
   p.sw_gu = (const bf16_t*)gu; p.sw_dgu = (bf16_t*)dgu; p.sw_dguT = (bf16_t*)dguT; p.sw_I = I; p.sw_ldt = ldt;
-  return mla_gemm256_dispatch(&p, 0, 0, 0, stream);
-}
-
-extern "C" int mla_gemm_dact_swiglu_bwd_rm(const void* dy, const void* w, const void* gu, void* dgu, void* dguT, int M, int I, int K,
-                                           int lda, int ldb, long long ldt, hipStream_t stream) {
+  p.sk_ws = workspace;
+  return mla_gemm256_dispatch(&p, 0, 0, workspace ? workspace_bytes : 0, stream);
+}
+extern "C" int mla_gemm_dact_swiglu_bwd(const void* dy, const void* wT, const void* gu, void* dgu, void* dguT, int M, int I, int K,
+                                        int lda, int ldb, long long ldt, hipStream_t stream) {
+  return mla_gemm_dact_swiglu_bwd_ws(dy, wT, gu, dgu, dguT, M, I, K, lda, ldb, ldt, nullptr, 0, stream);
+}
+
+extern "C" int mla_gemm_dact_swiglu_bwd_rm_ws(const void* dy, const void* w, const void* gu, void* dgu, void* dguT, int M, int I, int K,
+                                              int lda, int ldb, long long ldt, float* workspace, size_t workspace_bytes, hipStream_t stream) {
+  MLA_CHECK_ARG((((uintptr_t)workspace) & 15) == 0, "mla_gemm_dact_swiglu_bwd_rm: 16-B alignment required");
   MLA_CHECK_ARG(dy && w && gu && dgu, "mla_gemm_dact_swiglu_bwd_rm: null pointer");
   MLA_CHECK_ARG(M >= 256 && I >= 256 && K > 0 && K % 64 == 0 && I % 8 == 0 && M % 8 == 0,
                 "mla_gemm_dact_swiglu_bwd_rm: needs M, I >= 256, K %% 64 == 0, I %% 8 == 0, M %% 8 == 0");
@@ -1387,7 +1528,24 @@
   p.A = (const bf16_t*)dy; p.B = (const bf16_t*)w; p.C = dgu ;
   p.M = M; p.N = I; p.K = K; p.lda = lda; p.ldb = ldb; p.ldc = 2 * I; p.alpha = 1.f;
   p.sw_gu = (const bf16_t*)gu; p.sw_dgu = (bf16_t*)dgu; p.sw_dguT = (bf16_t*)dguT; p.sw_I = I; p.sw_ldt = ldt;
-  return mla_gemm256_dispatch(&p, 0, 1, 0, stream);
+  p.sk_ws = workspace;
+  return mla_gemm256_dispatch(&p, 0, 1, workspace ? workspace_bytes : 0, stream);
+}
+extern "C" int mla_gemm_dact_swiglu_bwd_rm(const void* dy, const void* w, const void* gu, void* dgu, void* dguT, int M, int I, int K,
+                                           int lda, int ldb, long long ldt, hipStream_t stream) {
+  return mla_gemm_dact_swiglu_bwd_rm_ws(dy, w, gu, dgu, dguT, M, I, K, lda, ldb, ldt, nullptr, 0, stream);
+}
+
+extern "C" int mla_gemm_tail_plan(int M, int N, int K, size_t workspace_bytes, int swiglu_bwd_rm, int* full_tiles) {
+  if (M < 256 || N < 256 || K <= 0 || (K % 64) != 0) return -1;
+  int ncu = 0, dev = 0, full = 0;
+  (void)hipGetDevice(&dev);
+  (void)hipDeviceGetAttribute(&ncu, hipDeviceAttributeMultiprocessorCount, dev);
+  if (ncu <= 0) ncu = 256;
+  const int tiles = ((M + 255) / 256) * ((N + 255) / 256);
+  const int s = workspace_bytes ? plan_split(tiles, planned_cus(ncu), K / 64, workspace_bytes, swiglu_bwd_rm != 0, &full) : 1;
+  if (full_tiles) *full_tiles = s > 1 ? full : tiles;
+  return s;
 }
 
 extern "C" int mla_gemm_res_norm(const void* A, const void* B, void* C, const void* R, const void* g, void* xg, float* ss, int M, int N,
@@ -1520,8 +1678,8 @@
   }
   if (p.sk_ws && ws_bytes) {
     int full = 0;
-    const int s = choose_split(tiles, planned_cus(ncu), p.K / 64, ws_bytes, &full);
-    if (s > 1 && full % 8 == 0) { p.sk_split = s; p.sk_full = full; }
+    const int s = plan_split(tiles, planned_cus(ncu), p.K / 64, ws_bytes, p.sw_gu != nullptr && b_mode == 1, &full);
+    if (s > 1) { p.sk_split = s; p.sk_full = full; }
   }
   const size_t bytesA = ((size_t)(p.M - 1) * p.lda + p.K) * 2, bytesB = ((size_t)(p.N - 1) * p.ldb + p.K) * 2;
   const int grid = ncu & ~7;
diff --git a/mla_amd/hip.py b/mla_amd/hip.py
--- a/mla_amd/hip.py
+++ b/mla_amd/hip.py
@@ -107,6 +107,13 @@
                                  c_void_p],
     "mla_gemm_dact_swiglu_bwd_rm": [c_void_p, c_void_p, c_void_p, c_void_p, c_void_p, c_int, c_int, c_int, c_int, c_int, c_longlong,
                                     c_void_p],
+    "mla_gemm_gateup_swiglu_ws": [c_void_p, c_void_p, c_void_p, c_void_p, c_void_p, c_int, c_int, c_int, c_int, c_int, c_longlong,
+                                  c_void_p, c_size_t, c_void_p],
+    "mla_gemm_dact_swiglu_bwd_ws": [c_void_p, c_void_p, c_void_p, c_void_p, c_void_p, c_int, c_int, c_int, c_int, c_int, c_longlong,
+                                    c_void_p, c_size_t, c_void_p],
+    "mla_gemm_dact_swiglu_bwd_rm_ws": [c_void_p, c_void_p, c_void_p, c_void_p, c_void_p, c_int, c_int, c_int, c_int, c_int, c_longlong,
+                                       c_void_p, c_size_t, c_void_p],
+    "mla_gemm_tail_plan": [c_int, c_int, c_int, c_size_t, c_int, c_void_p],
     "mla_rmsnorm_fwd": [c_void_p, c_void_p, c_void_p, c_void_p, c_int, c_int, c_float, c_void_p],
     "mla_rmsnorm_apply": [c_void_p, c_void_p, c_void_p, c_void_p, c_longlong, c_int, c_void_p],
     "mla_rmsnorm_prep": [c_void_p, c_void_p, c_void_p, c_void_p, c_int, c_int, c_float, c_void_p],
@@ -411,6 +418,24 @@
     return True
 
 
+_FUSED_TAIL = os.environ.get("MLA_FUSED_TAIL", "1")
+FUSED_TAIL = {"gateup": _FUSED_TAIL != "0", "dact": _FUSED_TAIL == "all"}
+
+
+def _fused_tail_ws(kind, device, tail, ws):
+    if not (FUSED_TAIL[kind] if tail is None else tail) or not SPLITK:
+        return None, 0
+    if ws is not None:
+        return ws, ws.numel() * ws.element_size()
+    return workspace(SPLITK_WS_BYTES, device), SPLITK_WS_BYTES
+
+
+def gemm_tail_plan(M: int, N: int, K: int, ws_bytes: Optional[int] = None, swiglu_bwd_rm: bool = False):
+    full = ctypes.c_int(0)
+    s = int(lib().mla_gemm_tail_plan(M, N, K, SPLITK_WS_BYTES if ws_bytes is None else int(ws_bytes), 1 if swiglu_bwd_rm else 0, ctypes.byref(full)))
+    return s, int(full.value)
+
+
 def gateup_swiglu_ok(x2d, wgu, want_t) -> bool:
     T, K = x2d.shape
     I = wgu.shape[0] // 2
@@ -418,7 +443,7 @@
             (not want_t or T % 8 == 0) and all(t.data_ptr() % 16 == 0 for t in (x2d, wgu)))
 
 
-def gemm_gateup_swiglu(x2d, wgu, want_t, norm=None, want_act=True, want_gu=True):
+def gemm_gateup_swiglu(x2d, wgu, want_t, norm=None, want_act=True, want_gu=True, tail=None, ws=None):
     T, K = x2d.shape
     I = wgu.shape[0] // 2
     ok = gateup_swiglu_ok(x2d, wgu, want_t)
@@ -439,14 +464,15 @@
         call("mla_gemm_gateup_swiglu_rs", _p(x2d), _p(wgu), _p(gu), _p(act), _p(actT), T, I, K, x2d.stride(0), wgu.stride(0), T,
              _p(ss), parts, eps, _p(rstd))
     else:
-        call("mla_gemm_gateup_swiglu", _p(x2d), _p(wgu), _p(gu), _p(act), _p(actT), T, I, K, x2d.stride(0), wgu.stride(0), T)
+        ws, ws_bytes = _fused_tail_ws("gateup", x2d.device, tail, ws)
+        call("mla_gemm_gateup_swiglu_ws", _p(x2d), _p(wgu), _p(gu), _p(act), _p(actT), T, I, K, x2d.stride(0), wgu.stride(0), T, _p(ws), ws_bytes)
     if prof is not None:
         ev1.record()
         prof.append((ev0, ev1, 2.0 * T * 2 * I * K, (0, 0, T, 2 * I, K, "swiglu_fwd_epilogue")))
     return (gu, act, actT) if norm is None else (gu, act, actT, rstd)
 
 
-def gemm_dact_swiglu_bwd(dy2d, wT, gu2d, want_t=True):
+def gemm_dact_swiglu_bwd(dy2d, wT, gu2d, want_t=True, tail=None, ws=None):
     T, K = dy2d.shape
     I = wT.shape[0]
     ok = (T >= 256 and I >= 256 and K % 64 == 0 and I % 8 == 0 and T % 8 == 0 and gu2d.shape == (T, 2 * I) and gu2d.is_contiguous() and
@@ -461,7 +487,8 @@
     if prof is not None:
         ev0, ev1 = torch.cuda.Event(enable_timing=True), torch.cuda.Event(enable_timing=True)
         ev0.record()
-    call("mla_gemm_dact_swiglu_bwd", _p(dy2d), _p(wT), _p(gu2d), _p(dgu), _p(dguT), T, I, K, dy2d.stride(0), wT.stride(0), T)
+    ws, ws_bytes = _fused_tail_ws("dact", dy2d.device, tail, ws)
+    call("mla_gemm_dact_swiglu_bwd_ws", _p(dy2d), _p(wT), _p(gu2d), _p(dgu), _p(dguT), T, I, K, dy2d.stride(0), wT.stride(0), T, _p(ws), ws_bytes)
     if prof is not None:
         ev1.record()
         prof.append((ev0, ev1, 2.0 * T * I * K, (0, 0, T, I, K, "swiglu_bwd_epilogue")))
@@ -476,7 +503,7 @@
             w.stride(0) % 8 == 0 and all(t.data_ptr() % 16 == 0 for t in (dy2d, w, gu2d)))
 
 
-def gemm_dact_swiglu_bwd_rm(dy2d, w, gu2d, want_t=True, dgu=None, dguT=None):
+def gemm_dact_swiglu_bwd_rm(dy2d, w, gu2d, want_t=True, dgu=None, dguT=None, tail=None, ws=None):
     T, K = dy2d.shape
     I = w.shape[1]
     for t, nm in ((dy2d, "dy"), (w, "w"), (gu2d, "gu")):
@@ -496,7 +523,8 @@
     if prof is not None:
         ev0, ev1 = torch.cuda.Event(enable_timing=True), torch.cuda.Event(enable_timing=True)
         ev0.record()
-    call("mla_gemm_dact_swiglu_bwd_rm", _p(dy2d), _p(w), _p(gu2d), _p(dgu), _p(dguT), T, I, K, dy2d.stride(0), w.stride(0), T)
+    ws, ws_bytes = _fused_tail_ws("dact", dy2d.device, tail, ws)
+    call("mla_gemm_dact_swiglu_bwd_rm_ws", _p(dy2d), _p(w), _p(gu2d), _p(dgu), _p(dguT), T, I, K, dy2d.stride(0), w.stride(0), T, _p(ws), ws_bytes)
     if prof is not None:
         ev1.record()
         prof.append((ev0, ev1, 2.0 * T * I * K, (0, 1, T, I, K, "swiglu_bwd_epilogue")))
```

After: 14.52 samples/s. No clear change (-0.2%).
